# tanmayrainanda/ishara

Hardware: AMD Instinct MI355X
Metric: landmark-frames/sec training (B=256,T=384,d=256) (higher is better)
Workload: dtype bf16; 1 GPU; configs[1]: get_model(dim=256, 2 squeeze + 2 conformer blocks, kernel_sizes=[11,5,3]) CTC train step (fwd+CTC+bwd+RAdam/Lookahead, dropout on); batch_per_gpu=256, global_batch=256, frames=384, features=224, params=7577784, parallelism=dp1, ranks_seen=1

## Files before the change

### include/ishara_hip.h

```cpp
#ifndef ISHARA_HIP_H
#define ISHARA_HIP_H
#include <stdint.h>
#ifdef __cplusplus
extern "C" {
#endif

typedef struct ishara_model ishara_model;
typedef void* ishara_stream;

enum { ISHARA_F32 = 0, ISHARA_BF16 = 1, ISHARA_F16 = 2 };
enum { ISHARA_FAMILY_KERAS_HYBRID = 0, ISHARA_FAMILY_TORCH_CONFORMER = 1, ISHARA_FAMILY_TORCH_SQUEEZEFORMER = 2 };

typedef struct ishara_config {
    int32_t dim;
    int32_t num_conv_squeeze_blocks;
    int32_t num_conv_conform_blocks;
    int32_t num_kernel_sizes;
    int32_t kernel_sizes[8];
    int32_t num_conv_per_block;
    float   dropout_rate;
    int32_t num_heads;
    int32_t expansion_factor;
    int32_t transformer_kernel_size;
    int32_t frames;
    int32_t features;
    int32_t num_classes;
    int32_t top_dim;
    int32_t squeeze_expansion;
    int32_t conformer_expansion;
    float   head_dropout;
    float   conformer_attn_dropout;
    int32_t dtype;
    int32_t max_batch;
    int32_t max_label_len;
    int32_t attn_impl;
    int32_t family;
    int32_t reduce_layer_index;
    int32_t recover_layer_index;
    int32_t half_step_residual;
} ishara_config;

const char* ishara_last_error(void);

int  ishara_create(const ishara_config* cfg, ishara_model** out);
void ishara_destroy(ishara_model* m);

int64_t ishara_param_total(const ishara_model* m);
int64_t ishara_param_trainable(const ishara_model* m);
int32_t ishara_param_entries(const ishara_model* m);
int  ishara_param_info(const ishara_model* m, int32_t i, const char** name, int32_t* ndim,
                       int64_t shape[2], int64_t* offset, int32_t* trainable);
int64_t ishara_workspace_bytes(const ishara_model* m);

int32_t ishara_workspace_plan_check(const ishara_model* m);
int ishara_workspace_guard_check(ishara_model* m);

int ishara_bind(ishara_model* m, float* params, float* grads, float* opt_m, float* opt_v,
                float* opt_slow, void* workspace, int64_t workspace_bytes);
int ishara_sync_weights(ishara_model* m, ishara_stream s);

int ishara_forward(ishara_model* m, const float* x, int32_t B, float* logits, int32_t training,
                   uint32_t seed, ishara_stream s);
int ishara_loss_backward(ishara_model* m, const float* logits, const int64_t* labels, int32_t B,
                         float* loss, float* nll, float loss_scale, ishara_stream s);
int ishara_encoder_forward(ishara_model* m, const float* x, int32_t B, float* y, int32_t training, uint32_t seed, ishara_stream s);
int32_t ishara_encoder_output_frames(const ishara_model* m);
int ishara_encoder_backward(ishara_model* m, const float* dy, int32_t B, float* dx, ishara_stream s);
int32_t ishara_grad_buckets(const ishara_model* m);
int ishara_grad_bucket(const ishara_model* m, int32_t i, int64_t* offset, int64_t* count);
int ishara_grad_buckets_enable(ishara_model* m);
int ishara_grad_bucket_wait(ishara_model* m, int32_t i, ishara_stream side);
int ishara_optimizer_step(ishara_model* m, float lr, float weight_decay, ishara_stream s);
int32_t ishara_optimizer_iterations(const ishara_model* m);
int ishara_optimizer_set_iterations(ishara_model* m, int32_t it);

int ishara_profile_enable(ishara_model* m, int32_t on);
int ishara_profile_report(ishara_model* m, char* buf, int32_t cap);

int ishara_greedy_decode(const float* logits, int32_t B, int32_t T, int32_t C, int32_t blank,
                         int32_t* out_idx, int32_t* out_len, ishara_stream s);
int ishara_preprocess(const float* raw, const int32_t* n_frames, int32_t max_frames, const float* mean, const float* stdv,
                      float* out, int32_t T, ishara_stream s);
int ishara_preprocess_batch(const float* raw, int64_t n_total, const int64_t* offsets, int32_t B, int32_t max_frames,
                            const float* mean, const float* stdv, float* out, int32_t T, ishara_stream s);
int ishara_edit_distance(const int32_t* out_idx, const int32_t* out_len, int32_t B, int32_t T, const int32_t* targets, int32_t L,
                         int32_t* dist, int32_t* tlen, ishara_stream s);

int64_t ishara_ctc_beam_workspace_bytes(int32_t B, int32_t T, int32_t C, int32_t beam_width);
int ishara_ctc_beam_decode(const float* logits, int32_t B, int32_t T, int32_t C, int32_t blank, int32_t beam_width, int32_t nbest,
                           const float* lm, float alpha, float beta, void* workspace,
                           int32_t* out_idx, int32_t* out_len, float* out_score, ishara_stream s);

int64_t ishara_ctc_align_workspace_bytes(int32_t B, int32_t T, int32_t L);
int ishara_ctc_align(const float* logits, const int64_t* labels, int32_t B, int32_t T, int32_t C, int32_t L, int32_t blank,
                     void* ws, int32_t* frame_pos, int32_t* start, int32_t* end, float* conf, float* score, ishara_stream s);

typedef struct ishara_clip_aug {
    int64_t offset;
    int32_t n;
    int32_t L1;
    int32_t shift;
    int32_t L2;
    int32_t mirror;
    int32_t t0[3];
    int32_t t1[3];
    int32_t fingers[3];
} ishara_clip_aug;
enum { ISHARA_LAYOUT_FLAT = 0, ISHARA_LAYOUT_HANDS_LIPS_XY = 1 };
int ishara_clip_batch(const float* raw, const ishara_clip_aug* clips, int32_t B, int32_t T, int32_t layout,
                      float* x, ishara_stream s);
int64_t ishara_ctc_workspace_bytes(int32_t B, int32_t T, int32_t L);
int ishara_ctc_loss(const float* logits, const int64_t* labels, int32_t B, int32_t T, int32_t C,
                    int32_t L, int32_t blank, float* nll, float* dlogits, float grad_scale,
                    void* ws, ishara_stream s);
int ishara_dropout_mask(uint32_t seed, uint32_t site, int32_t rows, int32_t cols, float rate,
                        float* out, ishara_stream s);

int ishara_debug_set_as_flags(int32_t flags);
int ishara_debug_set_nt_big(int32_t on);
int ishara_debug_force_regstage(int32_t on);
int32_t ishara_debug_module_count(ishara_model* m);
int ishara_debug_module_info(ishara_model* m, int32_t i, const char** name, int32_t* in_cols, int32_t* out_cols, int32_t* first_site, int32_t* n_sites);
int ishara_debug_module_forward(ishara_model* m, int32_t i, const float* x, int32_t B, float* y, int32_t training, uint32_t seed, ishara_stream s);
int ishara_debug_module_backward(ishara_model* m, int32_t i, const float* dy, int32_t B, float* dx, ishara_stream s);
int ishara_debug_head_loss_backward(ishara_model* m, const float* logits, const int64_t* labels, int32_t B, float* loss, float* nll,
                                    float loss_scale, float* dx, ishara_stream s);

int64_t ishara_op_scratch_bytes(int32_t M, int32_t K, int32_t N);
int ishara_op_dense_fwd(int32_t dt, const void* x, const float* W, const float* bias, void* y,
                        int32_t M, int32_t K, int32_t N, int32_t act, void* scratch, ishara_stream s);
int ishara_op_dense_fwd_ex(int32_t dt, const void* x, const float* W, const float* bias, const void* resid, void* y,
                           int32_t M, int32_t K, int32_t N, int32_t act, void* scratch, ishara_stream s);
int ishara_op_dense_bwd(int32_t dt, const void* x, const float* W, const void* dy, void* dx,
                        float* dW, float* db, int32_t M, int32_t K, int32_t N, void* scratch, ishara_stream s);
int64_t ishara_op_qkv_scratch_bytes(int32_t B, int32_t T, int32_t H, int32_t dh);
int ishara_op_qkv_fwd(int32_t dt, const void* x, const float* gamma, const float* beta, float eps, const float* W, const float* bias,
                      void* q, void* k, void* vt, int32_t B, int32_t T, int32_t H, int32_t dh, int32_t head_major, void* scratch, ishara_stream s);
int ishara_op_classifier_fwd(int32_t dt, const void* x, const float* W, const float* bias, float* logits, int32_t M, int32_t K, int32_t C,
                             int32_t route, void* scratch, ishara_stream s);
int ishara_op_ctc_loss(const float* logits, const int64_t* labels, int32_t B, int32_t T, int32_t C, int32_t L, int32_t blank,
                       float* nll, float* dlogits, float grad_scale, void* ws, void* dlb, ishara_stream s);
int ishara_op_log_softmax_fwd(const float* x, float* y, int32_t M, int32_t C, int32_t ld, ishara_stream s);
int ishara_op_log_softmax_bwd(const float* dy, const float* y, float* dx, int32_t M, int32_t C, int32_t ld, ishara_stream s);
int ishara_op_layernorm_fwd(int32_t dt, const void* x, const float* gamma, const float* beta, float eps,
                            void* y, float* mean, float* rstd, int32_t M, int32_t C, ishara_stream s);
int ishara_op_layernorm_bwd(int32_t dt, const void* dy, const void* x, const float* mean, const float* rstd,
                            const float* gamma, void* dx, float* dgamma, float* dbeta, int32_t M, int32_t C,
                            ishara_stream s);
int ishara_op_dwconv_fwd(int32_t dt, int32_t inop, const void* x, const float* w, const float* bias, void* y,
                         float* ssum, float* ssq, int32_t B, int32_t T, int32_t C, int32_t k, int32_t padl,
                         ishara_stream s);
int64_t ishara_op_dwconv_fwd_scratch_bytes(int32_t B, int32_t T, int32_t C);
int ishara_op_dwconv_fwd_ex(int32_t dt, int32_t inop, const void* x, const float* w, const float* bias, void* y,
                            float* ssum, float* ssq, void* scratch, int32_t B, int32_t T, int32_t C, int32_t k,
                            int32_t padl, ishara_stream s);
int64_t ishara_op_dwconv_scratch_bytes(int32_t C, int32_t k);
int ishara_op_dwconv_bwd(int32_t dt, int32_t inop, const void* dy, const void* x, const float* w, void* dx,
                         float* dw, float* dbias, void* scratch, int32_t B, int32_t T, int32_t C, int32_t k,
                         int32_t padl, ishara_stream s);
int64_t ishara_op_attn_scratch_bytes(int32_t B, int32_t H, int32_t T, int32_t dh);
int ishara_op_attn_scratch_layout_bytes(int32_t B, int32_t H, int32_t T, int32_t dh, int64_t* out);
int ishara_op_attn_fwd(int32_t dt, const void* qkv, void* o, int32_t B, int32_t H, int32_t T, int32_t dh,
                       float scale, uint32_t seed, uint32_t site, float rate, int32_t impl,
                       void* scratch, ishara_stream s);
int ishara_op_attn_bwd(int32_t dt, const void* o, const void* dout, void* dqkv, int32_t B, int32_t H,
                       int32_t T, int32_t dh, float scale, uint32_t seed, uint32_t site, float rate,
                       int32_t impl, void* scratch, ishara_stream s);

int64_t ishara_op_relattn_scratch_bytes(int32_t B, int32_t H, int32_t T, int32_t dh);
int ishara_op_relattn_fwd(int32_t dt, const void* q, const void* k, const void* v, const float* pe, const float* Wpos, const float* u, const float* vb,
                          void* o, float* lse, int32_t B, int32_t H, int32_t T, int32_t dh, uint32_t seed, uint32_t site, float rate,
                          void* scratch, ishara_stream s);
int ishara_op_relattn_bwd(int32_t dt, const void* q, const void* k, const void* v, const float* u, const float* vb, const void* o, const void* dO,
                          void* dq, void* dk, void* dv, float* du, float* dvb, float* dWpos, float* dposp,
                          int32_t B, int32_t H, int32_t T, int32_t dh, uint32_t seed, uint32_t site, float rate, void* scratch, ishara_stream s);
int64_t ishara_op_r4_subsample_scratch_bytes(int32_t B, int32_t T0, int32_t F, int32_t d);
int ishara_op_r4_subsample_fwd(int32_t dt, const float* x, const float* w1, const float* b1, const float* w2, const float* b2, void* sub,
                               int32_t B, int32_t T0, int32_t F, int32_t d, void* scratch, ishara_stream s);
int ishara_op_r4_subsample_bwd(int32_t dt, const float* x, const float* w1, const float* w2, const void* sub, const void* dsub,
                               float* dw1, float* db1, float* dw2, float* db2, float* dx, int32_t B, int32_t T0, int32_t F, int32_t d,
                               void* scratch, ishara_stream s);
int64_t ishara_op_r4_time_reduce_scratch_bytes(int32_t B, int32_t Tin, int32_t d);
int ishara_op_r4_time_reduce_fwd(int32_t dt, const void* h, const float* conv_w, const float* conv_b, const float* Wred, const float* bred,
                                 void* red, void* conv_out, int32_t B, int32_t Tin, int32_t d, void* scratch, ishara_stream s);
int ishara_op_r4_time_reduce_bwd(int32_t dt, const void* h, const float* conv_w, const void* dred, const void* extra, void* dh,
                                 float* dconv_w, float* dconv_b, float* dWred, float* dbred, int32_t B, int32_t Tin, int32_t d,
                                 void* scratch, ishara_stream s);
int ishara_op_r4_rows(int32_t dt, int32_t mode, const void* src, const void* a, void* dst, int32_t B, int32_t Tdst, int32_t Tsrc, int32_t d,
                      ishara_stream s);

#ifdef __cplusplus
}
#endif
#endif
```

### ishara_amd/_lib.py

```python
from __future__ import annotations

import ctypes as C
import os

_HERE = os.path.dirname(os.path.abspath(__file__))
LIB_PATH = os.path.join(_HERE, "libishara_hip.so")

F32, BF16, F16 = 0, 1, 2
FAMILY_KERAS_HYBRID, FAMILY_TORCH_CONFORMER, FAMILY_TORCH_SQUEEZEFORMER = 0, 1, 2


class IsharaError(RuntimeError):
    pass


class Config(C.Structure):
    _fields_ = [
        ("dim", C.c_int32), ("num_conv_squeeze_blocks", C.c_int32), ("num_conv_conform_blocks", C.c_int32),
        ("num_kernel_sizes", C.c_int32), ("kernel_sizes", C.c_int32 * 8), ("num_conv_per_block", C.c_int32),
        ("dropout_rate", C.c_float), ("num_heads", C.c_int32), ("expansion_factor", C.c_int32),
        ("transformer_kernel_size", C.c_int32), ("frames", C.c_int32), ("features", C.c_int32),
        ("num_classes", C.c_int32), ("top_dim", C.c_int32), ("squeeze_expansion", C.c_int32),
        ("conformer_expansion", C.c_int32), ("head_dropout", C.c_float), ("conformer_attn_dropout", C.c_float),
        ("dtype", C.c_int32), ("max_batch", C.c_int32), ("max_label_len", C.c_int32), ("attn_impl", C.c_int32),
        ("family", C.c_int32), ("reduce_layer_index", C.c_int32), ("recover_layer_index", C.c_int32), ("half_step_residual", C.c_int32),
    ]


class ClipAug(C.Structure):
    _fields_ = [
        ("offset", C.c_int64), ("n", C.c_int32), ("L1", C.c_int32), ("shift", C.c_int32), ("L2", C.c_int32),
        ("mirror", C.c_int32), ("t0", C.c_int32 * 3), ("t1", C.c_int32 * 3), ("fingers", C.c_int32 * 3),
    ]


LAYOUT_FLAT, LAYOUT_HANDS_LIPS_XY = 0, 1


_P, _I32, _I64, _U32, _F = C.c_void_p, C.c_int32, C.c_int64, C.c_uint32, C.c_float
SIGNATURES = {
    "ishara_last_error": (C.c_char_p, []),
    "ishara_create": (C.c_int, [C.POINTER(Config), C.POINTER(_P)]),
    "ishara_destroy": (None, [_P]),
    "ishara_param_total": (_I64, [_P]),
    "ishara_param_trainable": (_I64, [_P]),
    "ishara_param_entries": (_I32, [_P]),
    "ishara_param_info": (C.c_int, [_P, _I32, C.POINTER(C.c_char_p), C.POINTER(_I32), C.POINTER(_I64 * 2), C.POINTER(_I64), C.POINTER(_I32)]),
    "ishara_workspace_bytes": (_I64, [_P]),
    "ishara_workspace_plan_check": (_I32, [_P]),
    "ishara_workspace_guard_check": (C.c_int, [_P]),
    "ishara_grad_buckets": (_I32, [_P]),
    "ishara_grad_bucket": (C.c_int, [_P, _I32, C.POINTER(C.c_int64), C.POINTER(C.c_int64)]),
    "ishara_grad_buckets_enable": (C.c_int, [_P]),
    "ishara_grad_bucket_wait": (C.c_int, [_P, _I32, _P]),
    "ishara_bind": (C.c_int, [_P, _P, _P, _P, _P, _P, _P, _I64]),
    "ishara_sync_weights": (C.c_int, [_P, _P]),
    "ishara_forward": (C.c_int, [_P, _P, _I32, _P, _I32, _U32, _P]),
    "ishara_encoder_forward": (C.c_int, [_P, _P, _I32, _P, _I32, _U32, _P]),
    "ishara_encoder_backward": (C.c_int, [_P, _P, _I32, _P, _P]),
    "ishara_encoder_output_frames": (_I32, [_P]),
    "ishara_loss_backward": (C.c_int, [_P, _P, _P, _I32, _P, _P, _F, _P]),
    "ishara_optimizer_step": (C.c_int, [_P, _F, _F, _P]),
    "ishara_optimizer_iterations": (_I32, [_P]),
    "ishara_optimizer_set_iterations": (C.c_int, [_P, _I32]),
    "ishara_profile_enable": (C.c_int, [_P, _I32]),
    "ishara_profile_report": (C.c_int, [_P, C.c_char_p, _I32]),
    "ishara_greedy_decode": (C.c_int, [_P, _I32, _I32, _I32, _I32, _P, _P, _P]),
    "ishara_preprocess": (C.c_int, [_P, _P, _I32, _P, _P, _P, _I32, _P]),
    "ishara_preprocess_batch": (C.c_int, [_P, _I64, _P, _I32, _I32, _P, _P, _P, _I32, _P]),
    "ishara_edit_distance": (C.c_int, [_P, _P, _I32, _I32, _P, _I32, _P, _P, _P]),
    "ishara_ctc_beam_workspace_bytes": (_I64, [_I32, _I32, _I32, _I32]),
    "ishara_ctc_beam_decode": (C.c_int, [_P, _I32, _I32, _I32, _I32, _I32, _I32, _P, _F, _F, _P, _P, _P, _P, _P]),
    "ishara_ctc_align_workspace_bytes": (_I64, [_I32, _I32, _I32]),
    "ishara_ctc_align": (C.c_int, [_P, _P, _I32, _I32, _I32, _I32, _I32, _P, _P, _P, _P, _P, _P, _P]),
    "ishara_clip_batch": (C.c_int, [_P, _P, _I32, _I32, _I32, _P, _P]),
    "ishara_ctc_workspace_bytes": (_I64, [_I32, _I32, _I32]),
    "ishara_ctc_loss": (C.c_int, [_P, _P, _I32, _I32, _I32, _I32, _I32, _P, _P, _F, _P, _P]),
    "ishara_op_ctc_loss": (C.c_int, [_P, _P, _I32, _I32, _I32, _I32, _I32, _P, _P, _F, _P, _P, _P]),
    "ishara_dropout_mask": (C.c_int, [_U32, _U32, _I32, _I32, _F, _P, _P]),
    "ishara_debug_set_as_flags": (C.c_int, [_I32]),
    "ishara_debug_set_nt_big": (C.c_int, [_I32]),
    "ishara_debug_force_regstage": (C.c_int, [_I32]),
    "ishara_debug_module_count": (_I32, [_P]),
    "ishara_debug_module_info": (C.c_int, [_P, _I32, C.POINTER(C.c_char_p), C.POINTER(_I32), C.POINTER(_I32), C.POINTER(_I32), C.POINTER(_I32)]),
    "ishara_debug_module_forward": (C.c_int, [_P, _I32, _P, _I32, _P, _I32, _U32, _P]),
    "ishara_debug_module_backward": (C.c_int, [_P, _I32, _P, _I32, _P, _P]),
    "ishara_debug_head_loss_backward": (C.c_int, [_P, _P, _P, _I32, _P, _P, _F, _P, _P]),
    "ishara_op_scratch_bytes": (_I64, [_I32, _I32, _I32]),
    "ishara_op_dense_fwd": (C.c_int, [_I32, _P, _P, _P, _P, _I32, _I32, _I32, _I32, _P, _P]),
    "ishara_op_dense_fwd_ex": (C.c_int, [_I32, _P, _P, _P, _P, _P, _I32, _I32, _I32, _I32, _P, _P]),
    "ishara_op_dense_bwd": (C.c_int, [_I32, _P, _P, _P, _P, _P, _P, _I32, _I32, _I32, _P, _P]),
    "ishara_op_qkv_scratch_bytes": (_I64, [_I32, _I32, _I32, _I32]),
    "ishara_op_qkv_fwd": (C.c_int, [_I32, _P, _P, _P, _F, _P, _P, _P, _P, _P, _I32, _I32, _I32, _I32, _I32, _P, _P]),
    "ishara_op_classifier_fwd": (C.c_int, [_I32, _P, _P, _P, _P, _I32, _I32, _I32, _I32, _P, _P]),
    "ishara_op_log_softmax_fwd": (C.c_int, [_P, _P, _I32, _I32, _I32, _P]),
    "ishara_op_log_softmax_bwd": (C.c_int, [_P, _P, _P, _I32, _I32, _I32, _P]),
    "ishara_op_layernorm_fwd": (C.c_int, [_I32, _P, _P, _P, _F, _P, _P, _P, _I32, _I32, _P]),
    "ishara_op_layernorm_bwd": (C.c_int, [_I32, _P, _P, _P, _P, _P, _P, _P, _P, _I32, _I32, _P]),
    "ishara_op_dwconv_fwd": (C.c_int, [_I32, _I32, _P, _P, _P, _P, _P, _P, _I32, _I32, _I32, _I32, _I32, _P]),
    "ishara_op_dwconv_scratch_bytes": (_I64, [_I32, _I32]),
    "ishara_op_dwconv_fwd_scratch_bytes": (_I64, [_I32, _I32, _I32]),
    "ishara_op_dwconv_fwd_ex": (C.c_int, [_I32, _I32, _P, _P, _P, _P, _P, _P, _P, _I32, _I32, _I32, _I32, _I32, _P]),
    "ishara_op_dwconv_bwd": (C.c_int, [_I32, _I32, _P, _P, _P, _P, _P, _P, _P, _I32, _I32, _I32, _I32, _I32, _P]),
    "ishara_op_attn_scratch_bytes": (_I64, [_I32, _I32, _I32, _I32]),
    "ishara_op_attn_scratch_layout_bytes": (C.c_int, [_I32, _I32, _I32, _I32, C.POINTER(_I64)]),
    "ishara_op_attn_fwd": (C.c_int, [_I32, _P, _P, _I32, _I32, _I32, _I32, _F, _U32, _U32, _F, _I32, _P, _P]),
    "ishara_op_attn_bwd": (C.c_int, [_I32, _P, _P, _P, _I32, _I32, _I32, _I32, _F, _U32, _U32, _F, _I32, _P, _P]),
    "ishara_op_relattn_scratch_bytes": (_I64, [_I32, _I32, _I32, _I32]),
    "ishara_op_relattn_fwd": (C.c_int, [_I32] + [_P] * 9 + [_I32, _I32, _I32, _I32, _U32, _U32, _F, _P, _P]),
    "ishara_op_relattn_bwd": (C.c_int, [_I32] + [_P] * 14 + [_I32, _I32, _I32, _I32, _U32, _U32, _F, _P, _P]),
    "ishara_op_r4_subsample_scratch_bytes": (_I64, [_I32, _I32, _I32, _I32]),
    "ishara_op_r4_subsample_fwd": (C.c_int, [_I32] + [_P] * 6 + [_I32, _I32, _I32, _I32, _P, _P]),
    "ishara_op_r4_subsample_bwd": (C.c_int, [_I32] + [_P] * 10 + [_I32, _I32, _I32, _I32, _P, _P]),
    "ishara_op_r4_time_reduce_scratch_bytes": (_I64, [_I32, _I32, _I32]),
    "ishara_op_r4_time_reduce_fwd": (C.c_int, [_I32] + [_P] * 7 + [_I32, _I32, _I32, _P, _P]),
    "ishara_op_r4_time_reduce_bwd": (C.c_int, [_I32] + [_P] * 9 + [_I32, _I32, _I32, _P, _P]),
    "ishara_op_r4_rows": (C.c_int, [_I32, _I32, _P, _P, _P, _I32, _I32, _I32, _I32, _P]),
}

_lib = None


def load():
    global _lib
    if _lib is not None:
        return _lib
    if not os.path.exists(LIB_PATH):
        raise IsharaError(f"{LIB_PATH} is missing: build it with `python -m ishara_amd.build` "
                          "(hipcc --offload-arch=gfx950); there is no CPU fallback")
    lib = C.CDLL(LIB_PATH)
    for name, (res, args) in SIGNATURES.items():
        fn = getattr(lib, name)
        fn.restype = res
        fn.argtypes = args
    _lib = lib
    return lib


def check(rc: int, what: str = ""):
    if rc != 0:
        msg = load().ishara_last_error()
        raise IsharaError(f"{what} failed (rc={rc}): {msg.decode() if msg else '?'}")


def ptr(t):
    return None if t is None else C.c_void_p(t.data_ptr())


def stream():
    import torch
    return C.c_void_p(torch.cuda.current_stream().cuda_stream)


def aligned(nbytes: int, device):
    import torch
    t = torch.empty(int(nbytes) + 256, dtype=torch.uint8, device=device)
    return t, C.c_void_p(t.data_ptr() + (-t.data_ptr()) % 256)
```

### ishara_amd/csrc/api_ops.hip

```cpp
#include "model_types.h"

__global__ void dropout_mask_kernel(float* out, int rows, int cols, DropSpec d) {
    const size_t n = (size_t)rows * cols;
    for (size_t i = (size_t)blockIdx.x * blockDim.x + threadIdx.x; i < n; i += (size_t)gridDim.x * blockDim.x) {
        const uint32_t r = (uint32_t)(i / cols), c = (uint32_t)(i % cols);
        out[i] = (d.thr == 0u || rng_keep(rng_row_key(d.key, r), c, d.thr)) ? d.scale : 0.f;
    }
}
template <typename T>
__global__ void qkv_split_kernel(const T* qkv, T* q, T* k, T* vt, int B, int H, int Tn, int dh) {
    const int d = H * dh;
    const size_t n = (size_t)B * Tn * 3 * d;
    for (size_t i = (size_t)blockIdx.x * blockDim.x + threadIdx.x; i < n; i += (size_t)gridDim.x * blockDim.x) {
        const size_t m = i / (3 * d);
        const int col = (int)(i - m * 3 * d);
        const int h = col / (3 * dh), w = col - h * 3 * dh, part = w / dh, e = w - part * dh;
        const int b = (int)(m / Tn), t = (int)(m - (size_t)b * Tn);
        const T v = qkv[i];
        if (part == 0) q[((size_t)(b * H + h) * Tn + t) * dh + e] = v;
        else if (part == 1) k[((size_t)(b * H + h) * Tn + t) * dh + e] = v;
        else vt[((size_t)(b * H + h) * dh + e) * Tn + t] = v;
    }
}

// ... 55 lines not shown
                                       const float* mean, const float* stdv, float* out, int32_t T, ishara_stream s) {
    if (max_frames <= 0 || max_frames > 8192) { ishara_set_error("ishara_preprocess_batch: max_frames %d unsupported (1..8192)", max_frames); return -1; }
    if (B < 0 || B > 65535 || T < 1 || T > 4096) { ishara_set_error("ishara_preprocess_batch: B=%d T=%d unsupported (0 <= B <= 65535, 1 <= T <= 4096)", B, T); return -1; }
    if (n_total < 0) { ishara_set_error("ishara_preprocess_batch: n_total %lld < 0", (long long)n_total); return -1; }
    if (B > 0 && (!offsets || !mean || !stdv || !out || (n_total > 0 && !raw))) { ishara_set_error("ishara_preprocess_batch: null raw / offsets / mean / stdv / out"); return -1; }
    if (((uintptr_t)raw | (uintptr_t)out) % 16) { ishara_set_error("ishara_preprocess_batch: raw and out must be 16-byte aligned"); return -1; }
    return launch_preprocess_batch(raw, n_total, offsets, B, max_frames, mean, stdv, out, T, (hipStream_t)s);
}
extern "C" int ishara_edit_distance(const int32_t* out_idx, const int32_t* out_len, int32_t B, int32_t T, const int32_t* targets, int32_t L,
                                    int32_t* dist, int32_t* tlen, ishara_stream s) {
    if (L < 1 || L > SCORE_MAX_L) { ishara_set_error("ishara_edit_distance: target length L=%d unsupported (1..%d: one wavefront lane per target symbol)", L, SCORE_MAX_L); return -1; }
    if (B < 0 || T < 1 || T > 4096) { ishara_set_error("ishara_edit_distance: B=%d T=%d unsupported (B >= 0, 1 <= T <= 4096)", B, T); return -1; }
    if (B > 0 && (!out_idx || !out_len || !targets || !dist || !tlen)) { ishara_set_error("ishara_edit_distance: null argument"); return -1; }
    return launch_edit_distance(out_idx, out_len, B, T, targets, L, dist, tlen, (hipStream_t)s);
}
extern "C" int64_t ishara_ctc_beam_workspace_bytes(int32_t B, int32_t T, int32_t C, int32_t beam_width) {
    (void)C;
    if (B < 0 || T < 1 || T > 4096 || beam_width < 1 || beam_width > 32) return -1;
    return (int64_t)B * (int64_t)ctc_beam_workspace_words(T, beam_width) * 4;
}
extern "C" int ishara_ctc_beam_decode(const float* logits, int32_t B, int32_t T, int32_t C, int32_t blank, int32_t beam_width, int32_t nbest,
                                      const float* lm, float alpha, float beta, void* workspace,
                                      int32_t* out_idx, int32_t* out_len, float* out_score, ishara_stream s) {
    if (C < 2 || C > 64) { ishara_set_error("ishara_ctc_beam_decode: C=%d unsupported (2..64: one lane per class)", C); return -1; }
    if (blank < 0 || blank >= C) { ishara_set_error("ishara_ctc_beam_decode: blank %d outside 0..%d", blank, C - 1); return -1; }
    if (beam_width < 1 || beam_width > 32) { ishara_set_error("ishara_ctc_beam_decode: beam_width %d unsupported (1..32)", beam_width); return -1; }
    if (nbest < 1 || nbest > beam_width) { ishara_set_error("ishara_ctc_beam_decode: nbest %d outside 1..beam_width=%d", nbest, beam_width); return -1; }
    if (B < 0 || B > 2147483647 / 2 || T < 1 || T > 4096) { ishara_set_error("ishara_ctc_beam_decode: B=%d T=%d unsupported (B >= 0, 1 <= T <= 4096)", B, T); return -1; }
    if (!(alpha == alpha && beta == beta) || alpha - alpha != 0.0f || beta - beta != 0.0f) { ishara_set_error("ishara_ctc_beam_decode: alpha and beta must be finite"); return -1; }
    if (B > 0 && (!logits || !workspace || !out_idx || !out_len || !out_score)) { ishara_set_error("ishara_ctc_beam_decode: null argument"); return -1; }
    if ((uintptr_t)workspace % 4) { ishara_set_error("ishara_ctc_beam_decode: workspace must be 4-byte aligned"); return -1; }
    return launch_ctc_beam(logits, B, T, C, blank, beam_width, nbest, lm, alpha, beta, workspace, out_idx, out_len, out_score, (hipStream_t)s);
}
extern "C" int64_t ishara_ctc_align_workspace_bytes(int32_t B, int32_t T, int32_t L) {
    if (B < 0 || T < 1 || T > 4096 || L < 1 || L > 255) return -1;
    return (int64_t)ctc_align_workspace_bytes(B, T, L);
}
extern "C" int ishara_ctc_align(const float* logits, const int64_t* labels, int32_t B, int32_t T, int32_t C, int32_t L, int32_t blank,
                                void* ws, int32_t* frame_pos, int32_t* start, int32_t* end, float* conf, float* score, ishara_stream s) {
    const char* me = "ishara_ctc_align";
    if (B < 0) { ishara_set_error("%s: B=%d < 0", me, B); return -1; }
    if (T < 1 || T > 4096) { ishara_set_error("%s: T=%d outside 1..4096", me, T); return -1; }
    if (L < 1 || L > 255) { ishara_set_error("%s: L=%d outside 1..255 (2L+1 lattice states in at most 8 registers of a 64-lane wave)", me, L); return -1; }
    if (C < 2 || C > 64) { ishara_set_error("%s: C=%d outside 2..64", me, C); return -1; }
    if (blank < 0 || blank >= C) { ishara_set_error("%s: blank %d outside 0..%d", me, blank, C - 1); return -1; }
    if (B == 0) return 0;
    if (!logits || !labels || !ws || !frame_pos || !start || !end || !conf || !score) {
        ishara_set_error("%s: null logits / labels / ws / frame_pos / start / end / conf / score", me); return -1;
    }
    if ((uintptr_t)ws % 16) { ishara_set_error("%s: ws must be 16-byte aligned", me); return -1; }
    return launch_ctc_align(logits, labels, B, T, C, L, blank, ws, frame_pos, start, end, conf, score, (hipStream_t)s);
}
extern "C" int ishara_clip_batch(const float* raw, const ishara_clip_aug* clips, int32_t B, int32_t T, int32_t layout,
                                 float* x, ishara_stream s) {
    if (B < 0 || T < 1 || T > CLIP_MAX_T) { ishara_set_error("ishara_clip_batch: B=%d T=%d unsupported (B >= 0, 1 <= T <= %d)", B, T, CLIP_MAX_T); return -1; }
    if (layout != ISHARA_LAYOUT_FLAT && layout != ISHARA_LAYOUT_HANDS_LIPS_XY) { ishara_set_error("ishara_clip_batch: unknown layout %d", layout); return -1; }
    if (B > 0 && (!clips || !x)) { ishara_set_error("ishara_clip_batch: null clips / x"); return -1; }
    if (((uintptr_t)raw | (uintptr_t)x) % 16) { ishara_set_error("ishara_clip_batch: raw and x must be 16-byte aligned"); return -1; }
    return launch_clip_batch(raw, clips, B, T, layout, x, (hipStream_t)s);
}

static bool op_dt_ok(const char* op, int dt, bool f16_ok) {
    if (dt != DT_F32 && dt != DT_BF16 && dt != DT_F16) { ishara_set_error("%s: unknown dtype %d (ISHARA_F32 = 0, ISHARA_BF16 = 1, ISHARA_F16 = 2)", op, dt); return false; }
    if (dt == DT_F16 && !f16_ok) { ishara_set_error("%s: ISHARA_F16 is inference-only (no fp16 backward kernels)", op); return false; }
    return true;
}
#define OP_DT(op, dt, f16_ok) do { if (!op_dt_ok(op, dt, f16_ok)) return -1; } while (0)
struct OpShadow {
    size_t wt, wn, slab, total; int ldt, ldn;
    OpShadow(int dt, int K, int N, int M) {
        const int bk = dt_is16(dt) ? 64 : 32;
        const size_t es = dt_size(dt);
        ldt = (int)rup(K, bk); ldn = (int)rup(N, bk);
        wt = 0;
        wn = rup(rup(N, 128) * (size_t)ldt * es, 256);
        slab = wn + rup(rup(K, 128) * (size_t)ldn * es, 256);
        total = slab + gemm_tn_slab_floats(M, K, N, dt) * sizeof(float);
    }
    int build(int dt, const float* Wm, int K, int N, char* sc, hipStream_t s) const {
        HIP_CHECK_RET(hipMemsetAsync(sc, 0, slab, s));
        return launch_make_shadow(dt, Wm, K, N, sc + wt, ldt, sc + wn, ldn, s);
    }
};
extern "C" int64_t ishara_op_scratch_bytes(int32_t M, int32_t K, int32_t N) {
    return (int64_t)OpShadow(DT_F32, K, N, M).total;
}
extern "C" int ishara_op_dense_fwd(int32_t dt, const void* x, const float* Wm, const float* bias, void* y, int32_t M, int32_t K, int32_t N, int32_t act, void* scratch, ishara_stream st) {
    OP_DT("ishara_op_dense_fwd", dt, true);
    hipStream_t s = (hipStream_t)st;
    const OpShadow sh(dt, K, N, M);
    char* sc = (char*)scratch;
    CK(sh.build(dt, Wm, K, N, sc, s));
    OpArgs no; EpiArgs ea; ea.bias = bias; ea.act = act; ea.dbg = g_dbg_epi;
    return launch_gemm_nt(dt, dt, dt, OP_NONE, x, sc + sh.wt, y, M, N, K, sh.ldt, no, ea, s);
}
extern "C" int ishara_op_dense_fwd_ex(int32_t dt, const void* x, const float* Wm, const float* bias, const void* resid, void* y,
                                      int32_t M, int32_t K, int32_t N, int32_t act, void* scratch, ishara_stream st) {
    OP_DT("ishara_op_dense_fwd_ex", dt, true);
    hipStream_t s = (hipStream_t)st;
    const OpShadow sh(dt, K, N, M);
    char* sc = (char*)scratch;
    CK(sh.build(dt, Wm, K, N, sc, s));
    OpArgs no; EpiArgs ea; ea.bias = bias; ea.act = act; ea.resid = resid; ea.dbg = g_dbg_epi;
    return launch_gemm_nt(dt, dt, dt, OP_NONE, x, sc + sh.wt, y, M, N, K, sh.ldt, no, ea, s);
}
extern "C" int ishara_op_dense_bwd(int32_t dt, const void* x, const float* Wm, const void* dy, void* dx, float* dW, float* db,
                                   int32_t M, int32_t K, int32_t N, void* scratch, ishara_stream st) {
    OP_DT("ishara_op_dense_bwd", dt, false);
    hipStream_t s = (hipStream_t)st;
    const OpShadow sh(dt, K, N, M);
    char* sc = (char*)scratch;
    CK(sh.build(dt, Wm, K, N, sc, s));
    OpArgs no; EpiArgs ea;
    if (dx) CK(launch_gemm_nt(dt, dt, dt, OP_NONE, dy, sc + sh.wn, dx, M, K, N, sh.ldn, no, ea, s));
    return launch_gemm_tn(dt, dt, dt, OP_NONE, OP_NONE, x, dy, dW, db, (float*)(sc + sh.slab), M, K, N, no, no, s);
}
static void qkv_scratch_layout(int B, int T, int H, int dh, size_t& xn, size_t& mean, size_t& rstd, size_t& total) {
    const int M = B * T, d = H * dh;
    xn = rup(OpShadow(DT_F32, d, 3 * d, M).total, 256);
    mean = xn + rup((size_t)M * d * 4, 256);
    rstd = mean + rup((size_t)M * 4, 256);
    total = rstd + rup((size_t)M * 4, 256);
}
extern "C" int64_t ishara_op_qkv_scratch_bytes(int32_t B, int32_t T, int32_t H, int32_t dh) {
    if (B < 1 || T < 1 || H < 1 || dh < 1) return -1;
    size_t xn, mean, rstd, total;
    qkv_scratch_layout(B, T, H, dh, xn, mean, rstd, total);
    return (int64_t)total;
}
extern "C" int ishara_op_qkv_fwd(int32_t dt, const void* x, const float* gamma, const float* beta, float eps, const float* Wm, const float* bias,
                                 void* q, void* k, void* vt, int32_t B, int32_t T, int32_t H, int32_t dh, int32_t head_major, void* scratch, ishara_stream st) {
    OP_DT("ishara_op_qkv_fwd", dt, true);
    if (B < 1 || T < 1 || H < 1 || dh < 1 || T % 8 != 0 || dh % 8 != 0 || (head_major != 0 && head_major != 1)) {
        ishara_set_error("ishara_op_qkv_fwd: B=%d T=%d H=%d dh=%d head_major=%d unsupported (T, dh multiples of 8; head_major 0 / 1)", B, T, H, dh, head_major); return -1;
    }
    const int d = H * dh, M = B * T;
    if ((gamma != nullptr) != (beta != nullptr) || (gamma && d > 512)) { ishara_set_error("ishara_op_qkv_fwd: LayerNorm needs both gamma and beta and H*dh <= 512 (H*dh=%d)", d); return -1; }
    if (!x || !Wm || !q || !k || !vt || !scratch || ((uintptr_t)x | (uintptr_t)scratch) % 16 != 0) { ishara_set_error("ishara_op_qkv_fwd: null or misaligned buffer (x, scratch: 16-byte aligned)"); return -1; }
    hipStream_t s = (hipStream_t)st;
    const OpShadow sh(dt, d, 3 * d, M);
    char* sc = (char*)scratch;
    CK(sh.build(dt, Wm, d, 3 * d, sc, s));
    OpArgs no;
    EpiArgs eq; eq.mode = EPI_QKV; eq.q = q; eq.k = k; eq.vt = vt; eq.H = H; eq.dh = dh; eq.T = T; eq.head_major = head_major;
    const void* A = x;
    if (gamma && !ln_as_prologue(dt, M, 3 * d, d, sh.ldt, gamma, beta, eps, nullptr, nullptr, nullptr, eq)) {
        size_t xn, mean, rstd, tot;
        qkv_scratch_layout(B, T, H, dh, xn, mean, rstd, tot);
        CK(launch_layernorm_fwd(dt, x, gamma, beta, eps, sc + xn, (float*)(sc + mean), (float*)(sc + rstd), M, d, s));
        A = sc + xn;
    }
    eq.bias = bias;
    return launch_gemm_nt(dt, dt, dt, OP_NONE, A, sc + sh.wt, nullptr, M, 3 * d, d, sh.ldt, no, eq, s);
}
extern "C" int ishara_op_classifier_fwd(int32_t dt, const void* x, const float* Wm, const float* bias, float* logits, int32_t M, int32_t K, int32_t C,
                                        int32_t route, void* scratch, ishara_stream st) {
    OP_DT("ishara_op_classifier_fwd", dt, true);
    if (route < CLS_AUTO || route > CLS_GEMM) { ishara_set_error("ishara_op_classifier_fwd: unknown route %d (0 auto, 1 A-stationary, 2 dense_narrow, 3 GEMM)", route); return -1; }
    if (M < 1 || K < 1 || C < 1) { ishara_set_error("ishara_op_classifier_fwd: bad shape M=%d K=%d C=%d", M, K, C); return -1; }
    const int r = route == CLS_AUTO ? cls_route_auto(dt, M, K, C) : route;
    const char* why = nullptr;
    if (r != CLS_GEMM && !dt_is16(dt)) why = "16-bit operands only";
    else if (r == CLS_AS && (C > 64 || C % 4 != 0 || (K != 256 && K != 512))) why = "C <= 64, C % 4 == 0 and K 256 / 512 only";
    else if (r == CLS_AS && g_force_regstage) why = "the A-stationary kernel is switched off (ishara_debug_force_regstage)";
    else if (r == CLS_NARROW && (C > 64 || K % 32 != 0)) why = "C <= 64 and K % 32 == 0 only";
    else if (r == CLS_GEMM && K % (dt_is16(dt) ? 8 : 4) != 0) why = "16-byte operand rows only";
    if (why) { ishara_set_error("ishara_op_classifier_fwd: route %d does not take dt=%d M=%d K=%d C=%d: %s", r, dt, M, K, C, why); return -1; }
    if (!x || !Wm || !logits || !scratch || ((uintptr_t)x | (uintptr_t)scratch) % 16 != 0) { ishara_set_error("ishara_op_classifier_fwd: null or misaligned buffer (x, scratch: 16-byte aligned)"); return -1; }
    hipStream_t s = (hipStream_t)st;
    const OpShadow sh(dt, K, C, M);
    char* sc = (char*)scratch;
    CK(sh.build(dt, Wm, K, C, sc, s));
    return classifier_fwd(nullptr, r, dt, x, sc + sh.wt, sh.ldt, bias, logits, M, K, C, s);
}
extern "C" int ishara_op_log_softmax_fwd(const float* x, float* y, int32_t M, int32_t C, int32_t ld, ishara_stream s) { return launch_log_softmax_fwd(x, y, M, C, ld, (hipStream_t)s); }
extern "C" int ishara_op_log_softmax_bwd(const float* dy, const float* y, float* dx, int32_t M, int32_t C, int32_t ld, ishara_stream s) { return launch_log_softmax_bwd(dy, y, dx, M, C, ld, (hipStream_t)s); }
extern "C" int ishara_op_layernorm_fwd(int32_t dt, const void* x, const float* gamma, const float* beta, float eps, void* y, float* mean, float* rstd, int32_t M, int32_t C, ishara_stream s) {
    OP_DT("ishara_op_layernorm_fwd", dt, true);
    return launch_layernorm_fwd(dt, x, gamma, beta, eps, y, mean, rstd, M, C, (hipStream_t)s);
}
extern "C" int ishara_op_layernorm_bwd(int32_t dt, const void* dy, const void* x, const float* mean, const float* rstd, const float* gamma, void* dx, float* dgamma, float* dbeta, int32_t M, int32_t C, ishara_stream s) {
    OP_DT("ishara_op_layernorm_bwd", dt, false);
    return launch_layernorm_bwd(dt, dy, x, mean, rstd, gamma, nullptr, dx, dgamma, dbeta, nullptr, M, C, (hipStream_t)s);
}
extern "C" int ishara_op_dwconv_fwd(int32_t dt, int32_t inop, const void* x, const float* w, const float* bias, void* y, float* ssum, float* ssq,
                                    int32_t B, int32_t T, int32_t C, int32_t k, int32_t padl, ishara_stream s) {
    OP_DT("ishara_op_dwconv_fwd", dt, true);
    return launch_dwconv_fwd(dt, inop, x, w, bias, y, ssum, ssq, nullptr, B, T, C, k, padl, (hipStream_t)s);
}
extern "C" int64_t ishara_op_dwconv_fwd_scratch_bytes(int32_t B, int32_t T, int32_t C) { return (int64_t)(dwconv_fwd_scratch_floats(B, T, C) * sizeof(float)); }
extern "C" int ishara_op_dwconv_fwd_ex(int32_t dt, int32_t inop, const void* x, const float* w, const float* bias, void* y, float* ssum, float* ssq,
                                       void* scratch, int32_t B, int32_t T, int32_t C, int32_t k, int32_t padl, ishara_stream s) {
    OP_DT("ishara_op_dwconv_fwd_ex", dt, true);
    return launch_dwconv_fwd(dt, inop, x, w, bias, y, ssum, ssq, (float*)scratch, B, T, C, k, padl, (hipStream_t)s);
}
extern "C" int64_t ishara_op_dwconv_scratch_bytes(int32_t C, int32_t k) { return (int64_t)(dwconv_bwd_scratch_floats(C, k) * sizeof(float)); }
extern "C" int ishara_op_dwconv_bwd(int32_t dt, int32_t inop, const void* dy, const void* x, const float* w, void* dx, float* dw, float* dbias,
                                    void* scratch, int32_t B, int32_t T, int32_t C, int32_t k, int32_t padl, ishara_stream s) {
    OP_DT("ishara_op_dwconv_bwd", dt, false);
    return launch_dwconv_bwd(dt, inop, dy, x, w, dx, dw, dbias, (float*)scratch, B, T, C, k, padl, (hipStream_t)s);
}
struct AttnScratch {
    void *q, *k, *vt; float *lse, *delta; uint32_t* maskw; size_t total;
    AttnScratch(char* sc, int B, int H, int T, int dh) {
        const size_t seg = rup((size_t)B * H * T * dh * 4, 256), row = rup((size_t)B * H * T * 4, 256);
        q = sc; k = sc + seg; vt = sc + 2 * seg;
        lse = (float*)(sc + 3 * seg);
        delta = (float*)(sc + 3 * seg + row);
        maskw = (uint32_t*)(sc + 3 * seg + 2 * row);
        total = 3 * seg + 2 * row + rup(attn_mask_words(B, H, T) * 4, 256);
    }
};
extern "C" int64_t ishara_op_attn_scratch_bytes(int32_t B, int32_t H, int32_t T, int32_t dh) { return (int64_t)AttnScratch(nullptr, B, H, T, dh).total; }
extern "C" int ishara_op_attn_scratch_layout_bytes(int32_t B, int32_t H, int32_t T, int32_t dh, int64_t* out) {
    const char* me = "ishara_op_attn_scratch_layout_bytes";
    if (B < 1 || H < 1 || T < 1 || dh < 1) { ishara_set_error("%s: B=%d H=%d T=%d dh=%d: B, H, T and dh must be >= 1", me, B, H, T, dh); return -1; }
    if (!out) { ishara_set_error("%s: null out", me); return -1; }
    const AttnScratch a(nullptr, B, H, T, dh);
    const int64_t row = (int64_t)B * H * T * 4;
    out[0] = (int64_t)(uintptr_t)a.lse; out[1] = row;
    out[2] = (int64_t)(uintptr_t)a.delta; out[3] = row;
    out[4] = (int64_t)(uintptr_t)a.maskw; out[5] = (int64_t)attn_mask_words(B, H, T) * 4;
    return 0;
}
static bool attn_takes_mfma(int dt, int dh, int impl) { return impl >= 1 && dt == DT_BF16 && (dh == 32 || dh == 64); }
static int attn_op_refused(const char* me, int dt, int B, int H, int T, int dh, float rate, int impl, std::initializer_list<const void*> operands,
                           std::initializer_list<const char*> operand_names, const void* scratch) {
    if (B < 1 || H < 1 || T < 1) { ishara_set_error("%s: B=%d H=%d T=%d: B, H and T must be >= 1", me, B, H, T); return -1; }
    if (dh != 8 && dh != 16 && dh != 24 && dh != 32 && dh != 48 && dh != 64) { ishara_set_error("%s: head dim %d unsupported (8, 16, 24, 32, 48, 64)", me, dh); return -1; }
    if (impl < 0 || impl > 2) { ishara_set_error("%s: unknown impl %d (0 lane-split, 1 MFMA with cached keep bits, 2 MFMA hashing again in the backward)", me, impl); return -1; }
    if (impl == 2 && !attn_takes_mfma(dt, dh, impl)) { ishara_set_error("%s: impl 2 has MFMA kernels only: ISHARA_BF16 and head dim 32 / 64 (dtype %d, head dim %d)", me, dt, dh); return -1; }
    if (attn_takes_mfma(dt, dh, impl) && T % 8 != 0) { ishara_set_error("%s: T=%d: the MFMA kernels need T %% 8 == 0 (16-byte pieces of the V^T rows)", me, T); return -1; }
    if (!(rate >= 0.f && rate < 1.f)) { ishara_set_error("%s: rate %g outside [0, 1)", me, rate); return -1; }
    if ((int64_t)B * H > 65535 || (int64_t)B * H * T * dh * 3 > 2147483647LL) { ishara_set_error("%s: B=%d H=%d T=%d dh=%d: shape too large (B*H <= 65535: one grid row per head; 3*B*H*T*dh < 2^31)", me, B, H, T, dh); return -1; }
    for (size_t i = 0; i < operands.size(); ++i) if (!operands.begin()[i]) { ishara_set_error("%s: null %s", me, operand_names.begin()[i]); return -1; }
    if (!scratch) { ishara_set_error("%s: null scratch (ishara_op_attn_scratch_bytes)", me); return -1; }
    for (size_t i = 0; i < operands.size(); ++i)
        if ((uintptr_t)operands.begin()[i] % 16) { ishara_set_error("%s: misaligned %s: 16-byte aligned operands (vector loads and stores)", me, operand_names.begin()[i]); return -1; }
    if ((uintptr_t)scratch % 256) { ishara_set_error("%s: misaligned scratch: 256-byte aligned (the layout rounds every region to 256 bytes)", me); return -1; }
    return 0;
}
extern "C" int ishara_op_attn_fwd(int32_t dt, const void* qkv, void* o, int32_t B, int32_t H, int32_t T, int32_t dh, float scale,
                                  uint32_t seed, uint32_t site, float rate, int32_t impl, void* scratch, ishara_stream st) {
    OP_DT("ishara_op_attn_fwd", dt, true);
    if (dt == DT_F16 && rate > 0.f) { ishara_set_error("ishara_op_attn_fwd: ISHARA_F16 is inference-only: no attention dropout (rate %g)", rate); return -1; }
    if (attn_op_refused("ishara_op_attn_fwd", dt, B, H, T, dh, rate, impl, {qkv, o}, {"qkv", "o"}, scratch)) return -1;
    hipStream_t s = (hipStream_t)st;
    const AttnScratch a((char*)scratch, B, H, T, dh);
    if (dt == DT_BF16) hipLaunchKernelGGL(qkv_split_kernel<bf16>, dim3(1024), dim3(256), 0, s, (const bf16*)qkv, (bf16*)a.q, (bf16*)a.k, (bf16*)a.vt, B, H, T, dh);
    else if (dt == DT_F16) hipLaunchKernelGGL(qkv_split_kernel<f16>, dim3(1024), dim3(256), 0, s, (const f16*)qkv, (f16*)a.q, (f16*)a.k, (f16*)a.vt, B, H, T, dh);
    else hipLaunchKernelGGL(qkv_split_kernel<float>, dim3(1024), dim3(256), 0, s, (const float*)qkv, (float*)a.q, (float*)a.k, (float*)a.vt, B, H, T, dh);
    return launch_attn_fwd(dt, a.q, a.k, a.vt, o, a.lse, B, H, T, dh, scale, make_drop_attn(seed, site, rate, true), impl == 2 ? 1 : impl, impl == 2 ? nullptr : a.maskw, s);
}
extern "C" int ishara_op_attn_bwd(int32_t dt, const void* o, const void* dout, void* dqkv, int32_t B, int32_t H, int32_t T, int32_t dh, float scale,
                                  uint32_t seed, uint32_t site, float rate, int32_t impl, void* scratch, ishara_stream st) {
    OP_DT("ishara_op_attn_bwd", dt, false);
    if (attn_op_refused("ishara_op_attn_bwd", dt, B, H, T, dh, rate, impl, {o, dout, dqkv}, {"o", "dout", "dqkv"}, scratch)) return -1;
    hipStream_t s = (hipStream_t)st;
    const AttnScratch a((char*)scratch, B, H, T, dh);
    return launch_attn_bwd(dt, a.q, a.k, a.vt, o, dout, a.lse, a.delta, dqkv, B, H, T, dh, scale, make_drop_attn(seed, site, rate, true), 1, impl == 2 ? 1 : impl,
                           impl == 2 ? nullptr : a.maskw, s);
}

static bool op_r4_dt_ok(const char* op, int dt) {
    if (dt != DT_F32 && dt != DT_BF16 && dt != DT_F16) { ishara_set_error("%s: unknown dtype %d (ISHARA_F32 = 0, ISHARA_BF16 = 1, ISHARA_F16 = 2)", op, dt); return false; }
    if (dt == DT_F16) { ishara_set_error("%s: ISHARA_F16 is not supported (the torch Squeezeformer family has no fp16 kernels)", op); return false; }
    return true;
}
#define OP_R4_DT(op, dt) do { if (!op_r4_dt_ok(op, dt)) return -1; } while (0)
static bool op_misaligned(std::initializer_list<const void*> ps) { uintptr_t a = 0; for (const void* p : ps) a |= (uintptr_t)p; return a % 16 != 0; }
static bool op_any_null(std::initializer_list<const void*> ps) { for (const void* p : ps) if (!p) return true; return false; }
static size_t op_shadow_bytes(int K, int N, int M) { const size_t a = OpShadow(DT_F32, K, N, M).total, b = OpShadow(DT_BF16, K, N, M).total; return rup(a > b ? a : b, 256); }

struct RelAttnScratch {
    size_t pedt, posp, dposp, lse, delta, total;
    RelAttnScratch(int B, int H, int T, int dh) {
        const size_t d = (size_t)H * dh, R = 2 * (size_t)T - 1, tab = rup(R * d * 4, 256), row = rup((size_t)B * H * T * 4, 256);
        pedt = op_shadow_bytes((int)d, (int)d, (int)R);
        posp = pedt + tab; dposp = posp + tab; lse = dposp + tab; delta = lse + row; total = delta + row;
    }
};
static const char* relattn_shape_error(int B, int H, int T, int dh, float rate) {
    if (dh != 8 && dh != 16 && dh != 32 && dh != 64) return "head dim unsupported (8, 16, 32, 64)";
    if (B < 1 || H < 1 || T < 1) return "B, H and T must be >= 1";
    if ((int64_t)B * H > 65535 || (int64_t)B * H * T * dh > 2147483647LL || (2 * (int64_t)T - 1) * H * dh > 2147483647LL) return "shape too large (B*H <= 65535, B*H*T*dh < 2^31)";
    if (!(rate >= 0.f && rate < 1.f)) return "rate outside [0, 1)";
    return nullptr;
}
extern "C" int64_t ishara_op_relattn_scratch_bytes(int32_t B, int32_t H, int32_t T, int32_t dh) {
    if (relattn_shape_error(B, H, T, dh, 0.f)) return -1;
    return (int64_t)RelAttnScratch(B, H, T, dh).total;
}
extern "C" int ishara_op_relattn_fwd(int32_t dt, const void* q, const void* k, const void* v, const float* pe, const float* Wpos, const float* u, const float* vb,
                                     void* o, float* lse, int32_t B, int32_t H, int32_t T, int32_t dh, uint32_t seed, uint32_t site, float rate, void* scratch, ishara_stream st) {
    const char* me = "ishara_op_relattn_fwd";
    OP_R4_DT(me, dt);
    if (const char* why = relattn_shape_error(B, H, T, dh, rate)) { ishara_set_error("%s: B=%d H=%d T=%d dh=%d rate=%g: %s", me, B, H, T, dh, rate, why); return -1; }
    if (op_any_null({q, k, v, pe, Wpos, u, vb, o, scratch}) || op_misaligned({q, k, v, pe, Wpos, u, vb, o, lse, scratch})) {
        ishara_set_error("%s: null or misaligned buffer (all 16-byte aligned; only lse may be NULL)", me); return -1;
    }
    hipStream_t s = (hipStream_t)st;
    const int d = H * dh, R = 2 * T - 1;
    const OpShadow sh(dt, d, d, R);
    const RelAttnScratch a(B, H, T, dh);
    char* sc = (char*)scratch;
    CK(sh.build(dt, Wpos, d, d, sc, s));
// ... 149 lines not shown
```

### ishara_amd/csrc/gemm_as.hip

```cpp
#include <cstdio>
#include <map>
#include <string>
#include <type_traits>
#include "common.h"
#include "kernels.h"

#ifdef AS_F16
typedef f16 as_t;
typedef f16x8 as_v8;
#define AS_MFMA(b, a, acc) __builtin_amdgcn_mfma_f32_16x16x32_f16(b, a, acc, 0, 0, 0)
#define AS_DT DT_F16
#define AS_NAME(x) x##_f16
#else
typedef bf16 as_t;
typedef bf16x8 as_v8;
#define AS_MFMA(b, a, acc) __builtin_amdgcn_mfma_f32_16x16x32_bf16(b, a, acc, 0, 0, 0)
#define AS_DT DT_BF16
#define AS_NAME(x) x
#endif

extern int g_force_regstage;
bool gemm_nt_as_applicable(int dtC, int M, int N, int K, int ldb, const EpiArgs& ea);

#define AS_NS 32
#define AS_SMALL_M 1536
#define AS_MID_M_K512 32768
#define AS_MAXN 1024

typedef __attribute__((ext_vector_type(4))) uint32_t as_u32x4;

template <int N> DEVI void as_wait_vm() { asm volatile("s_waitcnt vmcnt(%0)" ::"n"(N) : "memory"); }

DEVI int as_swz(int r) { return (r & 3) | (((r >> 3) & 1) << 2); }

template <int GW, typename T> DEVI void as_st(T* p, const float (&v)[GW]) {
    if constexpr (GW == 8) store8(p, v); else store4(p, v);
}
template <int GW, typename T> DEVI void as_st_nt(T* p, const float (&v)[GW], bool nt = true) {
    if constexpr (GW == 8 && is_16b_t<T>::value) {
        as_v8 t;
#pragma unroll
        for (int i = 0; i < 8; ++i) t[i] = (as_t)v[i];
        if (nt) __builtin_nontemporal_store(t, reinterpret_cast<as_v8*>(p)); else *reinterpret_cast<as_v8*>(p) = t;
    } else as_st<GW>(p, v);
}
DEVI void as_st_pk(as_t* p, const as_v8& t, bool nt) {
    if (nt) __builtin_nontemporal_store(t, reinterpret_cast<as_v8*>(p)); else *reinterpret_cast<as_v8*>(p) = t;
}
template <typename TC, int GW> DEVI void as_unpack(const as_u32x4& r, float (&v)[GW]) {
    if constexpr (GW == 8 && std::is_same<TC, f16>::value) {
        const f16x8 h = __builtin_bit_cast(f16x8, r);
#pragma unroll
        for (int e = 0; e < 8; ++e) v[e] = (float)h[e];
    } else if constexpr (GW == 8) {
#pragma unroll
        for (int h = 0; h < 4; ++h) { v[2 * h] = __uint_as_float(r[h] << 16); v[2 * h + 1] = __uint_as_float(r[h] & 0xffff0000u); }
    } else {
#pragma unroll
        for (int h = 0; h < 4; ++h) v[h] = __uint_as_float(r[h]);
    }
}

enum { AS_RESID = 1, AS_DACT = 2, AS_ACT = 4, AS_DROP = 8, AS_ROWSCALE = 16, AS_PREOUT = 32, AS_QKV = 64, AS_ADDTAB = 128, AS_ALL = 255 };
template <int MASK, int F> DEVI bool as_on(bool runtime) {
    if constexpr ((MASK & F) == 0) return false;
    else if constexpr (MASK == AS_ALL) return runtime;
    else return true;
}

template <typename TC, int KT, int MASK, int RT, int DBG, int PRO, int NW = 4, int CS = 1>
DEVI void as_pass(const as_t* __restrict__ A, const as_t* __restrict__ Bt, TC* __restrict__ C, int M, int N, int ldb, const EpiArgs& ea,
                  char* smem, const float* bias_s, int m_base) {
    constexpr int RB = KT * 64;
    constexpr int NS = AS_NS;
    constexpr int SUB = NS * RB;
    constexpr int STAGE = SUB * CS;
    constexpr int R = CS > 1 ? 2 : (KT <= 8 ? 3 : 2);
    constexpr int K = KT * 32;
    constexpr int NI = STAGE / 1024;
    constexpr int DPW = (NI + NW - 1) / NW;
    constexpr bool PAIR = is_16b_t<TC>::value;
    constexpr int GW = PAIR ? 8 : 4;
    constexpr int NG = NS / (4 * GW);
    constexpr int SPS = RT * NG;
    constexpr bool COUNTED = (MASK & (AS_RESID | AS_DACT | AS_ADDTAB | AS_QKV)) == 0;
    constexpr int OPS = SPS * ((MASK & AS_PREOUT) ? 2 : 1);
    constexpr bool HOLDABLE = PAIR && std::is_same<TC, as_t>::value && MASK != AS_ALL && (MASK & AS_QKV) == 0;
    const bool hold = HOLDABLE && (ea.as_flags & 1) && !ea.n_valid;
    const bool nt_side = (ea.as_flags & 2) != 0;

    const int dbg = DBG ? ea.dbg : 0;
    const int tid = threadIdx.x, lane = tid & 63;
    const int wid = __builtin_amdgcn_readfirstlane(tid >> 6);
    const int c = lane & 15, g = lane >> 4;
    const int mw = m_base + wid * 16 * RT;
    const bool full = m_base + NW * 16 * RT <= M;
    const int nsteps = N / NS / (int)gridDim.y;
    const int nbase = (int)blockIdx.y * nsteps * NS;
    const int dmodel = ea.H * ea.dh;
    const bool f_resid = as_on<MASK, AS_RESID>(ea.resid != nullptr), f_dact = as_on<MASK, AS_DACT>(ea.dact != DACT_NONE);
    const bool f_act = as_on<MASK, AS_ACT>(ea.act != ACT_NONE), f_drop = as_on<MASK, AS_DROP>(ea.drop.thr != 0);
    const bool f_rowscale = as_on<MASK, AS_ROWSCALE>(ea.rowscale != nullptr), f_preout = as_on<MASK, AS_PREOUT>(ea.pre_out != nullptr);
    const bool f_qkv = as_on<MASK, AS_QKV>(ea.mode == EPI_QKV), f_addtab = as_on<MASK, AS_ADDTAB>(ea.addtab != nullptr);

    const as_t* bsrc[DPW];
#pragma unroll
    for (int t = 0; t < DPW; ++t) {
        const int o = ((wid * DPW + t) % NI) * 1024 + lane * 16;
        const int r = o / RB, p = (o % RB) >> 4;
        bsrc[t] = Bt + (size_t)(nbase + r) * ldb + ((p ^ as_swz(r)) << 3);
    }
    const size_t bstep = (size_t)NS * CS * ldb;
    auto issue = [&](int slot) {
#pragma unroll
        for (int t = 0; t < DPW; ++t) {
            __builtin_amdgcn_global_load_lds((const __attribute__((address_space(1))) void*)bsrc[t],
                                             (__attribute__((address_space(3))) void*)(smem + slot + ((wid * DPW + t) % NI) * 1024), 16, 0, 0);
            bsrc[t] += bstep;
        }
    };
    const int nstages = (nsteps + CS - 1) / CS;
#pragma unroll
    for (int st = 0; st < R - 1; ++st)
        if (st < nstages && !(dbg & 8)) issue(st * STAGE);

    as_v8 a[RT][KT];
    int mrow[RT];
#pragma unroll
    for (int i = 0; i < RT; ++i) {
        mrow[i] = min(mw + 16 * i + c, M - 1);
        const as_v8* p = reinterpret_cast<const as_v8*>(A + (size_t)mrow[i] * K + g * 8);
#pragma unroll
        for (int kt = 0; kt < KT; ++kt) a[i][kt] = p[kt * 4];
    }

    if constexpr (PRO != 0) {
        float* cs = reinterpret_cast<float*>(smem + (R - 1) * STAGE);
        const int bsm = min(m_base, M - 1) / ea.T;
        const float* c0 = PRO == 1 ? ea.ln_gamma : ea.pa_P + (size_t)bsm * K;
        const float* c1 = PRO == 1 ? ea.ln_beta : ea.pa_Q + (size_t)bsm * K;
        for (int x = tid; x < K; x += NW * 64) { cs[x] = c0[x]; cs[K + x] = c1[x]; }
        __syncthreads();
        auto unpack = [&](const as_v8& f, float (&v)[8]) {
            as_u32x4 t = __builtin_bit_cast(as_u32x4, f);
            asm volatile("" : "+v"(t));
            as_unpack<as_t, 8>(t, v);
        };
        float mean[RT], rstd[RT];
#pragma unroll
        for (int i = 0; i < RT; ++i) { mean[i] = 0.f; rstd[i] = 1.f; }
        if constexpr (PRO == 1) {
#pragma unroll
            for (int i = 0; i < RT; ++i) {
                float s = 0.f;
#pragma unroll
                for (int kt = 0; kt < KT; ++kt) {
                    float v[8];
                    unpack(a[i][kt], v);
#pragma unroll
                    for (int e = 0; e < 8; ++e) s += v[e];
                }
                s += __shfl_xor(s, 16, 64); s += __shfl_xor(s, 32, 64);
                mean[i] = s * (1.f / K);
                float q = 0.f;
#pragma unroll
                for (int kt = 0; kt < KT; ++kt) {
                    float v[8];
                    unpack(a[i][kt], v);
#pragma unroll
                    for (int e = 0; e < 8; ++e) { const float dlt = v[e] - mean[i]; q += dlt * dlt; }
                }
                q += __shfl_xor(q, 16, 64); q += __shfl_xor(q, 32, 64);
                rstd[i] = rsqrtf(q * (1.f / K) + ea.ln_eps);
                const int m = mw + 16 * i + c;
                if (g == 0 && m < M && ea.ln_mean && blockIdx.y == 0) { ea.ln_mean[m] = mean[i]; ea.ln_rstd[m] = rstd[i]; }
            }
        }
#pragma unroll
        for (int kt = 0; kt < KT; ++kt) {
            float wv[8], bv[8];
            {
                const float* cp = cs + 32 * kt + 8 * g;
                asm volatile("" : "+v"(cp));
                const f32x4 w0 = *reinterpret_cast<const f32x4*>(cp), w1 = *reinterpret_cast<const f32x4*>(cp + 4);
                const f32x4 b0 = *reinterpret_cast<const f32x4*>(cp + K), b1 = *reinterpret_cast<const f32x4*>(cp + K + 4);
#pragma unroll
                for (int e = 0; e < 4; ++e) { wv[e] = w0[e]; wv[4 + e] = w1[e]; bv[e] = b0[e]; bv[4 + e] = b1[e]; }
            }
#pragma unroll
            for (int i = 0; i < RT; ++i) {
                float v[8];
                unpack(a[i][kt], v);
                as_v8 t;
#pragma unroll
                for (int e = 0; e < 8; ++e) t[e] = (as_t)(PRO == 1 ? (v[e] - mean[i]) * rstd[i] * wv[e] + bv[e] : v[e] * wv[e] + bv[e]);
                a[i][kt] = t;
            }
        }
        __syncthreads();
    }

    const int frow = PAIR ? 8 * (c >> 2) + (c & 3) : c;
    const int sx = g ^ as_swz(frow);
    const int off_e = frow * RB + ((sx & 3) << 4) + ((sx >> 2) << 6);
    const int off_o = frow * RB + ((sx & 3) << 4) + (((sx >> 2) ^ 1) << 6);
    constexpr int JSTRIDE = (PAIR ? 4 : 16) * RB;

    float rsc[RT];
    uint32_t rk[RT];
    int bsamp[RT];
#pragma unroll
    for (int i = 0; i < RT; ++i) {
        const int m = mw + 16 * i + c;
        rsc[i] = 1.f; rk[i] = 0u; bsamp[i] = 0;
        if (f_rowscale || f_qkv) bsamp[i] = mrow[i] / ea.T;
        if (f_rowscale) rsc[i] = ea.rowscale[bsamp[i]];
        if (f_drop) rk[i] = rng_row_key(ea.drop.key, (uint32_t)m);
    }

    size_t eoff[RT];
#pragma unroll
    for (int i = 0; i < RT; ++i) eoff[i] = (size_t)mrow[i] * (ea.ldc ? ea.ldc : N) + GW * g;
    const TC* resid = reinterpret_cast<const TC*>(ea.resid);
    const TC* aux = reinterpret_cast<const TC*>(ea.aux);

#pragma unroll
    for (int i = 0; i < RT; ++i) {
#pragma unroll
        for (int kt = 0; kt < KT; ++kt) {
            as_u32x4 t = __builtin_bit_cast(as_u32x4, a[i][kt]);
            asm volatile("" : "+v"(t));
            a[i][kt] = __builtin_bit_cast(as_v8, t);
        }
        asm volatile("" : "+v"(rsc[i]));
    }

    as_v8 held[RT], held_pre[RT];
#pragma unroll
    for (int i = 0; i < RT; ++i) { held[i] = as_v8{}; held_pre[i] = as_v8{}; }
    int slot = 0;
    for (int s = 0; s < nsteps; ++s) {
        const int sub = CS > 1 ? (s & (CS - 1)) : 0;
        const bool sync = CS == 1 || sub == 0;
        const int sg = CS > 1 ? s / CS : s;
        if (sync) {
            if constexpr (CS > 1) {
                constexpr bool CCOUNT = MASK != AS_ALL && (MASK & AS_QKV) == 0;
                if (CCOUNT && full && !ea.n_valid && sg >= 1) as_wait_vm<CS * OPS>(); else as_wait_vm<0>();
            } else if constexpr (COUNTED) {
                if (full && !ea.n_valid && s >= R - 1 && s + R - 2 < nsteps) {
                    if (!hold) as_wait_vm<(R - 2) * DPW + (R - 1) * OPS>();
                    else if constexpr (R == 3) as_wait_vm<DPW + 2 * OPS>();
                    else { if (s & 1) as_wait_vm<0>(); else as_wait_vm<2 * OPS>(); }
                } else as_wait_vm<0>();
            } else {
                if (s + R - 2 < nsteps) as_wait_vm<(R - 2) * DPW>(); else as_wait_vm<0>();
            }
            asm volatile("s_waitcnt lgkmcnt(0)" ::: "memory");
            __builtin_amdgcn_s_barrier();
        }
        const int n0 = nbase + s * NS;
        as_u32x4 rs[RT][NG], au[RT][NG];
        if (f_resid) {
#pragma unroll
            for (int i = 0; i < RT; ++i)
#pragma unroll
                for (int q = 0; q < NG; ++q) rs[i][q] = *reinterpret_cast<const as_u32x4*>(resid + eoff[i] + n0 + 4 * GW * q);
        }
        if (f_dact) {
#pragma unroll
            for (int i = 0; i < RT; ++i)
#pragma unroll
                for (int q = 0; q < NG; ++q) au[i][q] = __builtin_nontemporal_load(reinterpret_cast<const as_u32x4*>(aux + eoff[i] + n0 + 4 * GW * q));
        }
        if (sync && sg + R - 1 < nstages && !(dbg & 8)) issue(slot == 0 ? (R - 1) * STAGE : slot - STAGE);
        f32x4 acc[2][RT];
#pragma unroll
        for (int j = 0; j < 2; ++j)
#pragma unroll
            for (int i = 0; i < RT; ++i) acc[j][i] = f32x4{0.f, 0.f, 0.f, 0.f};
        const char* st = smem + slot + sub * SUB;
        if (!(dbg & 6)) {
#pragma unroll
            for (int kt = 0; kt < KT; ++kt) {
#pragma unroll
                for (int j = 0; j < 2; ++j) {
                    const as_v8 b = *reinterpret_cast<const as_v8*>(st + ((kt & 1) ? off_o : off_e) + (kt >> 1) * 128 + j * JSTRIDE);
#pragma unroll
                    for (int i = 0; i < RT; ++i) acc[j][i] = AS_MFMA(b, a[i][kt], acc[j][i]);
                }
            }
        } else if (!(dbg & 4)) {
#pragma unroll
            for (int kt = 0; kt < KT; ++kt)
#pragma unroll
                for (int j = 0; j < 2; ++j) {
                    const f32x4 b = *reinterpret_cast<const f32x4*>(st + ((kt & 1) ? off_o : off_e) + (kt >> 1) * 128 + j * JSTRIDE);
                    acc[j][0] += b;
                }
        } else if (!(dbg & 2)) {
            const as_v8 b = a[0][0];
#pragma unroll
            for (int kt = 0; kt < KT; ++kt)
#pragma unroll
                for (int j = 0; j < 2; ++j)
#pragma unroll
                    for (int i = 0; i < RT; ++i) acc[j][i] = AS_MFMA(b, a[i][kt], acc[j][i]);
        } else {
#pragma unroll
            for (int i = 0; i < RT; ++i) acc[0][i][0] = (float)a[i][0][0] + (float)a[i][KT - 1][7];
        }
        if (dbg & 1) { if (acc[0][0][0] == 123.456f) C[0] = from_f<TC>(acc[1][RT - 1][2]); if (CS == 1 || sub == CS - 1) slot = slot == (R - 1) * STAGE ? 0 : slot + STAGE; continue; }
#pragma unroll
        for (int q = 0; q < NG; ++q) {
            const int n = n0 + 4 * GW * q + GW * g;
            if (ea.n_valid && n >= ea.n_valid) continue;
            float bias[GW];
#pragma unroll
            for (int h = 0; h < GW / 4; ++h) {
                const f32x4 bv = *reinterpret_cast<const f32x4*>(bias_s + n + 4 * h);
#pragma unroll
                for (int e = 0; e < 4; ++e) bias[4 * h + e] = bv[e];
            }
#pragma unroll
            for (int i = 0; i < RT; ++i) {
                const int m = mw + 16 * i + c;
                if (!full && m >= M) continue;
                const size_t off = eoff[i] + n0 + 4 * GW * q;
                float v[GW];
                const float bsc = (f_rowscale && ea.rowscale_bias) ? rsc[i] : 1.f;
                if constexpr (PAIR) {
#pragma unroll
                    for (int e = 0; e < 4; ++e) { v[e] = acc[0][i][e] + bias[e] * bsc; v[4 + e] = acc[1][i][e] + bias[4 + e] * bsc; }
                } else {
#pragma unroll
                    for (int e = 0; e < 4; ++e) v[e] = acc[q][i][e] + bias[e] * bsc;
                }
                if (f_addtab) {
                    const float* tp = ea.addtab + (size_t)(m % ea.tab_period) * N + n;
#pragma unroll
                    for (int h = 0; h < GW / 4; ++h) {
                        float t4[4];
                        load4(tp + 4 * h, t4);
#pragma unroll
                        for (int e = 0; e < 4; ++e) v[4 * h + e] += t4[e];
                    }
                }
                if (f_preout) {
                    if constexpr (HOLDABLE) {
                        if (hold) {
                            as_v8 t;
#pragma unroll
                            for (int e = 0; e < 8; ++e) t[e] = (as_t)v[e];
                            as_t* pp = reinterpret_cast<as_t*>(ea.pre_out) + off;
                            if (s & 1) { as_st_pk(pp - NS, held_pre[i], nt_side); as_st_pk(pp, t, nt_side); }
                            else if (s == nsteps - 1) as_st_pk(pp, t, nt_side);
                            else held_pre[i] = t;
                        } else as_st_nt<GW>(reinterpret_cast<TC*>(ea.pre_out) + off, v, nt_side);
                    } else as_st_nt<GW>(reinterpret_cast<TC*>(ea.pre_out) + off, v, nt_side);
                }
                if (f_act) {
                    if (ea.act == ACT_SWISH) {
#pragma unroll
                        for (int e = 0; e < GW; ++e) v[e] = swishf_(v[e]);
                    } else {
#pragma unroll
                        for (int e = 0; e < GW; ++e) v[e] = fmaxf(v[e], 0.f);
                    }
                }
                if (f_drop) {
                    rng_apply<GW>(rk[i], (uint32_t)n, ea.drop.thr, ea.drop.scale, v);
                }
                if (f_rowscale && !ea.rowscale_bias) {
#pragma unroll
                    for (int e = 0; e < GW; ++e) v[e] *= rsc[i];
                }
                if (f_dact) {
                    float x[GW];
                    as_unpack<TC, GW>(au[i][q], x);
                    if (ea.dact == DACT_SWISH) {
#pragma unroll
                        for (int e = 0; e < GW; ++e) v[e] *= dswishf_(x[e]);
                    } else {
#pragma unroll
                        for (int e = 0; e < GW; ++e) v[e] = x[e] > 0.f ? v[e] : 0.f;
                    }
                }
                if (f_resid) {
                    float x[GW];
                    as_unpack<TC, GW>(rs[i][q], x);
#pragma unroll
                    for (int e = 0; e < GW; ++e) v[e] += x[e];
                }
                if (!f_qkv) {
                    if constexpr (HOLDABLE) {
                        if (hold) {
                            as_v8 t;
#pragma unroll
                            for (int e = 0; e < 8; ++e) t[e] = (as_t)v[e];
                            as_t* cp = reinterpret_cast<as_t*>(C) + off;
                            if (s & 1) { as_st_pk(cp - NS, held[i], false); as_st_pk(cp, t, false); }
                            else if (s == nsteps - 1) as_st_pk(cp, t, false);
                            else held[i] = t;
                        } else as_st<GW>(C + off, v);
                    } else as_st<GW>(C + off, v);
                } else {
                    int h, part, ii;
                    if (ea.head_major) { h = n / (3 * ea.dh); const int w = n - h * 3 * ea.dh; part = w / ea.dh; ii = w - part * ea.dh; }
                    else { part = n / dmodel; const int w = n - part * dmodel; h = w / ea.dh; ii = w - h * ea.dh; }
                    const int t = m - bsamp[i] * ea.T;
                    if (part < 2) {
                        as_st<GW>(reinterpret_cast<TC*>(part == 0 ? ea.q : ea.k) + ((size_t)(bsamp[i] * ea.H + h) * ea.T + t) * ea.dh + ii, v);
                    } else {
                        TC* dst = reinterpret_cast<TC*>(ea.vt) + ((size_t)(bsamp[i] * ea.H + h) * ea.dh + ii) * ea.T + t;
#pragma unroll
                        for (int e = 0; e < GW; ++e) dst[(size_t)e * ea.T] = from_f<TC>(v[e]);
                    }
                }
            }
        }
        if (CS == 1 || sub == CS - 1) slot = slot == (R - 1) * STAGE ? 0 : slot + STAGE;
    }
    if constexpr (PRO != 0) {
        if (ea.pro_out && blockIdx.y == 0) {
#pragma unroll
            for (int i = 0; i < RT; ++i) {
                const int m = mw + 16 * i + c;
                if (m < M) {
                    as_v8* p = reinterpret_cast<as_v8*>(reinterpret_cast<as_t*>(ea.pro_out) + (size_t)m * K + g * 8);
#pragma unroll
                    for (int kt = 0; kt < KT; ++kt) as_st_pk(reinterpret_cast<as_t*>(&p[kt * 4]), a[i][kt], nt_side);
                }
            }
        }
    }
}

template <typename TC, int KT, int MASK, int DBG = 0, int PRO = 0>
__global__ __launch_bounds__(KT <= 16 ? 256 : 512, KT <= 8 ? 3 : (KT <= 16 ? 2 : 1)) void gemm_nt_as_kernel(const as_t* __restrict__ A, const as_t* __restrict__ Bt, TC* __restrict__ C,
                                                                         int M, int N, int ldb, EpiArgs ea) {
    constexpr int R = KT <= 8 ? 3 : 2;
    constexpr int STAGE = AS_NS * KT * 64;
    __shared__ __attribute__((aligned(16))) char smem[R * STAGE + AS_MAXN * 4];
    float* bias_s = reinterpret_cast<float*>(smem + R * STAGE);
    for (int n = threadIdx.x; n < N; n += (int)blockDim.x) bias_s[n] = (ea.bias && (!ea.n_valid || n < ea.n_valid)) ? ea.bias[n] : 0.f;
    if constexpr (KT <= 8) {
        if (M <= AS_SMALL_M) as_pass<TC, KT, MASK, 1, DBG, PRO>(A, Bt, C, M, N, ldb, ea, smem, bias_s, blockIdx.x * 64);
        else as_pass<TC, KT, MASK, 2, DBG, PRO>(A, Bt, C, M, N, ldb, ea, smem, bias_s, blockIdx.x * 128);
    } else if constexpr (KT >= 32) {
        as_pass<TC, KT, MASK, 1, DBG, PRO, 8>(A, Bt, C, M, N, ldb, ea, smem, bias_s, blockIdx.x * 128);
    } else if (M <= AS_MID_M_K512) {
        as_pass<TC, KT, MASK, 1, DBG, PRO>(A, Bt, C, M, N, ldb, ea, smem, bias_s, blockIdx.x * 64);
    } else {
        const int m_base = blockIdx.x * 192;
        as_pass<TC, KT, MASK, 2, DBG, PRO>(A, Bt, C, M, N, ldb, ea, smem, bias_s, m_base);
        if (m_base + 128 < M) {
            __builtin_amdgcn_s_barrier();
            as_pass<TC, KT, MASK, 1, DBG, PRO>(A, Bt, C, M, N, ldb, ea, smem, bias_s, m_base + 128);
        }
    }
}

#define AS_CHUNK_ROWS 384
template <int KT> struct AsChunk { static constexpr int NW = KT <= 8 ? 12 : 8, CS = KT <= 8 ? 4 : 2; };
template <typename TC, int KT, int MASK, int PRO = 0>
__global__ __launch_bounds__(AsChunk<KT>::NW * 64, 1) void gemm_nt_as_chunk_kernel(const as_t* __restrict__ A, const as_t* __restrict__ Bt, TC* __restrict__ C, int M, int N, int ldb, EpiArgs ea) {
    extern __shared__ __attribute__((aligned(16))) char csm[];
    constexpr int NW = AsChunk<KT>::NW, CS = AsChunk<KT>::CS;
    constexpr int STAGE = AS_NS * KT * 64 * CS;
    float* bias_s = reinterpret_cast<float*>(csm + 2 * STAGE);
    for (int n = threadIdx.x; n < N; n += (int)blockDim.x) bias_s[n] = (ea.bias && (!ea.n_valid || n < ea.n_valid)) ? ea.bias[n] : 0.f;
    const int m_base = blockIdx.x * AS_CHUNK_ROWS;
    if constexpr (KT <= 8) {
        as_pass<TC, KT, MASK, 2, 0, PRO, NW, CS>(A, Bt, C, M, N, ldb, ea, csm, bias_s, m_base);
    } else {
        as_pass<TC, KT, MASK, 2, 0, PRO, NW, CS>(A, Bt, C, M, N, ldb, ea, csm, bias_s, m_base);
        if (m_base + 256 < M) {
            __builtin_amdgcn_s_barrier();
            as_pass<TC, KT, MASK, 1, 0, PRO, NW, CS>(A, Bt, C, M, N, ldb, ea, csm, bias_s, m_base + 256);
        }
    }
}
template <typename KF> static bool as_chunk_prepare(KF kernel, int bytes) {
    static std::map<const void*, bool> done;
    const void* key = reinterpret_cast<const void*>(kernel);
    auto it = done.find(key);
    if (it != done.end()) return it->second;
    const bool ok = hipFuncSetAttribute(key, hipFuncAttributeMaxDynamicSharedMemorySize, bytes) == hipSuccess;
    done[key] = ok;
    return ok;
}

static int as_mask_of(const EpiArgs& ea) {
    return (ea.resid ? AS_RESID : 0) | (ea.dact != DACT_NONE ? AS_DACT : 0) | (ea.act != ACT_NONE ? AS_ACT : 0) | (ea.drop.thr ? AS_DROP : 0) |
           (ea.rowscale ? AS_ROWSCALE : 0) | (ea.pre_out ? AS_PREOUT : 0) | (ea.mode == EPI_QKV ? AS_QKV : 0) | (ea.addtab ? AS_ADDTAB : 0);
}

static int as_inst_mask(bool c_bf16, int mask, int K = 256) {
    if (!c_bf16) return mask == 0 ? 0 : AS_ALL;
    if (K == 128) return (mask == AS_DACT || mask == (AS_DACT | AS_DROP)) ? mask : AS_ALL;
    switch (mask) {
        case 0: case AS_RESID: case AS_RESID | AS_ROWSCALE: case AS_ROWSCALE: case AS_RESID | AS_DROP: case AS_ACT | AS_PREOUT: case AS_ACT | AS_PREOUT | AS_DROP:
        case AS_ACT | AS_DROP: case AS_ACT: case AS_DACT: case AS_DACT | AS_DROP: case AS_QKV: case AS_ADDTAB: return mask;
        default: return AS_ALL;
    }
}

#define AS_LAUNCH_PLAIN(MASK, PRO) hipLaunchKernelGGL((gemm_nt_as_kernel<TC, KT, MASK, 0, PRO>), grid, block, 0, s, (const as_t*)A, (const as_t*)Bt, (TC*)C, M, N, ldb, ea)
#ifdef AS_F16
#define AS_LAUNCH2(MASK, PRO) AS_LAUNCH_PLAIN(MASK, PRO)
#else
#define AS_LAUNCH2(MASK, PRO)                                                                                                         \
    do {                                                                                                                              \
        if constexpr ((KT == 8 || KT == 16) && std::is_same<TC, as_t>::value && (MASK) != AS_ALL) {                                   \
            constexpr int CB = 2 * AS_NS * KT * 64 * AsChunk<KT>::CS + AS_MAXN * 4;                                                   \
            if (chunked && as_chunk_prepare(gemm_nt_as_chunk_kernel<TC, KT, MASK, PRO>, CB)) {                                        \
                hipLaunchKernelGGL((gemm_nt_as_chunk_kernel<TC, KT, MASK, PRO>), dim3((M + AS_CHUNK_ROWS - 1) / AS_CHUNK_ROWS), dim3(AsChunk<KT>::NW * 64), CB, s, \
                                   (const as_t*)A, (const as_t*)Bt, (TC*)C, M, N, ldb, ea);                                           \
                break;                                                                                                                \
            }                                                                                                                         \
        }                                                                                                                             \
        AS_LAUNCH_PLAIN(MASK, PRO);                                                                                                   \
    } while (0)
#endif
#define AS_LAUNCH(MASK) AS_LAUNCH2(MASK, 0)
#ifdef AS_F16
extern int g_as_flags_override;
#else
int g_as_flags_override = -1;
#endif
static int as_default_flags() {
    static const int v = getenv("ISHARA_AS_FLAGS") ? atoi(getenv("ISHARA_AS_FLAGS")) : 51;
    return g_as_flags_override >= 0 ? g_as_flags_override : v;
}
static bool as_chunk_applies(int flags, int M, int N, int K, const EpiArgs& ea) {
    const int cs = K == 256 ? 4 : 2;
    return (K == 256 ? (flags & 16) : (K == 512 && (flags & 32))) && M >= 128 * AS_CHUNK_ROWS && (N / AS_NS) % cs == 0 && N >= 128 && !ea.n_valid && !ea.dbg &&
           (!ea.pa_P || (ea.T > 0 && ea.T % AS_CHUNK_ROWS == 0));
}
template <typename TC, int KT>
static int run_as(const void* A, const void* Bt, void* C, int M, int N, int ldb, const EpiArgs& ea_in, hipStream_t s) {
    EpiArgs ea = ea_in;
    if (ea.as_flags < 0) ea.as_flags = as_default_flags();
    const int BR = KT <= 8 ? (M <= AS_SMALL_M ? 64 : 128) : (KT <= 16 ? (M <= AS_MID_M_K512 ? 64 : 192) : 128);
    const int gx = (M + BR - 1) / BR, slots = KT <= 8 ? 768 : (KT <= 16 ? 512 : 256);
    int gy = 1;
    const int max_gy = M <= AS_SMALL_M ? 16 : 4, min_cols = M <= AS_SMALL_M ? 32 : 128;
    while (gy < max_gy && gx * gy * 2 <= slots && (N / AS_NS) % (gy * 2) == 0 && N / (gy * 2) >= min_cols) gy *= 2;
    const dim3 grid(gx, gy), block(KT <= 16 ? 256 : 512);
    const int mask = as_mask_of(ea);
    const bool chunked = (KT == 8 || KT == 16) && as_chunk_applies(ea.as_flags, M, N, KT * 32, ea) && gy == 1;
    (void)chunked;
    if constexpr (is_16b_t<TC>::value && KT >= 8) {
#define AS_PRO(MASK, PRO) AS_LAUNCH2(MASK, PRO)
        if (ea.ln_gamma) {
            switch (mask) {
                case 0: AS_PRO(0, 1); break;
                case AS_ACT | AS_PREOUT: AS_PRO(AS_ACT | AS_PREOUT, 1); break;
                case AS_ACT | AS_PREOUT | AS_DROP: AS_PRO(AS_ACT | AS_PREOUT | AS_DROP, 1); break;
                case AS_QKV: AS_PRO(AS_QKV, 1); break;
                default: ishara_set_error("gemm_nt_as: LayerNorm prologue with epilogue mask %d is not compiled", mask); return -1;
            }
            return hipGetLastError() == hipSuccess ? 0 : -2;
        }
        if (ea.pa_P) {
            switch (mask) {
                case AS_RESID: AS_PRO(AS_RESID, 2); break;
                case AS_RESID | AS_ROWSCALE: AS_PRO(AS_RESID | AS_ROWSCALE, 2); break;
                default: ishara_set_error("gemm_nt_as: affine prologue with epilogue mask %d is not compiled", mask); return -1;
            }
            return hipGetLastError() == hipSuccess ? 0 : -2;
        }
#undef AS_PRO
    }
    if constexpr (KT == 4) {
        if (mask == AS_DACT) AS_LAUNCH(AS_DACT); else if (mask == (AS_DACT | AS_DROP)) AS_LAUNCH(AS_DACT | AS_DROP); else AS_LAUNCH(AS_ALL);
    }
#ifdef AS_F16
    else if constexpr (is_16b_t<TC>::value) {
        switch (mask) {
            case 0: AS_LAUNCH(0); break;
            case AS_RESID: AS_LAUNCH(AS_RESID); break;
            case AS_ACT | AS_PREOUT: AS_LAUNCH(AS_ACT | AS_PREOUT); break;
            case AS_ACT: AS_LAUNCH(AS_ACT); break;
            case AS_QKV: AS_LAUNCH(AS_QKV); break;
            case AS_ADDTAB: AS_LAUNCH(AS_ADDTAB); break;
            default: AS_LAUNCH(AS_ALL); break;
        }
    }
#else
    else if constexpr (is_16b_t<TC>::value) {
        switch (mask) {
            case 0:
                if (ea.dbg) hipLaunchKernelGGL((gemm_nt_as_kernel<TC, KT, 0, 1>), grid, block, 0, s, (const as_t*)A, (const as_t*)Bt, (TC*)C, M, N, ldb, ea);
                else AS_LAUNCH(0);
                break;
            case AS_RESID: AS_LAUNCH(AS_RESID); break;
            case AS_RESID | AS_ROWSCALE: AS_LAUNCH(AS_RESID | AS_ROWSCALE); break;
            case AS_ROWSCALE: AS_LAUNCH(AS_ROWSCALE); break;
            case AS_RESID | AS_DROP: AS_LAUNCH(AS_RESID | AS_DROP); break;
            case AS_ACT | AS_PREOUT: AS_LAUNCH(AS_ACT | AS_PREOUT); break;
            case AS_ACT | AS_PREOUT | AS_DROP: AS_LAUNCH(AS_ACT | AS_PREOUT | AS_DROP); break;
            case AS_ACT | AS_DROP: AS_LAUNCH(AS_ACT | AS_DROP); break;
            case AS_ACT: AS_LAUNCH(AS_ACT); break;
            case AS_DACT: AS_LAUNCH(AS_DACT); break;
            case AS_DACT | AS_DROP: AS_LAUNCH(AS_DACT | AS_DROP); break;
            case AS_QKV: AS_LAUNCH(AS_QKV); break;
            case AS_ADDTAB: AS_LAUNCH(AS_ADDTAB); break;
            default: AS_LAUNCH(AS_ALL); break;
        }
    }
#endif
    else {
        if (mask == 0) AS_LAUNCH(0); else AS_LAUNCH(AS_ALL);
    }
    return hipGetLastError() == hipSuccess ? 0 : -2;
}
#undef AS_LAUNCH

#ifndef AS_F16
bool gemm_nt_as_prologue_ok(int dtA, int dtM, int dtC, int M, int N, int K, int ldb, const EpiArgs& ea) {
    if (!dt_is16(dtA) || dtM != dtA || dtC != dtA || (K != 256 && K != 512 && !(K == 1024 && dtA == DT_BF16)) || !gemm_nt_as_applicable(dtC, M, N, K, ldb, ea)) return false;
    if (ldb % 64 != 0 || g_force_regstage) return false;
    const int BR = K == 256 ? (M <= AS_SMALL_M ? 64 : 128) : (K == 512 ? (M <= AS_MID_M_K512 ? 64 : 192) : 128), gx = (M + BR - 1) / BR, slots = K == 256 ? 768 : (K == 512 ? 512 : 256);
    (void)gx; (void)slots;
    const int mask = as_mask_of(ea);
    if (ea.ln_gamma) return mask == 0 || mask == (AS_ACT | AS_PREOUT) || mask == (AS_ACT | AS_PREOUT | AS_DROP) || mask == AS_QKV;
    if (ea.pa_P) return ea.T > 0 && ea.T % BR == 0 && (mask == AS_RESID || mask == (AS_RESID | AS_ROWSCALE));
    return false;
}

bool gemm_nt_as_applicable(int dtC, int M, int N, int K, int ldb, const EpiArgs& ea) {
    if (K != 256 && K != 512 && !((K == 128 || K == 1024) && dtC == DT_BF16)) return false;
    if (N % AS_NS != 0 || N > AS_MAXN || ldb < K || ldb % 8 != 0 || M < 1) return false;
    if (ea.mode == EPI_QKV && (ea.dh % 8 != 0 || ea.T % 8 != 0)) return false;
    return true;
}

const char* gemm_nt_as_name(int dtC, int K, const EpiArgs& ea, int M, int N) {
    static std::map<int, std::string> names;
    const int inst = as_inst_mask(dtC == DT_BF16, as_mask_of(ea), K);
    const int pro = ea.ln_gamma ? 1 : (ea.pa_P ? 2 : 0);
    const bool chunk = dtC == DT_BF16 && inst != AS_ALL && as_chunk_applies(ea.as_flags < 0 ? as_default_flags() : ea.as_flags, M, N, K, ea);
    const int id = (dtC == DT_BF16 ? 0 : 1 << 20) | (pro << 22) | (chunk ? 1 << 24 : 0) | (K << 8) | inst;
    auto it = names.find(id);
    if (it == names.end()) {
        char buf[96];
        if (chunk) snprintf(buf, sizeof buf, "gemm_nt_as_chunk_kernel<bf16,%d,%d,%d>", K / 32, pro ? as_mask_of(ea) : inst, pro);
        else if (pro) snprintf(buf, sizeof buf, "gemm_nt_as_kernel<%s,%d,%d,0,%d>", dtC == DT_BF16 ? "bf16" : "f32", K / 32, as_mask_of(ea), pro);
        else snprintf(buf, sizeof buf, "gemm_nt_as_kernel<%s,%d,%d,0>", dtC == DT_BF16 ? "bf16" : "f32", K / 32, inst);
        it = names.emplace(id, buf).first;
    }
    return it->second.c_str();
}

#endif

#ifdef AS_F16
int launch_gemm_nt_as_f16(int dtC, const void* A, const void* Bt, void* C, int M, int N, int K, int ldb, const EpiArgs& ea, hipStream_t s) {
    if ((K != 256 && K != 512) || !gemm_nt_as_applicable(dtC, M, N, K, ldb, ea)) return 1;
    if (dtC == DT_F16) return K == 256 ? run_as<f16, 8>(A, Bt, C, M, N, ldb, ea, s) : run_as<f16, 16>(A, Bt, C, M, N, ldb, ea, s);
    return K == 256 ? run_as<float, 8>(A, Bt, C, M, N, ldb, ea, s) : run_as<float, 16>(A, Bt, C, M, N, ldb, ea, s);
}
#else
int launch_gemm_nt_as(int dtC, const void* A, const void* Bt, void* C, int M, int N, int K, int ldb, const EpiArgs& ea, hipStream_t s) {
    if (!gemm_nt_as_applicable(dtC, M, N, K, ldb, ea)) return 1;
    if (dtC == DT_BF16) return K == 128 ? run_as<bf16, 4>(A, Bt, C, M, N, ldb, ea, s) : (K == 256 ? run_as<bf16, 8>(A, Bt, C, M, N, ldb, ea, s) :
                               (K == 512 ? run_as<bf16, 16>(A, Bt, C, M, N, ldb, ea, s) : run_as<bf16, 32>(A, Bt, C, M, N, ldb, ea, s)));
    return K == 256 ? run_as<float, 8>(A, Bt, C, M, N, ldb, ea, s) : run_as<float, 16>(A, Bt, C, M, N, ldb, ea, s);
}
#endif
```

### ishara_amd/csrc/keras_hybrid.hip

```cpp
#include "model_types.h"
#include <stdlib.h>

__global__ void droppath_kernel(float* rs, int B, DropSpec d) {
    const int b = blockIdx.x * blockDim.x + threadIdx.x;
    if (b < B) rs[b] = (d.thr == 0u || rng_keep(rng_row_key(d.key, (uint32_t)b), 0u, d.thr)) ? d.scale : 0.f;
}

static void build_conv(ishara_model* m, const std::string& name, int k) {
    ConvBlock cb;
    const int d = m->d, c = 2 * d;
    cb.k = k;
    cb.W1 = m->dense(name + "_expand_conv", d, c, true);
    cb.dw = m->addp(name + "_dwconv/depthwise_kernel", k, c, true);
    cb.bn = m->bnp(name + "_bn", c);
    cb.eca = m->addp(name + "_eca/kernel", 5, 0, true);
    cb.W2 = m->dense(name + "_project_conv", c, d, true);
    cb.site = m->nsites++;
    m->convs.push_back(cb);
    m->layers.push_back({Layer::CONV, (int)m->convs.size() - 1});
    m->layer_entry_end.push_back(m->entries.size());
}
static FFN build_ffn(ishara_model* m, Norm ln, float eps, const std::string& n1, const std::string& n2, int e, bool out_drop) {
    FFN f; f.ln = ln; f.eps = eps;
    f.Wa = m->dense(n1, m->d, m->d * e, true);
// ... 121 lines not shown
    m->shadow_tab_off = m->alloc(m->denses.size() * sizeof(ShadowDesc)).off;
    m->pe = m->f32((size_t)T * d);
    m->stem_h0 = m->act(d); m->stem_out = m->act(d);
    if (m->stem_kp) m->stem_xb = m->alloc(Mx * (size_t)m->stem_kp * 2);
    m->stem_ssum = m->f32((size_t)B * d); m->stem_ssq = m->f32((size_t)B * d);
    m->stem_mean = m->f32(d); m->stem_rstd = m->f32(d); m->stem_a = m->f32(d); m->stem_bsh = m->f32(d);
    for (auto& cb : m->convs) {
        const int c = 2 * d;
        cb.z1 = m->act(c); cb.h2 = m->act(c); cb.h4 = m->act(c); cb.out = m->act(d);
        cb.ssum = m->f32((size_t)B * c); cb.ssq = m->f32((size_t)B * c);
        cb.mean = m->f32(c); cb.rstd = m->f32(c); cb.a = m->f32(c); cb.bsh = m->f32(c);
        cb.gn = m->f32((size_t)B * c); cb.sg = m->f32((size_t)B * c); cb.P = m->f32((size_t)B * c); cb.Q = m->f32((size_t)B * c);
        cb.rs = m->f32(B);
    }
    auto plan_ffn_act = [&](FFN& f) {
        f.xn = m->act(d); f.mean = m->f32(Mx); f.rstd = m->f32(Mx);
        f.za = m->act(f.Wa.N); f.u = m->act(f.Wa.N); f.out = m->act(d);
    };
    auto plan_mhsa_act = [&](MHSA& a) {
        a.xn = m->act(d); a.mean = m->f32(Mx); a.rstd = m->f32(Mx);
        a.q = m->act(d); a.k = m->act(d); a.vt = m->act(d); a.o = m->act(d);
        a.lse = m->f32((size_t)B * m->H * T); a.out = m->act(d);
        a.maskw = m->f32(attn_mask_words(B, m->H, T));
    };
    for (auto& sb : m->sqz) {
        plan_ffn_act(sb.ffn1); plan_mhsa_act(sb.mha);
        SqzConv& c = sb.conv;
        const int de = c.Wc1.N;
        c.xn = m->act(d); c.mean = m->f32(Mx); c.rstd = m->f32(Mx);
        c.zc = m->act(de); c.zd = m->act(de); c.hd = m->act(de); c.u3 = m->act(d);
        c.gap = m->f32((size_t)B * d); c.hid = m->f32((size_t)B * c.R); c.se = m->f32((size_t)B * d); c.out = m->act(d);
        plan_ffn_act(sb.ffn2);
    }
    for (auto& cb : m->conf) {
        plan_ffn_act(cb.ffn1); plan_mhsa_act(cb.mha);
        plan_confconv(m, cb.conv, Mx, B, d);
        plan_ffn_act(cb.ffn2);
    }
    m->head_hh = m->act(m->dtop);
    int maxw = 3 * d;
    if (m->dtop > maxw) maxw = m->dtop;
    for (auto& sb : m->sqz) if (sb.ffn1.Wa.N > maxw) maxw = sb.ffn1.Wa.N;
    for (auto& cb : m->conf) if (cb.ffn1.Wa.N > maxw) maxw = cb.ffn1.Wa.N;
    m->gA = m->act(d); m->gB = m->act(d);
    m->t1 = m->act(maxw); m->t2 = m->act(maxw); m->t3 = m->act(maxw);
    const int maxc = 2 * d > maxw ? 2 * d : maxw;
    m->S1 = m->f32((size_t)B * maxc); m->S2 = m->f32((size_t)B * maxc); m->E = m->f32((size_t)B * maxc);
    m->Fc = m->f32(maxc); m->Ecol = m->f32(maxc); m->ecap = m->f32((size_t)B * 8 * ECA_MAX_CHUNKS);
    m->dse = m->f32((size_t)B * d); m->dgapT = m->f32((size_t)B * d);
    m->psa_on = m->dt == DT_BF16 && !m->convs.empty() && getenv("ISHARA_NO_PSA") == nullptr;
    if (m->psa_on) { m->psaG = m->f32((size_t)B * d); m->psaR = m->f32((size_t)B * (size_t)((d + 63) / 64) * 2 * d); }
    m->slab = m->f32(slab_floats(m, Mx, B, T, maxw));
    { const size_t wf = wgrad_slab_floats(m, Mx);
      m->slab2[0] = m->f32(wf); m->slab2[1] = m->f32(wf); m->tn_defer_on = getenv("ISHARA_NO_DEFERRED_SLAB_SUMS") == nullptr; }
    {
        size_t need = 0;
        const size_t lnf = (layernorm_bwd_scratch_floats(d) + 63) & ~(size_t)63, dwf = (dwconv_bwd_scratch_floats(2 * maxw, 31) + 63) & ~(size_t)63;
        need = (size_t)m->layers.size() * (5 * lnf + 2 * dwf);
        const size_t cap = (size_t)256 << 20;
        m->red_cap = need < cap ? need : cap;
        m->red_on = getenv("ISHARA_NO_DEFERRED_REDUCE") == nullptr && m->red_cap > 0;
        if (m->red_on) m->red_arena = m->f32(m->red_cap);
    }
    m->ctcws = m->f32(ctc_workspace_floats(B, T, m->L));
    m->dlogits = m->f32(Mx * m->C);
    if (m->cls_pad) m->dlb = m->alloc(Mx * (size_t)m->cls_pad * 2);
    m->nllb = m->f32(B);
    m->delta = m->f32((size_t)B * m->H * T);
    m->ws_need = m->cur;
}


static uint32_t* attn_maskw(ishara_model* m, const Buf& off) {
    static const bool off_env = getenv("ISHARA_NO_ATTN_BITS") != nullptr;
    return off_env ? nullptr : reinterpret_cast<uint32_t*>(m->W(off));
}
bool ln_as_prologue(int dt, int M, int N, int K, int ldt, const float* gamma, const float* beta, float eps, float* mean, float* rstd, void* xn, EpiArgs& ea) {
    EpiArgs probe = ea;
    probe.ln_gamma = gamma; probe.ln_beta = beta; probe.ln_mean = mean; probe.pro_out = xn;
    if (!gemm_nt_as_prologue_ok(dt, dt, dt, M, N, K, ldt, probe)) return false;
    ea.ln_gamma = gamma; ea.ln_beta = beta; ea.ln_eps = eps;
    ea.ln_mean = mean; ea.ln_rstd = rstd; ea.pro_out = xn;
    return true;
}

static const void* ln_prologue(ishara_model* m, const DenseW& w, const Run& r, const void* x, const Norm& ln, float eps, Buf xn, Buf mean, Buf rstd, EpiArgs& ea, int* rc) {
    *rc = 0;
    if (ln_as_prologue(m->dt, r.M, w.N, w.K, w.ldt, m->P(ln.gamma), m->P(ln.beta), eps, r.training ? m->Wf(mean) : nullptr, r.training ? m->Wf(rstd) : nullptr,
                       r.training ? m->W(xn) : nullptr, ea))
        return x;
    *rc = [&]() -> int {
        CKP(m, "layernorm_fwd", 2.0 * r.M * m->d * (double)dt_size(m->dt), 0, launch_layernorm_fwd(m->dt, x, m->P(ln.gamma), m->P(ln.beta), eps, m->W(xn), m->Wf(mean), m->Wf(rstd), r.M, m->d, m->s));
        return 0;
    }();
    return m->W(xn);
}

static int conv_fwd(ishara_model* m, ConvBlock& cb, const Run& r, const void* x) {
    const int d = m->d, c = 2 * d, B = r.B, T = m->T, dt = m->dt;
    OpArgs no; EpiArgs e1;
    CK(gemm_fwd(m, cb.W1, x, dt, m->W(cb.z1), dt, r.M, OP_NONE, no, e1));
    int prows = 0;
    const bool infer_fused = !r.training && getenv("ISHARA_NO_INFER_FUSION") == nullptr;
    static const bool no_train_fusion = getenv("ISHARA_NO_STATS_FUSION") != nullptr;
    const bool train_fused = r.training && !no_train_fusion;
    CKP(m, "dwconv_fwd", 3.0 * r.M * m->d * (double)dt_size(m->dt), 0, launch_dwconv_fwd(dt, DWIN_SWISH, m->W(cb.z1), m->P(cb.dw), nullptr, m->W(cb.h2), m->Wf(cb.ssum), m->Wf(cb.ssq), m->Wf(m->slab), B, T, c, cb.k, cb.k - 1, m->s,
                                                                                          (infer_fused || train_fused) ? &prows : nullptr));
    if (train_fused && prows > 0)
    CKP(m, "bn_finalize", 0, 0, launch_bn_finalize(m->Wf(m->slab), m->Wf(m->slab) + c, B * prows, (float)B * T, m->P(cb.bn.gamma), m->P(cb.bn.beta), 1e-3f, 0.95f,
                          m->P(cb.bn.mm), m->P(cb.bn.mv), r.training, m->Wf(cb.mean), m->Wf(cb.rstd), m->Wf(cb.a), m->Wf(cb.bsh), c, m->s, 1.f, 2 * c));
    else if (!(infer_fused && prows > 0))
    CKP(m, "bn_finalize", 0, 0, launch_bn_finalize(m->Wf(cb.ssum), m->Wf(cb.ssq), B, (float)B * T, m->P(cb.bn.gamma), m->P(cb.bn.beta), 1e-3f, 0.95f,
                          m->P(cb.bn.mm), m->P(cb.bn.mv), r.training, m->Wf(cb.mean), m->Wf(cb.rstd), m->Wf(cb.a), m->Wf(cb.bsh), c, m->s));
    const DropSpec ds = dspec(r, cb.site, m->cfg.dropout_rate);
    EpiArgs e2; e2.resid = x;
    cb.folded = false; cb.psa = false;
    if (ds.thr) {
        e2.rowscale = m->Wf(cb.rs); e2.T = T;
        EpiArgs probe = e2; probe.bias = m->P(cb.W2.b);
        cb.folded = dt == DT_BF16 && !g_force_regstage && gemm_nt_as_applicable(dt, r.M, cb.W2.N, cb.W2.K, cb.W2.ldt, probe) && gemm_nt_as_applicable(dt, r.M, cb.W2.K, cb.W2.N, cb.W2.ldn, probe) &&
                    gemm_tn_bias_rowscale_ok(dt, dt, dt, r.M, cb.W2.K, cb.W2.N, T);
        e2.rowscale_bias = cb.folded ? 1 : 0;
    }
    if (infer_fused && prows > 0)
        CKP(m, "eca_fwd", 0, 0, launch_eca_fwd_infer(m->Wf(m->slab), prows, m->P(cb.bn.mm), m->P(cb.bn.mv), m->P(cb.bn.gamma), m->P(cb.bn.beta), 1e-3f, m->P(cb.eca), 1.f / T,
                                                       m->Wf(cb.gn), m->Wf(cb.sg), m->Wf(cb.P), m->Wf(cb.Q), B, c, m->s));
    else if (train_fused && prows > 0)
        CKP(m, "eca_fwd", 0, 0, launch_eca_fwd_part(m->Wf(m->slab), prows, m->Wf(cb.ssum), m->Wf(cb.a), m->Wf(cb.bsh), m->P(cb.eca), 1.f / T, m->Wf(cb.gn), m->Wf(cb.sg), m->Wf(cb.P), m->Wf(cb.Q), B, c, m->s,
                                                      ds.thr ? m->Wf(cb.rs) : nullptr, ds, cb.folded ? 1 : 0));
    else
    CKP(m, "eca_fwd", 0, 0, launch_eca_fwd(m->Wf(cb.ssum), m->Wf(cb.a), m->Wf(cb.bsh), m->P(cb.eca), 1.f / T, m->Wf(cb.gn), m->Wf(cb.sg), m->Wf(cb.P), m->Wf(cb.Q), B, c, m->s, ds.thr ? m->Wf(cb.rs) : nullptr, ds, cb.folded ? 1 : 0));
    {
        EpiArgs probe = e2; probe.pa_P = m->Wf(cb.P); probe.pa_Q = m->Wf(cb.Q); probe.T = T; probe.bias = m->P(cb.W2.b);
        probe.pro_out = r.training ? m->W(cb.h4) : nullptr;
        if (gemm_nt_as_prologue_ok(dt, dt, dt, r.M, cb.W2.N, cb.W2.K, cb.W2.ldt, probe)) {
            cb.psa = r.training && m->psa_on && (!ds.thr || cb.folded) && gemm_tn_psa_ok(dt, dt, dt, r.M, cb.W2.K, cb.W2.N, T);
            e2.pa_P = m->Wf(cb.P); e2.pa_Q = m->Wf(cb.Q); e2.T = T; e2.pro_out = (r.training && !cb.psa) ? m->W(cb.h4) : nullptr;
            CK(gemm_fwd(m, cb.W2, m->W(cb.h2), dt, m->W(cb.out), dt, r.M, OP_NONE, no, e2));
            return 0;
        }
    }
    CKP(m, "sample_affine", 4.0 * r.M * m->d * (double)dt_size(m->dt), 0, launch_sample_affine(dt, m->W(cb.h2), m->Wf(cb.P), m->Wf(cb.Q), nullptr, m->W(cb.h4), B, T, c, m->s));
    CK(gemm_fwd(m, cb.W2, m->W(cb.h4), dt, m->W(cb.out), dt, r.M, OP_NONE, no, e2));
    return 0;
}

static int ffn_fwd(ishara_model* m, FFN& f, const Run& r, const void* x) {
    const int dt = m->dt;
    OpArgs no;
    EpiArgs ea; ea.pre_out = m->W(f.za); ea.act = ACT_SWISH; ea.drop = dspec(r, f.site_in, m->cfg.dropout_rate);
    int rc;
    const void* ain = ln_prologue(m, f.Wa, r, x, f.ln, f.eps, f.xn, f.mean, f.rstd, ea, &rc);
    CK(rc);
    CK(gemm_fwd(m, f.Wa, ain, dt, m->W(f.u), dt, r.M, OP_NONE, no, ea));
    EpiArgs eb; eb.resid = x;
    if (f.has_out_drop) eb.drop = dspec(r, f.site_out, m->cfg.dropout_rate);
    CK(gemm_fwd(m, f.Wb, m->W(f.u), dt, m->W(f.out), dt, r.M, OP_NONE, no, eb));
    return 0;
}

static int mhsa_fwd(ishara_model* m, MHSA& a, const Run& r, const void* x) {
    const int dt = m->dt;
    OpArgs no;
    EpiArgs eq; eq.mode = EPI_QKV; eq.q = m->W(a.q); eq.k = m->W(a.k); eq.vt = m->W(a.vt); eq.H = m->H; eq.dh = m->dh; eq.T = m->T; eq.head_major = 1;
    int rc;
    const void* ain = ln_prologue(m, a.Wqkv, r, x, a.ln, a.eps, a.xn, a.mean, a.rstd, eq, &rc);
    CK(rc);
    CK(gemm_fwd(m, a.Wqkv, ain, dt, nullptr, dt, r.M, OP_NONE, no, eq));
    const float scale = 1.0f / sqrtf((float)m->d);
    CKP(m, "attn_fwd", 4.0 * r.M * m->d * (double)dt_size(m->dt), 4.0 * r.B * m->H * (double)m->T * m->T * m->dh, launch_attn_fwd(dt, m->W(a.q), m->W(a.k), m->W(a.vt), m->W(a.o), m->Wf(a.lse), r.B, m->H, m->T, m->dh, scale,
                       dspec_attn(r, a.site_attn, a.rate), m->cfg.attn_impl, attn_maskw(m, a.maskw), m->s));
    EpiArgs ep; ep.resid = x;
    if (a.has_out_drop) ep.drop = dspec(r, a.site_out, m->cfg.dropout_rate);
    CK(gemm_fwd(m, a.Wp, m->W(a.o), dt, m->W(a.out), dt, r.M, OP_NONE, no, ep));
    return 0;
}

static int sqzconv_fwd(ishara_model* m, SqzConv& c, const Run& r, const void* x) {
    const int dt = m->dt, d = m->d, de = c.Wc1.N, B = r.B, T = m->T;
    OpArgs no; EpiArgs e0;
    EpiArgs e1;
    int rc;
    const void* ain = ln_prologue(m, c.Wc1, r, x, c.ln, 1e-6f, c.xn, c.mean, c.rstd, e1, &rc);
    CK(rc);
    CK(gemm_fwd(m, c.Wc1, ain, dt, m->W(c.zc), dt, r.M, OP_NONE, no, e1));
    CKP(m, "dwconv_fwd", 3.0 * r.M * m->d * (double)dt_size(m->dt), 0, launch_dwconv_fwd(dt, DWIN_SWISH, m->W(c.zc), m->P(c.dw), nullptr, m->W(c.zd), nullptr, nullptr, nullptr, B, T, de, c.k, c.k - 1, m->s));
    CKP(m, "map_rows", 2.0 * r.M * de * (double)dt_size(m->dt), 0, launch_map_rows(dt, MAP_SWISH, m->W(c.zd), m->W(c.hd), nullptr, DropSpec{0, 0, 1.f}, r.M, T, de, m->s));
    CK(gemm_fwd(m, c.Wc3, m->W(c.hd), dt, m->W(c.u3), dt, r.M, OP_NONE, no, e0));
    CKP(m, "sample_reduce", 2.0 * r.M * m->d * (double)dt_size(m->dt), 0, launch_sample_reduce(dt, m->W(c.u3), nullptr, nullptr, nullptr, m->Wf(c.gap), nullptr, B, T, d, m->s));
    CKP(m, "se_fwd", 0, 0, launch_se_fwd(m->Wf(c.gap), 1.f / T, m->P(c.seW1), m->P(c.seb1), m->P(c.seW2), m->P(c.seb2), m->Wf(c.hid), m->Wf(c.se), B, d, c.R, m->s));
    CKP(m, "sample_affine", 4.0 * r.M * m->d * (double)dt_size(m->dt), 0, launch_sample_affine(dt, m->W(c.u3), m->Wf(c.se), nullptr, x, m->W(c.out), B, T, d, m->s));
    return 0;
}

int confconv_fwd(ishara_model* m, ConfConv& c, const Run& r, const void* x) {
    const int dt = m->dt, d = m->d, B = r.B, T = m->T;
    OpArgs no; EpiArgs e0;
    CK(gemm_fwd(m, c.Wp1, x, dt, m->W(c.g), dt, r.M, OP_NONE, no, e0));
    int prows = 0;
    static const bool no_train_fusion = getenv("ISHARA_NO_STATS_FUSION") != nullptr;
    const bool train_fused = r.training && !no_train_fusion;
    CKP(m, "dwconv_fwd", 3.0 * r.M * m->d * (double)dt_size(m->dt), 0, launch_dwconv_fwd(dt, DWIN_GLU, m->W(c.g), m->P(c.dw), c.dwb >= 0 ? m->P(c.dwb) : nullptr, m->W(c.v), r.training ? m->Wf(c.ssum) : nullptr, r.training ? m->Wf(c.ssq) : nullptr, m->Wf(m->slab), B, T, d, c.k, (c.k - 1) / 2, m->s,
                                                                                          train_fused ? &prows : nullptr));
    const float var_corr = c.bn_unbiased && B * T > 1 ? (float)((double)B * T / ((double)B * T - 1.0)) : 1.f;
    if (train_fused && prows > 0)
    CKP(m, "bn_finalize", 0, 0, launch_bn_finalize(m->Wf(m->slab), m->Wf(m->slab) + d, B * prows, (float)B * T, m->P(c.bn.gamma), m->P(c.bn.beta), c.bn_eps, c.bn_keep,
                          m->P(c.bn.mm), m->P(c.bn.mv), r.training, m->Wf(c.mean), m->Wf(c.rstd), m->Wf(c.a), m->Wf(c.bsh), d, m->s, var_corr, 2 * d));
    else
    CKP(m, "bn_finalize", 0, 0, launch_bn_finalize(m->Wf(c.ssum), m->Wf(c.ssq), B, (float)B * T, m->P(c.bn.gamma), m->P(c.bn.beta), c.bn_eps, c.bn_keep,
                          m->P(c.bn.mm), m->P(c.bn.mv), r.training, m->Wf(c.mean), m->Wf(c.rstd), m->Wf(c.a), m->Wf(c.bsh), d, m->s, var_corr));
    CKP(m, "col_affine", 2.0 * r.M * d * (double)dt_size(m->dt), 0, launch_col_affine(dt, m->W(c.v), m->Wf(c.a), m->Wf(c.bsh), m->W(c.bnv), r.M, d, m->s));
    const void* pin = m->W(c.bnv);
    if (c.swish_after_bn) {
        CKP(m, "map_rows", 2.0 * r.M * d * (double)dt_size(m->dt), 0, launch_map_rows(dt, MAP_SWISH, m->W(c.bnv), m->W(c.sw), nullptr, DropSpec{0, 0, 1.f}, r.M, T, d, m->s));
        pin = m->W(c.sw);
    }
    EpiArgs e2; e2.resid = x;
    if (c.has_out_drop) e2.drop = dspec(r, c.site_out, m->cfg.dropout_rate);
    CK(gemm_fwd(m, c.Wp2, pin, dt, m->W(c.r), dt, r.M, OP_NONE, no, e2));
    CKP(m, "layernorm_fwd", 2.0 * r.M * m->d * (double)dt_size(m->dt), 0, launch_layernorm_fwd(dt, m->W(c.r), m->P(c.ln.gamma), m->P(c.ln.beta), c.ln_eps, m->W(c.out), m->Wf(c.lnmean), m->Wf(c.lnrstd), r.M, d, m->s));
    return 0;
}

int cls_route_auto(int dt, int M, int K, int C) {
    const bool fusion = getenv("ISHARA_NO_INFER_FUSION") == nullptr;
    if (dt_is16(dt) && M <= 1536 && C <= 64 && C % 4 == 0 && (K == 256 || K == 512) && !g_force_regstage && fusion) return CLS_AS;
    if (dt_is16(dt) && M <= 4096 && C <= 64 && K % 32 == 0 && fusion) return CLS_NARROW;
    return CLS_GEMM;
}
#define CKP_OPT(m, key, by, fl, expr) do { if (m) CKP(m, key, by, fl, expr); else CK(expr); } while (0)
int classifier_fwd(ishara_model* m, int route, int dt, const void* A, const void* Wt, int ldt, const float* bias, float* logits, int M, int K, int C, hipStream_t s) {
    if (route == CLS_AUTO) route = cls_route_auto(dt, M, K, C);
    OpArgs no; EpiArgs ec; ec.bias = bias;
    if (route == CLS_AS) {
        ec.ldc = C; ec.n_valid = C;
        CKP_OPT(m, "classifier(as)", 0, 2.0 * M * C * K, launch_gemm_nt(dt, dt, DT_F32, OP_NONE, A, Wt, logits, M, 64, K, ldt, no, ec, s));
    } else if (route == CLS_NARROW) {
        CKP_OPT(m, "dense_narrow", 0, 2.0 * M * C * K, launch_dense_narrow(dt, A, Wt, ldt, bias, logits, M, C, K, s));
    } else {
        const double by = (double)M * K * dt_size(dt) + (double)M * C * 4 + (double)K * C * dt_size(dt);
        CKP_OPT(m, gemm_nt_kernel_name(dt, dt, DT_F32, OP_NONE, A, M, C, K, ldt, ec), by, 2.0 * M * C * K, launch_gemm_nt(dt, dt, DT_F32, OP_NONE, A, Wt, logits, M, C, K, ldt, no, ec, s));
    }
    return 0;
}

static int stem_fwd(ishara_model* m, const Run& r, const float* x) {
    const int dt = m->dt, d = m->d, T = m->T, B = r.B, training = r.training;
    OpArgs no;
    EpiArgs es; es.addtab = m->Wf(m->pe); es.tab_period = T;
    if (m->stem_kp) {
        CKP(m, "pack_rows_bf16", (double)r.M * (m->F * 4.0 + m->stem_kp * 2.0), 0, launch_pack_rows_bf16(x, m->W(m->stem_xb), r.M, m->F, m->stem_kp, m->s, dt));
        DenseW wp = m->stemW; wp.K = m->stem_kp;
        CK(gemm_fwd(m, wp, m->W(m->stem_xb), dt, m->W(m->stem_h0), dt, r.M, OP_NONE, no, es));
    } else
        CK(gemm_fwd(m, m->stemW, x, DT_F32, m->W(m->stem_h0), dt, r.M, OP_NONE, no, es));
    if (training)
    CKP(m, "sample_reduce", 2.0 * r.M * m->d * (double)dt_size(m->dt), 0, launch_sample_reduce(dt, m->W(m->stem_h0), m->W(m->stem_h0), nullptr, nullptr, m->Wf(m->stem_ssum), m->Wf(m->stem_ssq), B, T, d, m->s));
    CKP(m, "bn_finalize", 0, 0, launch_bn_finalize(m->Wf(m->stem_ssum), m->Wf(m->stem_ssq), B, (float)B * T, m->P(m->stem_bn.gamma), m->P(m->stem_bn.beta), 1e-3f, 0.95f,
                          m->P(m->stem_bn.mm), m->P(m->stem_bn.mv), training, m->Wf(m->stem_mean), m->Wf(m->stem_rstd), m->Wf(m->stem_a), m->Wf(m->stem_bsh), d, m->s));
    CKP(m, "col_affine", 2.0 * r.M * m->d * (double)dt_size(m->dt), 0, launch_col_affine(dt, m->W(m->stem_h0), m->Wf(m->stem_a), m->Wf(m->stem_bsh), m->W(m->stem_out), r.M, d, m->s));
    return 0;
}
static int head_fwd(ishara_model* m, const Run& r, const void* h, float* logits) {
    const int dt = m->dt;
    OpArgs no;
    EpiArgs et; et.act = ACT_RELU; et.drop = dspec(r, m->head_site, m->cfg.head_dropout);
    CK(gemm_fwd(m, m->topW, h, dt, m->W(m->head_hh), dt, r.M, OP_NONE, no, et));
    CK(classifier_fwd(m, CLS_AUTO, dt, m->W(m->head_hh), m->ws + m->clsW.wt, m->clsW.ldt, m->clsW.b >= 0 ? m->P(m->clsW.b) : nullptr, logits, r.M, m->clsW.K, m->C, m->s));
    return 0;
}

extern "C" int ishara_forward(ishara_model* m, const float* x, int32_t B, float* logits, int32_t training, uint32_t seed, ishara_stream st) {
    if (!m->ws) { ishara_set_error("ishara_forward: model is not bound"); return -1; }
    if (m->family != ISHARA_FAMILY_KERAS_HYBRID) { ishara_set_error("ishara_forward: this handle is an encoder-only family; use ishara_encoder_forward"); return -1; }
    if (B <= 0 || B > m->Bmax) { ishara_set_error("ishara_forward: batch %d outside 1..%d", B, m->Bmax); return -1; }
    if (m->dt == DT_F16 && training) {
        ishara_set_error("ishara_forward: ISHARA_F16 is an inference-only storage type (the reference's fp16 is the TFLite export, c14:1-5; it reports NaNs when TRAINING in fp16)");
        return -1;
    }
    m->s = (hipStream_t)st;
    Run r{B, B * m->T, training, seed};
    CK(stem_fwd(m, r, x));
    const void* h = m->W(m->stem_out);
    for (const Layer& L : m->layers) {
        if (L.kind == Layer::CONV) { ConvBlock& cb = m->convs[L.idx]; CK(conv_fwd(m, cb, r, h)); h = m->W(cb.out); }
        else if (L.kind == Layer::SQZ) {
            SqzBlock& sb = m->sqz[L.idx];
            CK(ffn_fwd(m, sb.ffn1, r, h)); h = m->W(sb.ffn1.out);
            CK(mhsa_fwd(m, sb.mha, r, h)); h = m->W(sb.mha.out);
            CK(sqzconv_fwd(m, sb.conv, r, h)); h = m->W(sb.conv.out);
            CK(ffn_fwd(m, sb.ffn2, r, h)); h = m->W(sb.ffn2.out);
        } else {
            ConfBlock& cb = m->conf[L.idx];
            CK(ffn_fwd(m, cb.ffn1, r, h)); h = m->W(cb.ffn1.out);
            CK(mhsa_fwd(m, cb.mha, r, h)); h = m->W(cb.mha.out);
            CK(confconv_fwd(m, cb.conv, r, h)); h = m->W(cb.conv.out);
            CK(ffn_fwd(m, cb.ffn2, r, h)); h = m->W(cb.ffn2.out);
        }
    }
    CK(head_fwd(m, r, h, logits));
    m->lastB = B; m->last_training = training; m->last_seed = seed; m->last_x = x; m->probe_mod = -1;
    return 0;
}

static const void* layer_out(ishara_model* m, const Layer& L) {
    return L.kind == Layer::CONV ? m->W(m->convs[L.idx].out) : (L.kind == Layer::SQZ ? m->W(m->sqz[L.idx].ffn2.out) : m->W(m->conf[L.idx].ffn2.out));
}
static int conv_bwd(ishara_model* m, ConvBlock& cb, const Run& r, const void* x, const void* g, void* gn) {
    const int d = m->d, c = 2 * d, B = r.B, T = m->T, dt = m->dt;
    OpArgs no;
    const DropSpec ds = dspec(r, cb.site, m->cfg.dropout_rate);
    const void* gs = g;
    EpiArgs e1;
    if (cb.psa) {
        const float* rs = ds.thr ? m->Wf(cb.rs) : nullptr;
        if (rs) { e1.rowscale = rs; e1.T = T; }
        CK(gemm_dgrad(m, cb.W2, g, dt, m->W(m->t1), r.M, OP_NONE, no, e1));
        TnPsa ps; ps.P = m->Wf(cb.P); ps.Q = m->Wf(cb.Q); ps.W = m->ws + cb.W2.wn; ps.ldw = cb.W2.ldn; ps.G = m->Wf(m->psaG); ps.Rpart = m->Wf(m->psaR); ps.T = T;
        { static const int psa_dbg = getenv("ISHARA_PSA_DBG") ? atoi(getenv("ISHARA_PSA_DBG")) : 0; ps.dbg = psa_dbg; }
        CK(gemm_wgrad(m, cb.W2, m->W(cb.h2), dt, OP_NONE, no, g, dt, OP_NONE, no, r.M, 0, 0, rs, rs ? T : 0, &ps));
    } else if (ds.thr && cb.folded) {
        e1.rowscale = m->Wf(cb.rs); e1.T = T;
        CK(gemm_dgrad(m, cb.W2, g, dt, m->W(m->t1), r.M, OP_NONE, no, e1));
        CK(gemm_wgrad(m, cb.W2, m->W(cb.h4), dt, OP_NONE, no, g, dt, OP_NONE, no, r.M, 0, 0, m->Wf(cb.rs), T));
    } else {
        if (ds.thr) {
            CKP(m, "map_rows", 2.0 * r.M * d * (double)dt_size(m->dt), 0, launch_map_rows(dt, MAP_ROWSCALE, g, m->W(m->t3), m->Wf(cb.rs), ds, r.M, T, d, m->s));
            gs = m->W(m->t3);
        }
        CK(gemm_dgrad(m, cb.W2, gs, dt, m->W(m->t1), r.M, OP_NONE, no, e1));
        CK(gemm_wgrad(m, cb.W2, m->W(cb.h4), dt, OP_NONE, no, gs, dt, OP_NONE, no, r.M));
    }
    if (!cb.psa) CKP(m, "sample_reduce", 2.0 * r.M * m->d * (double)dt_size(m->dt), 0, launch_sample_reduce(dt, m->W(m->t1), m->W(cb.h2), m->Wf(cb.mean), m->Wf(cb.rstd), m->Wf(m->S1), m->Wf(m->S2), B, T, c, m->s));
    PsaStats pst;
    if (cb.psa) { pst.G = m->Wf(m->psaG); pst.Rpart = m->Wf(m->psaR); pst.nparts = cb.W2.N / 64; pst.Wt = m->ws + cb.W2.wt; pst.ldt = cb.W2.ldt; pst.N = cb.W2.N;
                  pst.rs = ds.thr ? m->Wf(cb.rs) : nullptr; pst.mean = m->Wf(cb.mean); pst.rstd = m->Wf(cb.rstd); }
    CKP(m, "eca_bn_bwd_finalize", 0, 0, launch_eca_bn_bwd_finalize(m->Wf(m->S1), m->Wf(m->S2), m->Wf(cb.ssum), m->Wf(cb.gn), m->Wf(cb.sg), m->P(cb.eca), m->P(cb.bn.gamma), m->P(cb.bn.beta),
                                  m->Wf(cb.mean), m->Wf(cb.rstd), m->G(cb.bn.gamma), m->G(cb.bn.beta), m->G(cb.eca), m->Wf(m->E), m->Wf(m->Fc), m->Wf(m->ecap), B, T, c, m->s, cb.psa ? &pst : nullptr));
    DwBnArgs bn; bn.h = m->W(cb.h2); bn.mean = m->Wf(cb.mean); bn.rstd = m->Wf(cb.rstd); bn.a = m->Wf(cb.a); bn.sg = m->Wf(cb.sg); bn.E = m->Wf(m->E); bn.Fc = m->Wf(m->Fc); bn.e_per_sample = 1;
    const int fused = dwconv_bwd_deferred(m, r, 10.0, DWIN_SWISH, m->W(m->t1), &bn, m->W(cb.z1), cb.dw, -1, m->W(m->t2), c, cb.k, cb.k - 1);
    if (fused < 0) return fused;
    if (!fused) {
        CKP(m, "bn_bwd_apply", 6.0 * r.M * m->d * (double)dt_size(m->dt), 0, launch_bn_bwd_apply(dt, m->W(m->t1), m->W(cb.h2), m->Wf(cb.mean), m->Wf(cb.rstd), m->Wf(cb.a), m->Wf(cb.sg), m->Wf(m->E), 1, m->Wf(m->Fc), m->W(m->t1), B, T, c, m->s));
        CK(dwconv_bwd_deferred(m, r, 8.0, DWIN_SWISH, m->W(m->t1), nullptr, m->W(cb.z1), cb.dw, -1, m->W(m->t2), c, cb.k, cb.k - 1));
    }
    EpiArgs e2; e2.resid = g;
    CK(gemm_dgrad(m, cb.W1, m->W(m->t2), dt, gn, r.M, OP_NONE, no, e2));
    CK(gemm_wgrad(m, cb.W1, x, dt, OP_NONE, no, m->W(m->t2), dt, OP_NONE, no, r.M));
    return 0;
}

static int ffn_bwd(ishara_model* m, FFN& f, const Run& r, const void* x, const void* g, void* gn) {
    const int dt = m->dt;
    OpArgs no;
    int rc = 0;
    const void* gs = f.has_out_drop ? grad_through_dropout(m, r, f.site_out, m->cfg.dropout_rate, g, m->W(m->t3), m->T, m->d, &rc) : g;
    CK(rc);
    EpiArgs e1; e1.drop = dspec(r, f.site_in, m->cfg.dropout_rate); e1.dact = DACT_SWISH; e1.aux = m->W(f.za);
    CK(gemm_dgrad(m, f.Wb, gs, dt, m->W(m->t1), r.M, OP_NONE, no, e1));
    CK(gemm_wgrad(m, f.Wb, m->W(f.u), dt, OP_NONE, no, gs, dt, OP_NONE, no, r.M));
    EpiArgs e0;
    CK(gemm_dgrad(m, f.Wa, m->W(m->t1), dt, m->W(m->t2), r.M, OP_NONE, no, e0));
    CK(gemm_wgrad(m, f.Wa, m->W(f.xn), dt, OP_NONE, no, m->W(m->t1), dt, OP_NONE, no, r.M));
    return layernorm_bwd_deferred(m, r, m->W(m->t2), x, f.mean, f.rstd, f.ln, g, gn);
}

static int mhsa_bwd(ishara_model* m, MHSA& a, const Run& r, const void* x, const void* g, void* gn) {
    const int dt = m->dt;
    OpArgs no; EpiArgs e0;
    int rc = 0;
    const void* gs = a.has_out_drop ? grad_through_dropout(m, r, a.site_out, m->cfg.dropout_rate, g, m->W(m->t3), m->T, m->d, &rc) : g;
    CK(rc);
    CK(gemm_dgrad(m, a.Wp, gs, dt, m->W(m->t1), r.M, OP_NONE, no, e0));
    CK(gemm_wgrad(m, a.Wp, m->W(a.o), dt, OP_NONE, no, gs, dt, OP_NONE, no, r.M));
    const float scale = 1.0f / sqrtf((float)m->d);
    CKP(m, "attn_bwd", 8.0 * r.M * m->d * (double)dt_size(m->dt), 10.0 * r.B * m->H * (double)m->T * m->T * m->dh, launch_attn_bwd(dt, m->W(a.q), m->W(a.k), m->W(a.vt), m->W(a.o), m->W(m->t1), m->Wf(a.lse), m->Wf(m->delta), m->W(m->t2),
                       r.B, m->H, m->T, m->dh, scale, dspec_attn(r, a.site_attn, a.rate), 1, m->cfg.attn_impl, attn_maskw(m, a.maskw), m->s));
    CK(gemm_dgrad(m, a.Wqkv, m->W(m->t2), dt, m->W(m->t1), r.M, OP_NONE, no, e0));
    CK(gemm_wgrad(m, a.Wqkv, m->W(a.xn), dt, OP_NONE, no, m->W(m->t2), dt, OP_NONE, no, r.M));
    return layernorm_bwd_deferred(m, r, m->W(m->t1), x, a.mean, a.rstd, a.ln, g, gn);
}

static int sqzconv_bwd(ishara_model* m, SqzConv& c, const Run& r, const void* x, const void* g, void* gn) {
    const int dt = m->dt, d = m->d, de = c.Wc1.N, B = r.B, T = m->T;
    OpArgs no; EpiArgs e0;
    CKP(m, "sample_reduce", 2.0 * r.M * m->d * (double)dt_size(m->dt), 0, launch_sample_reduce(dt, g, m->W(c.u3), nullptr, nullptr, m->Wf(m->S1), m->Wf(m->dse), B, T, d, m->s));
    CKP(m, "se_bwd", 0, 0, launch_se_bwd(m->Wf(m->dse), m->Wf(c.gap), 1.f / T, m->P(c.seW1), m->P(c.seW2), m->Wf(c.hid), m->Wf(c.se),
                     m->G(c.seW1), m->G(c.seb1), m->G(c.seW2), m->G(c.seb2), m->Wf(m->dgapT), m->Wf(m->E), B, d, c.R, m->s));
    CKP(m, "sample_affine", 4.0 * r.M * m->d * (double)dt_size(m->dt), 0, launch_sample_affine(dt, g, m->Wf(c.se), m->Wf(m->dgapT), nullptr, m->W(m->t1), B, T, d, m->s));
    EpiArgs e1; e1.dact = DACT_SWISH; e1.aux = m->W(c.zd);
    CK(gemm_dgrad(m, c.Wc3, m->W(m->t1), dt, m->W(m->t2), r.M, OP_NONE, no, e1));
    CK(gemm_wgrad(m, c.Wc3, m->W(c.hd), dt, OP_NONE, no, m->W(m->t1), dt, OP_NONE, no, r.M));
    CK(dwconv_bwd_deferred(m, r, 8.0, DWIN_SWISH, m->W(m->t2), nullptr, m->W(c.zc), c.dw, -1, m->W(m->t1), de, c.k, c.k - 1));
    CK(gemm_dgrad(m, c.Wc1, m->W(m->t1), dt, m->W(m->t2), r.M, OP_NONE, no, e0));
    CK(gemm_wgrad(m, c.Wc1, m->W(c.xn), dt, OP_NONE, no, m->W(m->t1), dt, OP_NONE, no, r.M));
    return layernorm_bwd_deferred(m, r, m->W(m->t2), x, c.mean, c.rstd, c.ln, g, gn);
}

int confconv_bwd(ishara_model* m, ConfConv& c, const Run& r, const void* x, const void* g, void* gn) {
    const int dt = m->dt, d = m->d, B = r.B, T = m->T;
    OpArgs no;
    CK(layernorm_bwd_deferred(m, r, g, m->W(c.r), c.lnmean, c.lnrstd, c.ln, nullptr, m->W(m->t1)));
    int rc = 0;
    const void* gs = c.has_out_drop ? grad_through_dropout(m, r, c.site_out, m->cfg.dropout_rate, m->W(m->t1), m->W(m->t3), T, d, &rc) : m->W(m->t1);
    CK(rc);
    EpiArgs es; if (c.swish_after_bn) { es.dact = DACT_SWISH; es.aux = m->W(c.bnv); }
    CK(gemm_dgrad(m, c.Wp2, gs, dt, m->W(m->t2), r.M, OP_NONE, no, es));
    CK(gemm_wgrad(m, c.Wp2, c.swish_after_bn ? m->W(c.sw) : m->W(c.bnv), dt, OP_NONE, no, gs, dt, OP_NONE, no, r.M));
    CKP(m, "sample_reduce", 2.0 * r.M * m->d * (double)dt_size(m->dt), 0, launch_sample_reduce(dt, m->W(m->t2), m->W(c.v), m->Wf(c.mean), m->Wf(c.rstd), m->Wf(m->S1), m->Wf(m->S2), B, T, d, m->s));
    CKP(m, "bn_bwd_finalize", 0, 0, launch_bn_bwd_finalize(m->Wf(m->S1), m->Wf(m->S2), m->G(c.bn.gamma), m->G(c.bn.beta), m->Wf(m->Ecol), m->Wf(m->Fc), B, T, d, m->s));
    DwBnArgs bn; bn.h = m->W(c.v); bn.mean = m->Wf(c.mean); bn.rstd = m->Wf(c.rstd); bn.a = m->Wf(c.a); bn.E = m->Wf(m->Ecol); bn.Fc = m->Wf(m->Fc);
    const int fused = dwconv_bwd_deferred(m, r, 6.0, DWIN_GLU, m->W(m->t2), &bn, m->W(c.g), c.dw, c.dwb, m->W(m->t3), d, c.k, (c.k - 1) / 2);
    if (fused < 0) return fused;
    if (!fused) {
        CKP(m, "bn_bwd_apply", 6.0 * r.M * m->d * (double)dt_size(m->dt), 0, launch_bn_bwd_apply(dt, m->W(m->t2), m->W(c.v), m->Wf(c.mean), m->Wf(c.rstd), m->Wf(c.a), nullptr, m->Wf(m->Ecol), 0, m->Wf(m->Fc), m->W(m->t2), B, T, d, m->s));
        CK(dwconv_bwd_deferred(m, r, 8.0, DWIN_GLU, m->W(m->t2), nullptr, m->W(c.g), c.dw, c.dwb, m->W(m->t3), d, c.k, (c.k - 1) / 2));
    }
    EpiArgs e2; e2.resid = m->W(m->t1);
    CK(gemm_dgrad(m, c.Wp1, m->W(m->t3), dt, gn, r.M, OP_NONE, no, e2));
    CK(gemm_wgrad(m, c.Wp1, x, dt, OP_NONE, no, m->W(m->t3), dt, OP_NONE, no, r.M));
    return 0;
}

static int head_bwd(ishara_model* m, const Run& r, const void* hin, void* g) {
    const int dt = m->dt;
    OpArgs no; EpiArgs e0;
    EpiArgs eh; eh.drop = dspec(r, m->head_site, m->cfg.head_dropout); eh.dact = DACT_POS; eh.aux = m->W(m->head_hh);
    if (m->cls_pad && r.M % 64 == 0 && r.M >= 256 && m->clsW.K % 128 == 0 && !g_force_tn_regstage) {
        DenseW wp = m->clsW; wp.N = m->cls_pad;
        CK(gemm_dgrad(m, wp, m->W(m->dlb), dt, m->W(m->t1), r.M, OP_NONE, no, eh));
        CK(gemm_wgrad(m, wp, m->W(m->head_hh), dt, OP_NONE, no, m->W(m->dlb), dt, OP_NONE, no, r.M, 0, m->C));
    } else {
        CK(gemm_dgrad(m, m->clsW, m->Wf(m->dlogits), DT_F32, m->W(m->t1), r.M, OP_NONE, no, eh));
        CK(gemm_wgrad(m, m->clsW, m->W(m->head_hh), dt, OP_NONE, no, m->Wf(m->dlogits), DT_F32, OP_NONE, no, r.M));
    }
    CK(gemm_dgrad(m, m->topW, m->W(m->t1), dt, g, r.M, OP_NONE, no, e0));
    CK(gemm_wgrad(m, m->topW, hin, dt, OP_NONE, no, m->W(m->t1), dt, OP_NONE, no, r.M));
    return 0;
}
static int stem_bwd(ishara_model* m, const Run& r, const void* g) {
    const int dt = m->dt, d = m->d, T = m->T, B = r.B;
    OpArgs no;
    CKP(m, "sample_reduce", 2.0 * r.M * m->d * (double)dt_size(m->dt), 0, launch_sample_reduce(dt, g, m->W(m->stem_h0), m->Wf(m->stem_mean), m->Wf(m->stem_rstd), m->Wf(m->S1), m->Wf(m->S2), B, T, d, m->s));
    CKP(m, "bn_bwd_finalize", 0, 0, launch_bn_bwd_finalize(m->Wf(m->S1), m->Wf(m->S2), m->G(m->stem_bn.gamma), m->G(m->stem_bn.beta), m->Wf(m->Ecol), m->Wf(m->Fc), B, T, d, m->s));
    CKP(m, "bn_bwd_apply", 6.0 * r.M * m->d * (double)dt_size(m->dt), 0, launch_bn_bwd_apply(dt, g, m->W(m->stem_h0), m->Wf(m->stem_mean), m->Wf(m->stem_rstd), m->Wf(m->stem_a), nullptr, m->Wf(m->Ecol), 0, m->Wf(m->Fc), m->W(m->t1), B, T, d, m->s));
    if (m->stem_kp && r.M % 64 == 0 && r.M >= 256 && d % 128 == 0 && !g_force_tn_regstage) {
        DenseW wp = m->stemW; wp.K = m->stem_kp;
        CK(gemm_wgrad(m, wp, m->W(m->stem_xb), dt, OP_NONE, no, m->W(m->t1), dt, OP_NONE, no, r.M, m->F));
    } else
        CK(gemm_wgrad(m, m->stemW, m->last_x, DT_F32, OP_NONE, no, m->W(m->t1), dt, OP_NONE, no, r.M));
    return 0;
}

extern "C" int ishara_loss_backward(ishara_model* m, const float* logits, const int64_t* labels, int32_t B, float* loss, float* nll, float loss_scale, ishara_stream st) {
    if (!m->ws || !m->grads) { ishara_set_error("ishara_loss_backward: model is not bound (grads required)"); return -1; }
    if (m->family != ISHARA_FAMILY_KERAS_HYBRID) { ishara_set_error("ishara_loss_backward: this handle is an encoder-only family; use ishara_encoder_backward"); return -1; }
    if (B != m->lastB || !m->last_training) { ishara_set_error("ishara_loss_backward: call ishara_forward(training=1) with the same batch first"); return -1; }
    m->s = (hipStream_t)st;
    m->red.njobs = 0; m->red.nblocks = 0; m->red_off = 0; g_red_sink = nullptr;
    m->tn_defer.pending = false;
    Run r{B, B * m->T, 1, m->last_seed};
    const int T = m->T;
    float* nl = nll ? nll : m->Wf(m->nllb);
    CK(launch_fill_u32(m->grads, (size_t)m->n_train, 0u, m->s));
    CKP(m, "ctc", 2.0 * r.M * m->C * 4, 0, launch_ctc(logits, labels, B, T, m->C, m->L, m->C - 1, nl, m->Wf(m->dlogits), loss_scale / (float)B, m->Wf(m->ctcws), m->s, m->cls_pad ? m->W(m->dlb) : nullptr));
    if (loss) CKP(m, "mean", 0, 0, launch_mean(nl, loss, B, 1.f / (float)B, m->s));
    const void* hin = m->layers.empty() ? m->W(m->stem_out) : layer_out(m, m->layers.back());
    void* g = m->W(m->gA); void* gn = m->W(m->gB);
    CK(head_bwd(m, r, hin, g));
    for (int li = (int)m->layers.size() - 1; li >= 0; --li) {
        const Layer& L = m->layers[li];
        const void* lin = li > 0 ? layer_out(m, m->layers[li - 1]) : m->W(m->stem_out);
#define STEP(call) do { CK(call); void* _t = g; g = gn; gn = _t; } while (0)
        if (L.kind == Layer::CONV) { STEP(conv_bwd(m, m->convs[L.idx], r, lin, g, gn)); }
        else if (L.kind == Layer::SQZ) {
            SqzBlock& sb = m->sqz[L.idx];
            STEP(ffn_bwd(m, sb.ffn2, r, m->W(sb.conv.out), g, gn));
            STEP(sqzconv_bwd(m, sb.conv, r, m->W(sb.mha.out), g, gn));
            STEP(mhsa_bwd(m, sb.mha, r, m->W(sb.ffn1.out), g, gn));
            STEP(ffn_bwd(m, sb.ffn1, r, lin, g, gn));
        } else {
            ConfBlock& cb = m->conf[L.idx];
            STEP(ffn_bwd(m, cb.ffn2, r, m->W(cb.conv.out), g, gn));
            STEP(confconv_bwd(m, cb.conv, r, m->W(cb.mha.out), g, gn));
            STEP(mhsa_bwd(m, cb.mha, r, m->W(cb.ffn1.out), g, gn));
            STEP(ffn_bwd(m, cb.ffn1, r, lin, g, gn));
        }
#undef STEP
        if (!m->bucket_ev.empty() && m->bucket_after_layer[li] >= 0) { CK(wgrad_flush(m)); CK(red_flush(m)); HIP_CHECK_RET(hipEventRecord(m->bucket_ev[m->bucket_after_layer[li]], m->s)); }
    }
    CK(stem_bwd(m, r, g));
    CK(wgrad_flush(m));
    CK(red_flush(m));
    if (!m->bucket_ev.empty()) HIP_CHECK_RET(hipEventRecord(m->bucket_ev.back(), m->s));
    return 0;
}

struct ProbeMod {
    enum Kind { STEM, CONV, FFN_, MHSA_, SQZCONV, CONFCONV, HEAD } kind;
    std::string name; int in_cols, out_cols; uint32_t first_site, n_sites;
    void* ptr;
    Buf in, out;
};
static std::vector<ProbeMod> probe_modules(ishara_model* m) {
    std::vector<ProbeMod> v;
    uint32_t site = 0;
    Buf prev = m->stem_out;
    auto add = [&](ProbeMod::Kind k, const std::string& name, int in_cols, int out_cols, uint32_t n_sites, void* ptr, Buf out) {
        v.push_back(ProbeMod{k, name, in_cols, out_cols, site, n_sites, ptr, prev, out});
        site += n_sites; prev = out;
    };
    const int d = m->d;
    add(ProbeMod::STEM, "stem", m->F, d, 0, nullptr, m->stem_out);
    for (const Layer& L : m->layers) {
        if (L.kind == Layer::CONV) {
// ... 133 lines not shown
```

### ishara_amd/csrc/kernels.h

```cpp
#pragma once
#include "common.h"
#include "../../include/ishara_hip.h"

enum DType : int { DT_F32 = 0, DT_BF16 = 1, DT_F16 = 2 };
static inline size_t dt_size(int dt) { return dt == DT_F32 ? 4 : 2; }
static inline bool dt_is16(int dt) { return dt != DT_F32; }

enum : int { OP_NONE = 0, OP_SWISH = 1, OP_COLAFFINE = 2, OP_ROWSCALE = 3, OP_DROPMASK = 4 };
struct OpArgs {
    const float* c1 = nullptr;
    const float* c0 = nullptr;
    const float* rs = nullptr;
    int T = 1;
    DropSpec drop = {0, 0, 1.f};
};

enum : int { ACT_NONE = 0, ACT_SWISH = 1, ACT_RELU = 2 };
enum : int { DACT_NONE = 0, DACT_SWISH = 1, DACT_POS = 2 };
enum : int { EPI_STD = 0, EPI_QKV = 1 };
struct EpiArgs {
    const float* bias = nullptr;
    const float* addtab = nullptr;
    int tab_period = 1;
    void* pre_out = nullptr;
    int act = ACT_NONE;
    DropSpec drop = {0, 0, 1.f};
    const float* rowscale = nullptr;
    int T = 1;
    int rowscale_bias = 0;
    int dact = DACT_NONE;
    const void* aux = nullptr;
    const void* resid = nullptr;
    int mode = EPI_STD;
    void* q = nullptr; void* k = nullptr; void* vt = nullptr;
    int H = 1, dh = 1;
    int dbg = 0;
    const float* ln_gamma = nullptr;
    const float* ln_beta = nullptr;
    float ln_eps = 0.f;
    float* ln_mean = nullptr;
    float* ln_rstd = nullptr;
    const float* pa_P = nullptr;
    const float* pa_Q = nullptr;
    void* pro_out = nullptr;
    int head_major = 1;
    int ldc = 0, n_valid = 0;
    int as_flags = -1;
};

int launch_gemm_nt(int dtA, int dtM, int dtC, int op, const void* A, const void* Bt, void* C,
                   int M, int N, int K, int ldb, const OpArgs& oa, const EpiArgs& ea, hipStream_t s);

size_t gemm_tn_slab_floats(int M, int Ka, int Nb, int dtM);
#define RED_MAXJOBS 48
struct RedJob { const float* slab; float* out0; float* out1; size_t stride; int n0, n, splits, nb, nbv, first_block; };
struct RedSink { RedJob job[RED_MAXJOBS]; int njobs = 0; int nblocks = 0; };
extern RedSink* g_red_sink;
bool reduce_sink_full();
int launch_reduce_flush(RedSink* sink, hipStream_t s);
bool gemm_tn_bias_rowscale_ok(int dtA, int dtB, int dtM, int M, int Ka, int Nb, int T);
struct TnDefer { float* slab[2] = {nullptr, nullptr}; int turn = 0; bool pending = false;
                 const float* p_slab = nullptr; float* p_out0 = nullptr; float* p_out1 = nullptr; int p_n0 = 0, p_n = 0, p_splits = 0; size_t p_stride = 0; int p_nb = 0, p_nbv = 0; };
int launch_gemm_tn_flush(TnDefer* defer, hipStream_t s);
struct TnPsa { const float* P = nullptr; const float* Q = nullptr;
               const void* W = nullptr; int ldw = 0;
               float* G = nullptr; float* Rpart = nullptr; int T = 0;
               int dbg = 0; };
bool gemm_tn_psa_ok(int dtA, int dtB, int dtM, int M, int Ka, int Nb, int T);
int launch_gemm_tn(int dtA, int dtB, int dtM, int opA, int opB, const void* A, const void* B,
                   float* out, float* dbias, float* slab, int M, int Ka, int Nb,
                   const OpArgs& oa, const OpArgs& ob, hipStream_t s, int ka_valid = 0, int nb_valid = 0,
                   const float* bias_rowscale = nullptr, int bias_T = 0, TnDefer* defer = nullptr, const TnPsa* psa = nullptr);
int launch_dense_narrow(int dt, const void* A, const void* Wt, int ldt, const float* bias, float* C, int M, int N, int K, hipStream_t s);
int launch_pack_rows_bf16(const float* x, void* xb, int M, int F, int Kp, hipStream_t s, int dt = DT_BF16);

bool gemm_nt_as_applicable(int dtC, int M, int N, int K, int ldb, const EpiArgs& ea);
bool gemm_nt_as_prologue_ok(int dtA, int dtM, int dtC, int M, int N, int K, int ldb, const EpiArgs& ea);
const char* gemm_nt_kernel_name(int dtA, int dtM, int dtC, int op, const void* A, int M, int N, int K, int ldb, const EpiArgs& ea);
extern int g_force_tn_regstage;
extern int g_force_regstage, g_dbg_tn, g_force_dw_lds, g_tn_blocks, g_attn_bwd_two_pass, g_as_flags_override, g_nt_big;
extern int g_tn_phase;
const char* gemm_tn_kernel_name(int dtA, int dtB, int dtM, int opA, int opB, int M, int Ka, int Nb, bool brs = false);

int launch_make_shadow(int dtM, const float* W, int K, int N, void* Wt, int ldt, void* Wn, int ldn, hipStream_t s);
struct ShadowDesc { const float* W; void* Wt; void* Wn; int K, N, ldt, ldn, tile0, tiles_n; };
int launch_make_shadow_batched(int dtM, const ShadowDesc* tab, int ntab, int total_tiles, hipStream_t s);

int launch_log_softmax_fwd(const float* x, float* y, int M, int C, int ld, hipStream_t s);
int launch_log_softmax_bwd(const float* dy, const float* y, float* dx, int M, int C, int ld, hipStream_t s);
int launch_layernorm_fwd(int dt, const void* x, const float* gamma, const float* beta, float eps,
                         void* y, float* mean, float* rstd, int M, int C, hipStream_t s);
size_t layernorm_bwd_scratch_floats(int C);
int launch_layernorm_bwd(int dt, const void* dy, const void* x, const float* mean, const float* rstd,
                         const float* gamma, const void* resid, void* dx, float* dgamma, float* dbeta,
                         float* scratch, int M, int C, hipStream_t s);

enum : int { DWIN_NONE = 0, DWIN_SWISH = 1, DWIN_GLU = 2 };
int launch_dwconv_fwd(int dt, int inop, const void* x, const float* w, const float* bias, void* y,
                      float* ssum, float* ssq, float* part, int B, int T, int C, int k, int padl, hipStream_t s, int* part_rows = nullptr);
size_t dwconv_fwd_scratch_floats(int B, int T, int C);
size_t dwconv_bwd_scratch_floats(int C, int k);
struct DwBnArgs { const void* h = nullptr; const float* mean = nullptr; const float* rstd = nullptr; const float* a = nullptr;
                  const float* sg = nullptr; const float* E = nullptr; const float* Fc = nullptr; int e_per_sample = 0; };
int launch_dwconv_bwd_bn(int dt, int inop, const void* dy, const DwBnArgs& bn, const void* x, const float* w, void* dx,
                         float* dw, float* dbias, float* scratch, int B, int T, int C, int k, int padl, hipStream_t s);
int launch_dwconv_bwd(int dt, int inop, const void* dy, const void* x, const float* w, void* dx,
                      float* dw, float* dbias, float* scratch, int B, int T, int C, int k, int padl, hipStream_t s);

int launch_bn_finalize(const float* ssum, const float* ssq, int nb, float count, const float* gamma, const float* beta,
                       float eps, float momentum, float* moving_mean, float* moving_var, int training,
                       float* mean, float* rstd, float* a, float* b, int C, hipStream_t s, float var_corr = 1.f, int stride = 0);
int launch_eca_fwd(const float* gap, const float* a, const float* b, const float* w5, float invT,
                   float* gn, float* sgate, float* P, float* Q, int B, int C, hipStream_t s, float* rs = nullptr, DropSpec dp = {0, 0, 1.f}, int dp_fold = 0);
int launch_eca_fwd_part(const float* part, int prows, float* gap_out, const float* a, const float* b, const float* w5, float invT,
                        float* gn, float* sgate, float* P, float* Q, int B, int C, hipStream_t s, float* rs = nullptr, DropSpec dp = {0, 0, 1.f}, int dp_fold = 0);
int launch_eca_fwd_infer(const float* part, int prows, const float* mm, const float* mv, const float* gamma, const float* beta, float eps, const float* w5, float invT,
                         float* gn, float* sgate, float* P, float* Q, int B, int C, hipStream_t s);
int launch_sample_affine(int dt, const void* x, const float* P, const float* Q, const void* resid, void* y,
                         int B, int T, int C, hipStream_t s);
int launch_col_affine(int dt, const void* x, const float* a, const float* b, void* y, int M, int C, hipStream_t s);
enum : int { MAP_SWISH = 0, MAP_ROWSCALE = 1, MAP_DROPMASK = 2 };
int launch_map_rows(int dt, int op, const void* x, void* y, const float* rs, DropSpec drop, int M, int T, int C, hipStream_t s);
int launch_sample_reduce(int dt, const void* dy, const void* other, const float* mean, const float* rstd,
                         float* S1, float* S2, int B, int T, int C, hipStream_t s);
#define ECA_MAX_CHUNKS 4
struct PsaStats { const float* G = nullptr; const float* Rpart = nullptr; int nparts = 0; const void* Wt = nullptr; int ldt = 0, N = 0;
                  const float* rs = nullptr; const float* mean = nullptr; const float* rstd = nullptr; };
int launch_eca_bn_bwd_finalize(float* S1, float* S2, const float* gap, const float* gn, const float* sgate,
                               const float* w5, const float* gamma, const float* beta, const float* mean, const float* rstd,
                               float* dgamma, float* dbeta, float* dw5, float* E, float* Fc, float* dw5part , int B, int T, int C, hipStream_t s,
                               const PsaStats* ps = nullptr);
int launch_bn_bwd_finalize(const float* S1, const float* S2, float* dgamma, float* dbeta, float* Ecol, float* Fc,
                           int B, int T, int C, hipStream_t s);
int launch_bn_bwd_apply(int dt, const void* dy, const void* x, const float* mean, const float* rstd, const float* a,
                        const float* sg, const float* E, int e_per_sample, const float* Fc, void* dx,
                        int B, int T, int C, hipStream_t s);
int launch_se_fwd(const float* gap, float invT, const float* W1, const float* b1, const float* W2, const float* b2,
                  float* hid_pre, float* se, int B, int C, int R, hipStream_t s);
int launch_se_bwd(const float* dse, const float* gap, float invT, const float* W1, const float* W2,
                  const float* hid_pre, const float* se, float* dW1, float* db1, float* dW2, float* db2,
                  float* dgapT, float* scr , int B, int C, int R, hipStream_t s);

size_t attn_mask_words(int B, int H, int T);
int launch_attn_fwd(int dt, const void* q, const void* k, const void* vt, void* o, float* lse,
                    int B, int H, int T, int dh, float scale, DropSpec drop, int impl, uint32_t* maskbits, hipStream_t s);
int launch_attn_bwd(int dt, const void* q, const void* k, const void* vt, const void* o, const void* dout,
                    const float* lse, float* delta, void* dqkv, int B, int H, int T, int dh, float scale,
                    DropSpec drop, int head_major, int impl, uint32_t* maskbits, hipStream_t s);

size_t ctc_workspace_floats(int B, int T, int L);
size_t ctc_lds_bytes(int T, int L);
size_t ctc_lds_limit();
int launch_ctc(const float* logits, const int64_t* labels, int B, int T, int C, int L, int blank,
               float* nll, float* dlogits, float grad_scale, float* ws, hipStream_t s, void* dlb = nullptr);
int launch_fill_u32(void* p, size_t n_words, uint32_t v, hipStream_t s);
int launch_mean(const float* v, float* out, int n, float scale, hipStream_t s);
int launch_greedy_decode(const float* logits, int B, int T, int C, int blank, int* out_idx, int* out_len, hipStream_t s);

int launch_preprocess(const float* raw, const int* n_frames, int max_frames, const float* mean, const float* stdv, float* out, int T, hipStream_t s);
int launch_preprocess_batch(const float* raw, int64_t n_total, const int64_t* offsets, int B, int max_frames, const float* mean, const float* stdv,
                            float* out, int T, hipStream_t s);
#define SCORE_MAX_L 64
int launch_edit_distance(const int* out_idx, const int* out_len, int B, int T, const int* targets, int L, int* dist, int* tlen, hipStream_t s);
__host__ __device__ size_t ctc_beam_workspace_words(int T, int W);
int launch_ctc_beam(const float* logits, int B, int T, int C, int blank, int W, int nbest, const float* lm, float alpha, float beta,
                    void* ws, int* out_idx, int* out_len, float* out_score, hipStream_t s);
bool ctc_align_bp_in_lds(int T, int L);
size_t ctc_align_workspace_bytes(int B, int T, int L);
int launch_ctc_align(const float* logits, const int64_t* labels, int B, int T, int C, int L, int blank, void* ws, int* frame_pos, int* start,
                     int* end, float* conf, float* score, hipStream_t s);
#define CLIP_MAX_T 4096
int launch_clip_batch(const float* raw, const ishara_clip_aug* clips, int B, int T, int layout, float* x, hipStream_t s);

struct RAdamArgs { float lr, wd, beta1, beta2, eps, c1, c2, r_t; int rect; int sync; float slow_step; };
int launch_radam_lookahead(float* theta, const float* grad, float* m, float* v, float* slow, int64_t n,
                           RAdamArgs a, hipStream_t s);
int launch_scale(float* x, int64_t n, float scale, hipStream_t s);
```

Baseline: 6.856 million frames/s.

## Fuse FFN up and down projections into one A-stationary GEMM kernel

Adds a fused feed-forward kernel that runs the LayerNorm prologue, the first GEMM with swish, dropout and pre-activation output, and then the second GEMM with dropout and residual, all in one launch per row chunk. The backward dgrad pair (through Wb, then dswish, then Wa) uses the same kernel. The intent is to keep the intermediate activation on chip instead of writing and rereading it between two launches, and to save launch overhead. The default AS flags now enable the path (bit 64). It adds standalone op entry points and refactors the prologue and epilogue into helpers. The risk is register and LDS pressure, which can lower occupancy.

```diff
diff --git a/include/ishara_hip.h b/include/ishara_hip.h
--- a/include/ishara_hip.h
+++ b/include/ishara_hip.h
@@ -136,6 +136,12 @@
 int64_t ishara_op_qkv_scratch_bytes(int32_t B, int32_t T, int32_t H, int32_t dh);
 int ishara_op_qkv_fwd(int32_t dt, const void* x, const float* gamma, const float* beta, float eps, const float* W, const float* bias,
                       void* q, void* k, void* vt, int32_t B, int32_t T, int32_t H, int32_t dh, int32_t head_major, void* scratch, ishara_stream s);
+int64_t ishara_ffn_op_scratch_bytes(int32_t M, int32_t K1, int32_t N1, int32_t N2);
+int ishara_ffn_op_fwd(int32_t dt, const void* x, const float* gamma, const float* beta, float eps, const float* Wa, const float* ba, const float* Wb, const float* bb,
+                      uint32_t seed, uint32_t site_in, float rate_in, uint32_t site_out, float rate_out,
+                      void* xn, float* mean, float* rstd, void* za, void* u, void* out, int32_t M, int32_t K1, int32_t N1, int32_t N2, void* scratch, ishara_stream s);
+int ishara_ffn_op_dgrad(int32_t dt, const void* gs, const void* za, const float* Wa, const float* Wb, uint32_t seed, uint32_t site_in, float rate_in,
+                        void* t1, void* t2, int32_t M, int32_t K1, int32_t N1, int32_t N2, void* scratch, ishara_stream s);
 int ishara_op_classifier_fwd(int32_t dt, const void* x, const float* W, const float* bias, float* logits, int32_t M, int32_t K, int32_t C,
                              int32_t route, void* scratch, ishara_stream s);
 int ishara_op_ctc_loss(const float* logits, const int64_t* labels, int32_t B, int32_t T, int32_t C, int32_t L, int32_t blank,
diff --git a/ishara_amd/_lib.py b/ishara_amd/_lib.py
--- a/ishara_amd/_lib.py
+++ b/ishara_amd/_lib.py
@@ -90,6 +90,9 @@
     "ishara_op_dense_fwd": (C.c_int, [_I32, _P, _P, _P, _P, _I32, _I32, _I32, _I32, _P, _P]),
     "ishara_op_dense_fwd_ex": (C.c_int, [_I32, _P, _P, _P, _P, _P, _I32, _I32, _I32, _I32, _P, _P]),
     "ishara_op_dense_bwd": (C.c_int, [_I32, _P, _P, _P, _P, _P, _P, _I32, _I32, _I32, _P, _P]),
+    "ishara_ffn_op_scratch_bytes": (_I64, [_I32, _I32, _I32, _I32]),
+    "ishara_ffn_op_fwd": (C.c_int, [_I32, _P, _P, _P, _F, _P, _P, _P, _P, _U32, _U32, _F, _U32, _F, _P, _P, _P, _P, _P, _P, _I32, _I32, _I32, _I32, _P, _P]),
+    "ishara_ffn_op_dgrad": (C.c_int, [_I32, _P, _P, _P, _P, _U32, _U32, _F, _P, _P, _I32, _I32, _I32, _I32, _P, _P]),
     "ishara_op_qkv_scratch_bytes": (_I64, [_I32, _I32, _I32, _I32]),
     "ishara_op_qkv_fwd": (C.c_int, [_I32, _P, _P, _P, _F, _P, _P, _P, _P, _P, _I32, _I32, _I32, _I32, _I32, _P, _P]),
     "ishara_op_classifier_fwd": (C.c_int, [_I32, _P, _P, _P, _P, _I32, _I32, _I32, _I32, _P, _P]),
diff --git a/ishara_amd/csrc/api_ops.hip b/ishara_amd/csrc/api_ops.hip
--- a/ishara_amd/csrc/api_ops.hip
+++ b/ishara_amd/csrc/api_ops.hip
@@ -231,6 +231,77 @@
     }
     eq.bias = bias;
     return launch_gemm_nt(dt, dt, dt, OP_NONE, A, sc + sh.wt, nullptr, M, 3 * d, d, sh.ldt, no, eq, s);
+}
+struct FfnShadows {
+    OpShadow a, b; size_t boff;
+    FfnShadows(int K1, int N1, int N2, int M) : a(DT_BF16, K1, N1, M), b(DT_BF16, N1, N2, M), boff(rup(a.slab, 256)) {}
+    size_t total() const { return boff + b.slab; }
+};
+static bool ffn_op_ok(const char* me, int dt, int M, int K1, int N1, int N2) {
+    if (!op_dt_ok(me, dt, false)) return false;
+    if (dt != DT_BF16) { ishara_set_error("%s: ISHARA_BF16 only (dt=%d): the feed-forward pair is a training path of the bf16 model", me, dt); return false; }
+    if (M < 1 || K1 < 8 || N1 < 8 || N2 < 8 || K1 > 4096 || N1 > 4096 || N2 > 4096 || (K1 | N1 | N2) % 8 != 0) {
+        ishara_set_error("%s: bad shape M=%d K1=%d N1=%d N2=%d (M >= 1; K1, N1, N2 multiples of 8 in 8..4096)", me, M, K1, N1, N2); return false;
+    }
+    return true;
+}
+extern "C" int64_t ishara_ffn_op_scratch_bytes(int32_t M, int32_t K1, int32_t N1, int32_t N2) {
+    if (M < 1 || K1 < 1 || N1 < 1 || N2 < 1) return -1;
+    return (int64_t)FfnShadows(K1, N1, N2, M).total();
+}
+extern "C" int ishara_ffn_op_fwd(int32_t dt, const void* x, const float* gamma, const float* beta, float eps, const float* Wa, const float* ba, const float* Wb, const float* bb,
+                                 uint32_t seed, uint32_t site_in, float rate_in, uint32_t site_out, float rate_out,
+                                 void* xn, float* mean, float* rstd, void* za, void* u, void* out, int32_t M, int32_t K1, int32_t N1, int32_t N2, void* scratch, ishara_stream st) {
+    const char* me = "ishara_ffn_op_fwd";
+    if (!ffn_op_ok(me, dt, M, K1, N1, N2)) return -1;
+    if (!(rate_in >= 0.f && rate_in < 1.f) || !(rate_out >= 0.f && rate_out < 1.f)) { ishara_set_error("%s: dropout rates must lie in [0, 1)", me); return -1; }
+    if (K1 != N2) { ishara_set_error("%s: the residual needs N2 == K1 (K1=%d N2=%d)", me, K1, N2); return -1; }
+    if (!x || !gamma || !beta || !Wa || !Wb || !xn || !mean || !rstd || !za || !u || !out || !scratch || ((uintptr_t)x | (uintptr_t)scratch) % 16 != 0) {
+        ishara_set_error("%s: null or misaligned buffer (x, scratch: 16-byte aligned; ba, bb may be NULL)", me); return -1;
+    }
+    hipStream_t s = (hipStream_t)st;
+    const FfnShadows sh(K1, N1, N2, M);
+    char* sa = (char*)scratch; char* sb = sa + sh.boff;
+    EpiArgs ea; ea.pre_out = za; ea.act = ACT_SWISH; ea.drop = make_drop(seed, site_in, rate_in, true); ea.bias = ba;
+    EpiArgs eb; eb.resid = x; eb.drop = make_drop(seed, site_out, rate_out, true); eb.bias = bb;
+    const bool fused = (gemm_nt_as_flags() & 64) != 0;
+    if (!ln_as_prologue(dt, M, N1, K1, sh.a.ldt, gamma, beta, eps, mean, rstd, xn, ea)) {
+        ishara_set_error("%s: M=%d K1=%d N1=%d: the A-stationary kernel does not take this shape with the LayerNorm prologue%s", me, M, K1, N1, g_force_regstage ? " (switched off: ishara_debug_force_regstage)" : ""); return -1;
+    }
+    if (fused && !gemm_nt_as_ffn_ok(dt, x, M, K1, N1, N2, sh.a.ldt, sh.b.ldt, ea, eb)) {
+        ishara_set_error("%s: M=%d K1=%d N1=%d N2=%d: the FFN kernel takes K1 = 256, N1 = 512, N2 = 256 and M >= %d (as_flags bit 7 lifts the row bound) only", me, M, K1, N1, N2, 128 * 384); return -1;
+    }
+    CK(sh.a.build(dt, Wa, K1, N1, sa, s));
+    CK(sh.b.build(dt, Wb, N1, N2, sb, s));
+    if (fused) return launch_gemm_nt_as_ffn(dt, x, sa + sh.a.wt, sh.a.ldt, sb + sh.b.wt, sh.b.ldt, u, out, M, K1, N1, N2, ea, eb, s);
+    OpArgs no;
+    CK(launch_gemm_nt(dt, dt, dt, OP_NONE, x, sa + sh.a.wt, u, M, N1, K1, sh.a.ldt, no, ea, s));
+    return launch_gemm_nt(dt, dt, dt, OP_NONE, u, sb + sh.b.wt, out, M, N2, N1, sh.b.ldt, no, eb, s);
+}
+extern "C" int ishara_ffn_op_dgrad(int32_t dt, const void* gs, const void* za, const float* Wa, const float* Wb, uint32_t seed, uint32_t site_in, float rate_in,
+                                   void* t1, void* t2, int32_t M, int32_t K1, int32_t N1, int32_t N2, void* scratch, ishara_stream st) {
+    const char* me = "ishara_ffn_op_dgrad";
+    if (!ffn_op_ok(me, dt, M, K1, N1, N2)) return -1;
+    if (!(rate_in >= 0.f && rate_in < 1.f)) { ishara_set_error("%s: the dropout rate must lie in [0, 1)", me); return -1; }
+    if (!gs || !za || !Wa || !Wb || !t1 || !t2 || !scratch || ((uintptr_t)gs | (uintptr_t)scratch) % 16 != 0) {
+        ishara_set_error("%s: null or misaligned buffer (gs, scratch: 16-byte aligned)", me); return -1;
+    }
+    hipStream_t s = (hipStream_t)st;
+    const FfnShadows sh(K1, N1, N2, M);
+    char* sa = (char*)scratch; char* sb = sa + sh.boff;
+    EpiArgs e1; e1.drop = make_drop(seed, site_in, rate_in, true); e1.dact = DACT_SWISH; e1.aux = za;
+    EpiArgs e0;
+    const bool fused = (gemm_nt_as_flags() & 64) != 0;
+    if (fused && !gemm_nt_as_ffn_ok(dt, gs, M, N2, N1, K1, sh.b.ldn, sh.a.ldn, e1, e0)) {
+        ishara_set_error("%s: M=%d K1=%d N1=%d N2=%d: the FFN kernel takes K1 = 256, N1 = 512, N2 = 256 and M >= %d (as_flags bit 7 lifts the row bound) only%s", me, M, K1, N1, N2, 128 * 384,
+                         g_force_regstage ? "; the A-stationary kernels are switched off (ishara_debug_force_regstage)" : ""); return -1;
+    }
+    CK(sh.a.build(dt, Wa, K1, N1, sa, s));
+    CK(sh.b.build(dt, Wb, N1, N2, sb, s));
+    if (fused) return launch_gemm_nt_as_ffn(dt, gs, sb + sh.b.wn, sh.b.ldn, sa + sh.a.wn, sh.a.ldn, t1, t2, M, N2, N1, K1, e1, e0, s);
+    OpArgs no;
+    CK(launch_gemm_nt(dt, dt, dt, OP_NONE, gs, sb + sh.b.wn, t1, M, N1, N2, sh.b.ldn, no, e1, s));
+    return launch_gemm_nt(dt, dt, dt, OP_NONE, t1, sa + sh.a.wn, t2, M, K1, N1, sh.a.ldn, no, e0, s);
 }
 extern "C" int ishara_op_classifier_fwd(int32_t dt, const void* x, const float* Wm, const float* bias, float* logits, int32_t M, int32_t K, int32_t C,
                                         int32_t route, void* scratch, ishara_stream st) {
diff --git a/ishara_amd/csrc/gemm_as.hip b/ishara_amd/csrc/gemm_as.hip
--- a/ishara_amd/csrc/gemm_as.hip
+++ b/ishara_amd/csrc/gemm_as.hip
@@ -66,6 +66,116 @@
     if constexpr ((MASK & F) == 0) return false;
     else if constexpr (MASK == AS_ALL) return runtime;
     else return true;
+}
+
+DEVI void as_epi_head(float (&v)[8], const f32x4& acc0, const f32x4& acc1, const float (&bias)[8], float bsc) {
+#pragma unroll
+    for (int e = 0; e < 4; ++e) { v[e] = acc0[e] + bias[e] * bsc; v[4 + e] = acc1[e] + bias[4 + e] * bsc; }
+}
+template <typename TC, int GW>
+DEVI void as_epi_tail(float (&v)[GW], const EpiArgs& ea, bool f_act, bool f_drop, bool f_rowscale, bool f_dact, bool f_resid, uint32_t rk, uint32_t n, float rsc,
+                      const as_u32x4& au, const as_u32x4& rs) {
+    if (f_act) {
+        if (ea.act == ACT_SWISH) {
+#pragma unroll
+            for (int e = 0; e < GW; ++e) v[e] = swishf_(v[e]);
+        } else {
+#pragma unroll
+            for (int e = 0; e < GW; ++e) v[e] = fmaxf(v[e], 0.f);
+        }
+    }
+    if (f_drop) {
+        rng_apply<GW>(rk, n, ea.drop.thr, ea.drop.scale, v);
+    }
+    if (f_rowscale) {
+#pragma unroll
+        for (int e = 0; e < GW; ++e) v[e] *= rsc;
+    }
+    if (f_dact) {
+        float x[GW];
+        as_unpack<TC, GW>(au, x);
+        if (ea.dact == DACT_SWISH) {
+#pragma unroll
+            for (int e = 0; e < GW; ++e) v[e] *= dswishf_(x[e]);
+        } else {
+#pragma unroll
+            for (int e = 0; e < GW; ++e) v[e] = x[e] > 0.f ? v[e] : 0.f;
+        }
+    }
+    if (f_resid) {
+        float x[GW];
+        as_unpack<TC, GW>(rs, x);
+#pragma unroll
+        for (int e = 0; e < GW; ++e) v[e] += x[e];
+    }
+}
+
+template <int KT, int RT, int PRO, int NW>
+DEVI void as_prologue(as_v8 (&a)[RT][KT], float* cs, int M, const EpiArgs& ea, int m_base, int mw) {
+    constexpr int K = KT * 32;
+    const int tid = threadIdx.x, lane = tid & 63, c = lane & 15, g = lane >> 4;
+    const int bsm = min(m_base, M - 1) / ea.T;
+    const float* c0 = PRO == 1 ? ea.ln_gamma : ea.pa_P + (size_t)bsm * K;
+    const float* c1 = PRO == 1 ? ea.ln_beta : ea.pa_Q + (size_t)bsm * K;
+    for (int x = tid; x < K; x += NW * 64) { cs[x] = c0[x]; cs[K + x] = c1[x]; }
+    __syncthreads();
+    auto unpack = [&](const as_v8& f, float (&v)[8]) {
+        as_u32x4 t = __builtin_bit_cast(as_u32x4, f);
+        asm volatile("" : "+v"(t));
+        as_unpack<as_t, 8>(t, v);
+    };
+    float mean[RT], rstd[RT];
+#pragma unroll
+    for (int i = 0; i < RT; ++i) { mean[i] = 0.f; rstd[i] = 1.f; }
+    if constexpr (PRO == 1) {
+#pragma unroll
+        for (int i = 0; i < RT; ++i) {
+            float s = 0.f;
+#pragma unroll
+            for (int kt = 0; kt < KT; ++kt) {
+                float v[8];
+                unpack(a[i][kt], v);
+#pragma unroll
+                for (int e = 0; e < 8; ++e) s += v[e];
+            }
+            s += __shfl_xor(s, 16, 64); s += __shfl_xor(s, 32, 64);
+            mean[i] = s * (1.f / K);
+            float q = 0.f;
+#pragma unroll
+            for (int kt = 0; kt < KT; ++kt) {
+                float v[8];
+                unpack(a[i][kt], v);
+#pragma unroll
+                for (int e = 0; e < 8; ++e) { const float dlt = v[e] - mean[i]; q += dlt * dlt; }
+            }
+            q += __shfl_xor(q, 16, 64); q += __shfl_xor(q, 32, 64);
+            rstd[i] = rsqrtf(q * (1.f / K) + ea.ln_eps);
+            const int m = mw + 16 * i + c;
+            if (g == 0 && m < M && ea.ln_mean && blockIdx.y == 0) { ea.ln_mean[m] = mean[i]; ea.ln_rstd[m] = rstd[i]; }
+        }
+    }
+#pragma unroll
+    for (int kt = 0; kt < KT; ++kt) {
+        float wv[8], bv[8];
+        {
+            const float* cp = cs + 32 * kt + 8 * g;
+            asm volatile("" : "+v"(cp));
+            const f32x4 w0 = *reinterpret_cast<const f32x4*>(cp), w1 = *reinterpret_cast<const f32x4*>(cp + 4);
+            const f32x4 b0 = *reinterpret_cast<const f32x4*>(cp + K), b1 = *reinterpret_cast<const f32x4*>(cp + K + 4);
+#pragma unroll
+            for (int e = 0; e < 4; ++e) { wv[e] = w0[e]; wv[4 + e] = w1[e]; bv[e] = b0[e]; bv[4 + e] = b1[e]; }
+        }
+#pragma unroll
+        for (int i = 0; i < RT; ++i) {
+            float v[8];
+            unpack(a[i][kt], v);
+            as_v8 t;
+#pragma unroll
+            for (int e = 0; e < 8; ++e) t[e] = (as_t)(PRO == 1 ? (v[e] - mean[i]) * rstd[i] * wv[e] + bv[e] : v[e] * wv[e] + bv[e]);
+            a[i][kt] = t;
+        }
+    }
+    __syncthreads();
 }
 
 template <typename TC, int KT, int MASK, int RT, int DBG, int PRO, int NW = 4, int CS = 1>
@@ -134,71 +244,7 @@
         for (int kt = 0; kt < KT; ++kt) a[i][kt] = p[kt * 4];
     }
 
-    if constexpr (PRO != 0) {
-        float* cs = reinterpret_cast<float*>(smem + (R - 1) * STAGE);
-        const int bsm = min(m_base, M - 1) / ea.T;
-        const float* c0 = PRO == 1 ? ea.ln_gamma : ea.pa_P + (size_t)bsm * K;
-        const float* c1 = PRO == 1 ? ea.ln_beta : ea.pa_Q + (size_t)bsm * K;
-        for (int x = tid; x < K; x += NW * 64) { cs[x] = c0[x]; cs[K + x] = c1[x]; }
-        __syncthreads();
-        auto unpack = [&](const as_v8& f, float (&v)[8]) {
-            as_u32x4 t = __builtin_bit_cast(as_u32x4, f);
-            asm volatile("" : "+v"(t));
-            as_unpack<as_t, 8>(t, v);
-        };
-        float mean[RT], rstd[RT];
-#pragma unroll
-        for (int i = 0; i < RT; ++i) { mean[i] = 0.f; rstd[i] = 1.f; }
-        if constexpr (PRO == 1) {
-#pragma unroll
-            for (int i = 0; i < RT; ++i) {
-                float s = 0.f;
-#pragma unroll
-                for (int kt = 0; kt < KT; ++kt) {
-                    float v[8];
-                    unpack(a[i][kt], v);
-#pragma unroll
-                    for (int e = 0; e < 8; ++e) s += v[e];
-                }
-                s += __shfl_xor(s, 16, 64); s += __shfl_xor(s, 32, 64);
-                mean[i] = s * (1.f / K);
-                float q = 0.f;
-#pragma unroll
-                for (int kt = 0; kt < KT; ++kt) {
-                    float v[8];
-                    unpack(a[i][kt], v);
-#pragma unroll
-                    for (int e = 0; e < 8; ++e) { const float dlt = v[e] - mean[i]; q += dlt * dlt; }
-                }
-                q += __shfl_xor(q, 16, 64); q += __shfl_xor(q, 32, 64);
-                rstd[i] = rsqrtf(q * (1.f / K) + ea.ln_eps);
-                const int m = mw + 16 * i + c;
-                if (g == 0 && m < M && ea.ln_mean && blockIdx.y == 0) { ea.ln_mean[m] = mean[i]; ea.ln_rstd[m] = rstd[i]; }
-            }
-        }
-#pragma unroll
-        for (int kt = 0; kt < KT; ++kt) {
-            float wv[8], bv[8];
-            {
-                const float* cp = cs + 32 * kt + 8 * g;
-                asm volatile("" : "+v"(cp));
-                const f32x4 w0 = *reinterpret_cast<const f32x4*>(cp), w1 = *reinterpret_cast<const f32x4*>(cp + 4);
-                const f32x4 b0 = *reinterpret_cast<const f32x4*>(cp + K), b1 = *reinterpret_cast<const f32x4*>(cp + K + 4);
-#pragma unroll
-                for (int e = 0; e < 4; ++e) { wv[e] = w0[e]; wv[4 + e] = w1[e]; bv[e] = b0[e]; bv[4 + e] = b1[e]; }
-            }
-#pragma unroll
-            for (int i = 0; i < RT; ++i) {
-                float v[8];
-                unpack(a[i][kt], v);
-                as_v8 t;
-#pragma unroll
-                for (int e = 0; e < 8; ++e) t[e] = (as_t)(PRO == 1 ? (v[e] - mean[i]) * rstd[i] * wv[e] + bv[e] : v[e] * wv[e] + bv[e]);
-                a[i][kt] = t;
-            }
-        }
-        __syncthreads();
-    }
+    if constexpr (PRO != 0) as_prologue<KT, RT, PRO, NW>(a, reinterpret_cast<float*>(smem + (R - 1) * STAGE), M, ea, m_base, mw);
 
     const int frow = PAIR ? 8 * (c >> 2) + (c & 3) : c;
     const int sx = g ^ as_swz(frow);
@@ -329,10 +375,8 @@
                 const size_t off = eoff[i] + n0 + 4 * GW * q;
                 float v[GW];
                 const float bsc = (f_rowscale && ea.rowscale_bias) ? rsc[i] : 1.f;
-                if constexpr (PAIR) {
-#pragma unroll
-                    for (int e = 0; e < 4; ++e) { v[e] = acc[0][i][e] + bias[e] * bsc; v[4 + e] = acc[1][i][e] + bias[4 + e] * bsc; }
-                } else {
+                if constexpr (PAIR) as_epi_head(v, acc[0][i], acc[1][i], bias, bsc);
+                else {
 #pragma unroll
                     for (int e = 0; e < 4; ++e) v[e] = acc[q][i][e] + bias[e] * bsc;
                 }
@@ -359,39 +403,7 @@
                         } else as_st_nt<GW>(reinterpret_cast<TC*>(ea.pre_out) + off, v, nt_side);
                     } else as_st_nt<GW>(reinterpret_cast<TC*>(ea.pre_out) + off, v, nt_side);
                 }
-                if (f_act) {
-                    if (ea.act == ACT_SWISH) {
-#pragma unroll
-                        for (int e = 0; e < GW; ++e) v[e] = swishf_(v[e]);
-                    } else {
-#pragma unroll
-                        for (int e = 0; e < GW; ++e) v[e] = fmaxf(v[e], 0.f);
-                    }
-                }
-                if (f_drop) {
-                    rng_apply<GW>(rk[i], (uint32_t)n, ea.drop.thr, ea.drop.scale, v);
-                }
-                if (f_rowscale && !ea.rowscale_bias) {
-#pragma unroll
-                    for (int e = 0; e < GW; ++e) v[e] *= rsc[i];
-                }
-                if (f_dact) {
-                    float x[GW];
-                    as_unpack<TC, GW>(au[i][q], x);
-                    if (ea.dact == DACT_SWISH) {
-#pragma unroll
-                        for (int e = 0; e < GW; ++e) v[e] *= dswishf_(x[e]);
-                    } else {
-#pragma unroll
-                        for (int e = 0; e < GW; ++e) v[e] = x[e] > 0.f ? v[e] : 0.f;
-                    }
-                }
-                if (f_resid) {
-                    float x[GW];
-                    as_unpack<TC, GW>(rs[i][q], x);
-#pragma unroll
-                    for (int e = 0; e < GW; ++e) v[e] += x[e];
-                }
+                as_epi_tail<TC, GW>(v, ea, f_act, f_drop, f_rowscale && !ea.rowscale_bias, f_dact, f_resid, rk[i], (uint32_t)n, rsc[i], au[i][q], rs[i][q]);
                 if (!f_qkv) {
                     if constexpr (HOLDABLE) {
                         if (hold) {
@@ -490,6 +502,218 @@
     done[key] = ok;
     return ok;
 }
+
+#ifndef AS_F16
+#define AS_FFN_NW 8
+#define AS_FFN_ROWS (AS_FFN_NW * 16)
+#define AS_FFN_LDS (2 * 65536 + (512 + 256) * 4)
+DEVI int as_swz2(int r) { return ((r >> 1) & 1) | (((r >> 3) & 1) << 1); }
+
+template <int EM1, int EM2, int PRO>
+DEVI void as_ffn_pass(const as_t* __restrict__ A, const as_t* __restrict__ B1, int ldb1, const as_t* __restrict__ B2, int ldb2, as_t* __restrict__ C1, as_t* __restrict__ C2,
+                      int M, const EpiArgs& e1, const EpiArgs& e2, char* smem, const float* bias1_s, const float* bias2_s, int m_base) {
+    constexpr int KT = 8, RB = KT * 64, NS = AS_NS, K1 = 256, N1 = 512, N2 = 256;
+    constexpr int SUB = NS * RB;
+    constexpr int STEP = 2 * SUB, STAGE = 2 * STEP;
+    constexpr int NW = AS_FFN_NW, DPW = STAGE / 1024 / NW;
+    constexpr int NSTAGES = N1 / NS / 2;
+    constexpr int OPS1 = (EM1 & AS_PREOUT) ? 2 : 1;
+    constexpr bool FWD = (EM1 & AS_ACT) != 0;
+    const bool hold = (e1.as_flags & 1) != 0;
+    const bool nt_side = (e1.as_flags & 2) != 0;
+    const int tid = threadIdx.x, lane = tid & 63;
+    const int wid = __builtin_amdgcn_readfirstlane(tid >> 6);
+    const int c = lane & 15, g = lane >> 4;
+    const int mw = m_base + wid * 16;
+    const bool full = m_base + AS_FFN_ROWS <= M;
+    const bool f_drop1 = (EM1 & AS_DROP) != 0, f_drop2 = (EM2 & AS_DROP) != 0;
+
+    const as_t* bsrc[DPW];
+    const bool slice = (wid >> 1) & 1;
+    const int sub_w = wid >> 2;
+#pragma unroll
+    for (int t = 0; t < DPW; ++t) {
+        const int o = (((wid & 1) * DPW + t) << 10) + lane * 16;
+        if (!slice) { const int r = o / RB, p = (o % RB) >> 4; bsrc[t] = B1 + (size_t)(NS * sub_w + r) * ldb1 + ((p ^ as_swz(r)) << 3); }
+        else { const int r = o >> 6, p = (o >> 4) & 3; bsrc[t] = B2 + (size_t)r * ldb2 + NS * sub_w + ((p ^ as_swz2(r)) << 3); }
+    }
+    const size_t bstep = slice ? (size_t)2 * NS : (size_t)2 * NS * ldb1;
+    auto issue = [&](int slot) {
+#pragma unroll
+        for (int t = 0; t < DPW; ++t) {
+            __builtin_amdgcn_global_load_lds((const __attribute__((address_space(1))) void*)bsrc[t],
+                                             (__attribute__((address_space(3))) void*)(smem + slot + (wid * DPW + t) * 1024), 16, 0, 0);
+            bsrc[t] += bstep;
+        }
+    };
+    issue(0);
+
+    as_v8 a[1][KT];
+    const int mrow = min(mw + c, M - 1);
+    const int m = mw + c;
+    {
+        const as_v8* p = reinterpret_cast<const as_v8*>(A + (size_t)mrow * K1 + g * 8);
+#pragma unroll
+        for (int kt = 0; kt < KT; ++kt) a[0][kt] = p[kt * 4];
+    }
+    if constexpr (PRO != 0) as_prologue<KT, 1, PRO, NW>(a, reinterpret_cast<float*>(smem + STAGE), M, e1, m_base, mw);
+
+    const int frow = 8 * (c >> 2) + (c & 3);
+    const int sx = g ^ as_swz(frow);
+    const int off_e = frow * RB + ((sx & 3) << 4) + ((sx >> 2) << 6);
+    const int off_o = frow * RB + ((sx & 3) << 4) + (((sx >> 2) ^ 1) << 6);
+    const int off2 = SUB + frow * 64 + ((g ^ as_swz2(frow)) << 4);
+
+    uint32_t rk1 = 0u, rk2 = 0u;
+    if (f_drop1) rk1 = rng_row_key(e1.drop.key, (uint32_t)m);
+    if (f_drop2) rk2 = rng_row_key(e2.drop.key, (uint32_t)m);
+    const size_t eoff1 = (size_t)mrow * N1 + 8 * g, eoff2 = (size_t)mrow * N2 + 8 * g;
+    const as_t* aux = reinterpret_cast<const as_t*>(e1.aux);
+    const bool st_ok = full || m < M;
+
+#pragma unroll
+    for (int kt = 0; kt < KT; ++kt) {
+        as_u32x4 t = __builtin_bit_cast(as_u32x4, a[0][kt]);
+        asm volatile("" : "+v"(t));
+        a[0][kt] = __builtin_bit_cast(as_v8, t);
+    }
+
+    f32x4 acc2[N2 / 32][2];
+#pragma unroll
+    for (int t2 = 0; t2 < N2 / 32; ++t2) { acc2[t2][0] = f32x4{0.f, 0.f, 0.f, 0.f}; acc2[t2][1] = f32x4{0.f, 0.f, 0.f, 0.f}; }
+    as_v8 held = as_v8{}, held_pre = as_v8{};
+    as_u32x4 au_next[2] = {as_u32x4{}, as_u32x4{}};
+    if constexpr ((EM1 & AS_DACT) != 0) {
+#pragma unroll
+        for (int sub = 0; sub < 2; ++sub) au_next[sub] = __builtin_nontemporal_load(reinterpret_cast<const as_u32x4*>(aux + eoff1 + sub * NS));
+    }
+    int slot = 0;
+    for (int sg = 0; sg < NSTAGES; ++sg) {
+        if (full && sg >= 1) as_wait_vm<2 * OPS1>(); else as_wait_vm<0>();
+        asm volatile("s_waitcnt lgkmcnt(0)" ::: "memory");
+        __builtin_amdgcn_s_barrier();
+        as_u32x4 au_cur[2] = {au_next[0], au_next[1]};
+        if (sg + 1 < NSTAGES) {
+            if constexpr ((EM1 & AS_DACT) != 0) {
+#pragma unroll
+                for (int sub = 0; sub < 2; ++sub) au_next[sub] = __builtin_nontemporal_load(reinterpret_cast<const as_u32x4*>(aux + eoff1 + (2 * sg + 2 + sub) * NS));
+                __builtin_amdgcn_sched_barrier(0);
+            }
+            issue(slot ^ STAGE);
+            __builtin_amdgcn_sched_barrier(0);
+        }
+#pragma unroll
+        for (int sub = 0; sub < 2; ++sub) {
+            const int n0 = (2 * sg + sub) * NS;
+            const as_u32x4 au = au_cur[sub], none = as_u32x4{};
+            f32x4 acc[2] = {f32x4{0.f, 0.f, 0.f, 0.f}, f32x4{0.f, 0.f, 0.f, 0.f}};
+            const char* st = smem + slot + sub * STEP;
+#pragma unroll
+            for (int kt = 0; kt < KT; ++kt) {
+#pragma unroll
+                for (int j = 0; j < 2; ++j) {
+                    const as_v8 b = *reinterpret_cast<const as_v8*>(st + ((kt & 1) ? off_o : off_e) + (kt >> 1) * 128 + j * 4 * RB);
+                    acc[j] = AS_MFMA(b, a[0][kt], acc[j]);
+                }
+            }
+            const int n = n0 + 8 * g;
+            float bias[8], v[8];
+#pragma unroll
+            for (int h = 0; h < 2; ++h) {
+                const f32x4 bv = *reinterpret_cast<const f32x4*>(bias1_s + n + 4 * h);
+#pragma unroll
+                for (int e = 0; e < 4; ++e) bias[4 * h + e] = bv[e];
+            }
+            as_epi_head(v, acc[0], acc[1], bias, 1.f);
+            if constexpr ((EM1 & AS_PREOUT) != 0) {
+                as_v8 t;
+#pragma unroll
+                for (int e = 0; e < 8; ++e) t[e] = (as_t)v[e];
+                as_t* pp = reinterpret_cast<as_t*>(e1.pre_out) + eoff1 + n0;
+                if (st_ok) {
+                    if (!hold) as_st_pk(pp, t, nt_side);
+                    else if (sub == 1) { as_st_pk(pp - NS, held_pre, nt_side); as_st_pk(pp, t, nt_side); }
+                }
+                if (sub == 0) held_pre = t;
+            }
+            as_epi_tail<as_t, 8>(v, e1, (EM1 & AS_ACT) != 0, f_drop1, false, (EM1 & AS_DACT) != 0, false, rk1, (uint32_t)n, 1.f, au, none);
+            as_v8 us;
+#pragma unroll
+            for (int e = 0; e < 8; ++e) us[e] = (as_t)v[e];
+            {
+                as_t* cp = C1 + eoff1 + n0;
+                if (st_ok) {
+                    if (!hold) as_st_pk(cp, us, FWD && nt_side);
+                    else if (sub == 1) { as_st_pk(cp - NS, held, FWD && nt_side); as_st_pk(cp, us, FWD && nt_side); }
+                }
+                if (sub == 0) held = us;
+            }
+            const char* st2 = st + off2;
+#pragma unroll
+            for (int t2 = 0; t2 < N2 / 32; ++t2) {
+#pragma unroll
+                for (int jj = 0; jj < 2; ++jj) {
+                    const as_v8 b = *reinterpret_cast<const as_v8*>(st2 + t2 * 2048 + jj * 256);
+                    acc2[t2][jj] = AS_MFMA(b, us, acc2[t2][jj]);
+                }
+            }
+            __builtin_amdgcn_sched_group_barrier(0x100, 3, 0);
+#pragma unroll
+            for (int q = 0; q < N2 / 16 - 3; ++q) { __builtin_amdgcn_sched_group_barrier(0x8, 1, 0); __builtin_amdgcn_sched_group_barrier(0x100, 1, 0); }
+            __builtin_amdgcn_sched_group_barrier(0x8, 3, 0);
+        }
+        slot ^= STAGE;
+    }
+    as_u32x4 rs[N2 / 32];
+    const as_t* resid = reinterpret_cast<const as_t*>(e2.resid);
+#pragma unroll
+    for (int t2 = 0; t2 < N2 / 32; ++t2) {
+        rs[t2] = as_u32x4{};
+        if constexpr ((EM2 & AS_RESID) != 0) rs[t2] = *reinterpret_cast<const as_u32x4*>(resid + eoff2 + 32 * t2);
+    }
+#pragma unroll
+    for (int t2 = 0; t2 < N2 / 32; ++t2) {
+        const int n = 32 * t2 + 8 * g;
+        float bias[8], v[8];
+#pragma unroll
+        for (int h = 0; h < 2; ++h) {
+            const f32x4 bv = *reinterpret_cast<const f32x4*>(bias2_s + n + 4 * h);
+#pragma unroll
+            for (int e = 0; e < 4; ++e) bias[4 * h + e] = bv[e];
+        }
+        as_epi_head(v, acc2[t2][0], acc2[t2][1], bias, 1.f);
+        as_epi_tail<as_t, 8>(v, e2, false, f_drop2, false, false, (EM2 & AS_RESID) != 0, rk2, (uint32_t)n, 1.f, rs[t2], rs[t2]);
+        as_v8 t;
+#pragma unroll
+        for (int e = 0; e < 8; ++e) t[e] = (as_t)v[e];
+        if (st_ok) as_st_pk(C2 + eoff2 + 32 * t2, t, false);
+    }
+    if constexpr (PRO != 0) {
+        if (e1.pro_out && m < M) {
+            as_v8* p = reinterpret_cast<as_v8*>(reinterpret_cast<as_t*>(e1.pro_out) + (size_t)m * K1 + g * 8);
+#pragma unroll
+            for (int kt = 0; kt < KT; ++kt) as_st_pk(reinterpret_cast<as_t*>(&p[kt * 4]), a[0][kt], nt_side);
+        }
+    }
+}
+
+template <int EM1, int EM2, int PRO>
+__global__ __launch_bounds__(AS_FFN_NW * 64, 1) void gemm_nt_as_ffn_kernel(const as_t* __restrict__ A, const as_t* __restrict__ B1, int ldb1, const as_t* __restrict__ B2, int ldb2,
+                                                                            as_t* __restrict__ C1, as_t* __restrict__ C2, int M, EpiArgs e1, EpiArgs e2) {
+    extern __shared__ __attribute__((aligned(16))) char fsm[];
+    float* bias1_s = reinterpret_cast<float*>(fsm + 2 * 65536);
+    float* bias2_s = bias1_s + 512;
+    for (int n = threadIdx.x; n < 512; n += (int)blockDim.x) bias1_s[n] = e1.bias ? e1.bias[n] : 0.f;
+    for (int n = threadIdx.x; n < 256; n += (int)blockDim.x) bias2_s[n] = e2.bias ? e2.bias[n] : 0.f;
+#pragma unroll 1
+    for (int p = 0; p < AS_CHUNK_ROWS / AS_FFN_ROWS; ++p) {
+        const int m_base = blockIdx.x * AS_CHUNK_ROWS + p * AS_FFN_ROWS;
+        if (m_base >= M) break;
+        if (p) __syncthreads();
+        as_ffn_pass<EM1, EM2, PRO>(A, B1, ldb1, B2, ldb2, C1, C2, M, e1, e2, fsm, bias1_s, bias2_s, m_base);
+    }
+}
+#endif
 
 static int as_mask_of(const EpiArgs& ea) {
     return (ea.resid ? AS_RESID : 0) | (ea.dact != DACT_NONE ? AS_DACT : 0) | (ea.act != ACT_NONE ? AS_ACT : 0) | (ea.drop.thr ? AS_DROP : 0) |
@@ -530,9 +754,12 @@
 int g_as_flags_override = -1;
 #endif
 static int as_default_flags() {
-    static const int v = getenv("ISHARA_AS_FLAGS") ? atoi(getenv("ISHARA_AS_FLAGS")) : 51;
+    static const int v = getenv("ISHARA_AS_FLAGS") ? atoi(getenv("ISHARA_AS_FLAGS")) : 115;
     return g_as_flags_override >= 0 ? g_as_flags_override : v;
 }
+#ifndef AS_F16
+int gemm_nt_as_flags() { return as_default_flags(); }
+#endif
 static bool as_chunk_applies(int flags, int M, int N, int K, const EpiArgs& ea) {
     const int cs = K == 256 ? 4 : 2;
     return (K == 256 ? (flags & 16) : (K == 512 && (flags & 32))) && M >= 128 * AS_CHUNK_ROWS && (N / AS_NS) % cs == 0 && N >= 128 && !ea.n_valid && !ea.dbg &&
@@ -630,6 +857,63 @@
     return false;
 }
 
+bool gemm_nt_big_applicable(int dtA, int dtM, int dtC, int op, const void* A, int M, int N, int K, int ldb, const EpiArgs& ea);
+static int as_ffn_inst(const EpiArgs& e1, const EpiArgs& e2) {
+    const int m1 = as_mask_of(e1), m2 = as_mask_of(e2);
+    if (e1.pa_P || e2.ln_gamma || e2.pa_P) return -1;
+    if (e1.ln_gamma) {
+        if (m1 != (AS_ACT | AS_PREOUT | AS_DROP) && m1 != (AS_ACT | AS_PREOUT)) return -1;
+        if (m2 != AS_RESID && m2 != (AS_RESID | AS_DROP)) return -1;
+        return (m1 & AS_DROP ? 1 : 0) | (m2 & AS_DROP ? 2 : 0);
+    }
+    if (m2 != 0) return -1;
+    return m1 == (AS_DACT | AS_DROP) ? 4 : (m1 == AS_DACT ? 5 : -1);
+}
+bool gemm_nt_as_ffn_ok(int dt, const void* A, int M, int K1, int N1, int N2, int ldb1, int ldb2, const EpiArgs& e1, const EpiArgs& e2) {
+    const int flags = e1.as_flags < 0 ? as_default_flags() : e1.as_flags;
+    if (!(flags & 64) || dt != DT_BF16 || K1 != 256 || N1 != 512 || N2 != 256 || M < 1 || g_force_regstage) return false;
+    if (!(flags & 128) && M < 128 * AS_CHUNK_ROWS) return false;
+    if (ldb1 < K1 || ldb1 % 64 != 0 || ldb2 < N1 || ldb2 % 8 != 0 || ((uintptr_t)A) % 16 != 0) return false;
+    if (e1.dbg || e2.dbg || e1.n_valid || e2.n_valid || e1.ldc || e2.ldc) return false;
+    if (gemm_nt_big_applicable(dt, dt, dt, OP_NONE, A, M, N2, N1, ldb2, e2)) return false;
+    return as_ffn_inst(e1, e2) >= 0;
+}
+const char* gemm_nt_as_ffn_name(const EpiArgs& e1, const EpiArgs& e2) {
+    static std::map<int, std::string> names;
+    const int id = as_ffn_inst(e1, e2);
+    auto it = names.find(id);
+    if (it == names.end()) {
+        char buf[64];
+        snprintf(buf, sizeof buf, "gemm_nt_as_ffn_kernel<%d,%d,%d>", as_mask_of(e1), as_mask_of(e2), e1.ln_gamma ? 1 : 0);
+        it = names.emplace(id, buf).first;
+    }
+    return it->second.c_str();
+}
+int launch_gemm_nt_as_ffn(int dt, const void* A, const void* B1, int ldb1, const void* B2, int ldb2, void* C1, void* C2, int M, int K1, int N1, int N2,
+                          const EpiArgs& e1_in, const EpiArgs& e2_in, hipStream_t s) {
+    if (!gemm_nt_as_ffn_ok(dt, A, M, K1, N1, N2, ldb1, ldb2, e1_in, e2_in)) return 1;
+    EpiArgs e1 = e1_in, e2 = e2_in;
+    if (e1.as_flags < 0) e1.as_flags = as_default_flags();
+    e2.as_flags = e1.as_flags;
+    const dim3 grid((M + AS_CHUNK_ROWS - 1) / AS_CHUNK_ROWS), block(AS_FFN_NW * 64);
+#define AS_FFN_LAUNCH(M1, M2, PRO)                                                                                                       \
+    do {                                                                                                                                 \
+        if (!as_chunk_prepare(gemm_nt_as_ffn_kernel<M1, M2, PRO>, AS_FFN_LDS)) { ishara_set_error("gemm_nt_as_ffn: %d bytes of dynamic LDS refused", AS_FFN_LDS); return -2; } \
+        hipLaunchKernelGGL((gemm_nt_as_ffn_kernel<M1, M2, PRO>), grid, block, AS_FFN_LDS, s, (const as_t*)A, (const as_t*)B1, ldb1, (const as_t*)B2, ldb2,       \
+                           (as_t*)C1, (as_t*)C2, M, e1, e2);                                                                             \
+    } while (0)
+    switch (as_ffn_inst(e1, e2)) {
+        case 0: AS_FFN_LAUNCH(AS_ACT | AS_PREOUT, AS_RESID, 1); break;
+        case 1: AS_FFN_LAUNCH(AS_ACT | AS_PREOUT | AS_DROP, AS_RESID, 1); break;
+        case 2: AS_FFN_LAUNCH(AS_ACT | AS_PREOUT, AS_RESID | AS_DROP, 1); break;
+        case 3: AS_FFN_LAUNCH(AS_ACT | AS_PREOUT | AS_DROP, AS_RESID | AS_DROP, 1); break;
+        case 4: AS_FFN_LAUNCH(AS_DACT | AS_DROP, 0, 0); break;
+        default: AS_FFN_LAUNCH(AS_DACT, 0, 0); break;
+    }
+#undef AS_FFN_LAUNCH
+    return hipGetLastError() == hipSuccess ? 0 : -2;
+}
+
 bool gemm_nt_as_applicable(int dtC, int M, int N, int K, int ldb, const EpiArgs& ea) {
     if (K != 256 && K != 512 && !((K == 128 || K == 1024) && dtC == DT_BF16)) return false;
     if (N % AS_NS != 0 || N > AS_MAXN || ldb < K || ldb % 8 != 0 || M < 1) return false;
diff --git a/ishara_amd/csrc/keras_hybrid.hip b/ishara_amd/csrc/keras_hybrid.hip
--- a/ishara_amd/csrc/keras_hybrid.hip
+++ b/ishara_amd/csrc/keras_hybrid.hip
@@ -297,9 +297,18 @@
     int rc;
     const void* ain = ln_prologue(m, f.Wa, r, x, f.ln, f.eps, f.xn, f.mean, f.rstd, ea, &rc);
     CK(rc);
-    CK(gemm_fwd(m, f.Wa, ain, dt, m->W(f.u), dt, r.M, OP_NONE, no, ea));
     EpiArgs eb; eb.resid = x;
     if (f.has_out_drop) eb.drop = dspec(r, f.site_out, m->cfg.dropout_rate);
+    if (f.Wa.b >= 0) ea.bias = m->P(f.Wa.b);
+    if (f.Wb.b >= 0) eb.bias = m->P(f.Wb.b);
+    if (ain == x && gemm_nt_as_ffn_ok(dt, x, r.M, f.Wa.K, f.Wa.N, f.Wb.N, f.Wa.ldt, f.Wb.ldt, ea, eb)) {
+        const double es = (double)dt_size(dt);
+        const double by = r.M * es * (2.0 * f.Wa.K + (ea.pro_out ? f.Wa.K : 0) + 2.0 * f.Wa.N + f.Wb.N) + 2.0 * f.Wa.K * f.Wa.N * es;
+        CKP(m, gemm_nt_as_ffn_name(ea, eb), by, 2.0 * r.M * ((double)f.Wa.K * f.Wa.N + (double)f.Wb.K * f.Wb.N),
+            launch_gemm_nt_as_ffn(dt, x, m->ws + f.Wa.wt, f.Wa.ldt, m->ws + f.Wb.wt, f.Wb.ldt, m->W(f.u), m->W(f.out), r.M, f.Wa.K, f.Wa.N, f.Wb.N, ea, eb, m->s));
+        return 0;
+    }
+    CK(gemm_fwd(m, f.Wa, ain, dt, m->W(f.u), dt, r.M, OP_NONE, no, ea));
     CK(gemm_fwd(m, f.Wb, m->W(f.u), dt, m->W(f.out), dt, r.M, OP_NONE, no, eb));
     return 0;
 }
@@ -502,10 +511,16 @@
     const void* gs = f.has_out_drop ? grad_through_dropout(m, r, f.site_out, m->cfg.dropout_rate, g, m->W(m->t3), m->T, m->d, &rc) : g;
     CK(rc);
     EpiArgs e1; e1.drop = dspec(r, f.site_in, m->cfg.dropout_rate); e1.dact = DACT_SWISH; e1.aux = m->W(f.za);
-    CK(gemm_dgrad(m, f.Wb, gs, dt, m->W(m->t1), r.M, OP_NONE, no, e1));
+    EpiArgs e0;
+    const bool pair = gemm_nt_as_ffn_ok(dt, gs, r.M, f.Wb.N, f.Wb.K, f.Wa.K, f.Wb.ldn, f.Wa.ldn, e1, e0);
+    if (pair) {
+        const double es = (double)dt_size(dt);
+        const double by = r.M * es * (2.0 * f.Wb.N + 2.0 * f.Wb.K) + 2.0 * f.Wa.K * f.Wa.N * es;
+        CKP(m, gemm_nt_as_ffn_name(e1, e0), by, 2.0 * r.M * ((double)f.Wa.K * f.Wa.N + (double)f.Wb.K * f.Wb.N),
+            launch_gemm_nt_as_ffn(dt, gs, m->ws + f.Wb.wn, f.Wb.ldn, m->ws + f.Wa.wn, f.Wa.ldn, m->W(m->t1), m->W(m->t2), r.M, f.Wb.N, f.Wb.K, f.Wa.K, e1, e0, m->s));
+    } else CK(gemm_dgrad(m, f.Wb, gs, dt, m->W(m->t1), r.M, OP_NONE, no, e1));
     CK(gemm_wgrad(m, f.Wb, m->W(f.u), dt, OP_NONE, no, gs, dt, OP_NONE, no, r.M));
-    EpiArgs e0;
-    CK(gemm_dgrad(m, f.Wa, m->W(m->t1), dt, m->W(m->t2), r.M, OP_NONE, no, e0));
+    if (!pair) CK(gemm_dgrad(m, f.Wa, m->W(m->t1), dt, m->W(m->t2), r.M, OP_NONE, no, e0));
     CK(gemm_wgrad(m, f.Wa, m->W(f.xn), dt, OP_NONE, no, m->W(m->t1), dt, OP_NONE, no, r.M));
     return layernorm_bwd_deferred(m, r, m->W(m->t2), x, f.mean, f.rstd, f.ln, g, gn);
 }
diff --git a/ishara_amd/csrc/kernels.h b/ishara_amd/csrc/kernels.h
--- a/ishara_amd/csrc/kernels.h
+++ b/ishara_amd/csrc/kernels.h
@@ -77,6 +77,11 @@
 bool gemm_nt_as_applicable(int dtC, int M, int N, int K, int ldb, const EpiArgs& ea);
 bool gemm_nt_as_prologue_ok(int dtA, int dtM, int dtC, int M, int N, int K, int ldb, const EpiArgs& ea);
 const char* gemm_nt_kernel_name(int dtA, int dtM, int dtC, int op, const void* A, int M, int N, int K, int ldb, const EpiArgs& ea);
+bool gemm_nt_as_ffn_ok(int dt, const void* A, int M, int K1, int N1, int N2, int ldb1, int ldb2, const EpiArgs& e1, const EpiArgs& e2);
+int launch_gemm_nt_as_ffn(int dt, const void* A, const void* B1, int ldb1, const void* B2, int ldb2, void* C1, void* C2, int M, int K1, int N1, int N2,
+                          const EpiArgs& e1, const EpiArgs& e2, hipStream_t s);
+const char* gemm_nt_as_ffn_name(const EpiArgs& e1, const EpiArgs& e2);
+int gemm_nt_as_flags();
 extern int g_force_tn_regstage;
 extern int g_force_regstage, g_dbg_tn, g_force_dw_lds, g_tn_blocks, g_attn_bwd_two_pass, g_as_flags_override, g_nt_big;
 extern int g_tn_phase;
```

After: 6.851 million frames/s. About the same (-0.1%).
